# FocoosAI/focoos

Measured on AMD Instinct MI355X. Metric: images/sec @ 640^2 (infer bs=32), higher is better.
Workload: dtype bf16; 1 GPU; fai-detr-l-obj365 inference, bf16 MFMA, bs=32/GPU, 640x640, random-init weights (seed 0), uint8 HWC images resident in HBM, device post-process + D2H of packed detections included; global_batch=32, parallelism=replicas x1 (no data-path collective), steps_are=hipGraph replays, batches_in_flight=3, concurrent_batch_parts=1

## Files before the change

focoos_amd/_lib.py:

```python
from __future__ import annotations

import ctypes as C
import os
from typing import Optional

from .build import LIB_PATH, LIB_PATH_FP16

FX_ACT = {None: 0, "none": 0, "relu": 1, "silu": 2, "gelu": 3}


class FocoosAmdError(RuntimeError):
    pass


class FxConvDesc(C.Structure):
    _fields_ = [
        ("x", C.c_void_p), ("w", C.c_void_p), ("bias", C.c_void_p), ("residual", C.c_void_p), ("y", C.c_void_p),
        ("B", C.c_int32), ("H", C.c_int32), ("W", C.c_int32), ("C", C.c_int32), ("ldx", C.c_int32),
        ("Ho", C.c_int32), ("Wo", C.c_int32), ("N", C.c_int32), ("ldy", C.c_int32), ("ldr", C.c_int32),
        ("KH", C.c_int32), ("KW", C.c_int32), ("stride", C.c_int32), ("pad", C.c_int32),
        ("pool2", C.c_int32), ("act", C.c_int32), ("out_f32", C.c_int32), ("residual_after_act", C.c_int32),
        ("y_batch_stride", C.c_int64), ("w_frag", C.c_void_p), ("mask", C.c_void_p), ("ldm", C.c_int32), ("reserved0", C.c_int32),
    ]


def conv_frag_eligible(n: int, c: int, k: int, c32: bool = True) -> bool:
    if k == 1:
        return n % 256 == 0 and c % 256 == 0
    if k != 3:
        return False
    if c == 32:
        return c32 and n in (32, 64)
    return (n in (64, 128) or n % 256 == 0) and c % 64 == 0


class FxAugRecord(C.Structure):
    _fields_ = [
        ("crop_w", C.c_int32), ("crop_h", C.c_int32), ("pad_x", C.c_int32), ("pad_y", C.c_int32), ("res_w", C.c_int32), ("res_h", C.c_int32),
        ("crop_x", C.c_int32), ("crop_y", C.c_int32), ("flags", C.c_int32), ("reserved0", C.c_int32),
        ("brightness", C.c_float), ("contrast", C.c_float), ("saturation", C.c_float), ("reserved1", C.c_int32 * 3),
    ]


class FxPackEntry(C.Structure):
    _fields_ = [
        ("w", C.c_void_p), ("scale", C.c_void_p), ("bias", C.c_void_p), ("w_fwd", C.c_void_p), ("w_dgrad", C.c_void_p),
        ("w_fwd_frag", C.c_void_p), ("w_dgrad_frag", C.c_void_p), ("bias_out", C.c_void_p),
        ("N", C.c_int32), ("C", C.c_int32), ("KH", C.c_int32), ("KW", C.c_int32), ("ld_fwd", C.c_int32), ("ld_dgrad", C.c_int32),
        ("first_block", C.c_int32), ("n_offset", C.c_int32), ("n_total", C.c_int32), ("reserved", C.c_int32),
    ]


class FxPublishEntry(C.Structure):
    _fields_ = [
        ("w", C.c_void_p), ("bn_weight", C.c_void_p), ("bn_bias", C.c_void_p), ("bn_mean", C.c_void_p), ("bn_var", C.c_void_p),
        ("bias", C.c_void_p), ("w_rows", C.c_void_p), ("w_frag", C.c_void_p), ("bias_out", C.c_void_p), ("eps", C.c_double),
        ("N", C.c_int32), ("C", C.c_int32), ("KH", C.c_int32), ("KW", C.c_int32), ("Np", C.c_int32), ("first_block", C.c_int32),
    ]


class FxPwChainDesc(C.Structure):
    _fields_ = [
        ("x1", C.c_void_p), ("x2", C.c_void_p), ("residual", C.c_void_p), ("w1", C.c_void_p), ("bias1", C.c_void_p), ("y1", C.c_void_p),
        ("w2", C.c_void_p), ("bias2", C.c_void_p), ("y2", C.c_void_p),
        ("M", C.c_int32), ("K1a", C.c_int32), ("K1b", C.c_int32), ("N1", C.c_int32), ("N2", C.c_int32),
        ("ldx1", C.c_int32), ("ldx2", C.c_int32), ("ldr", C.c_int32), ("ldy1", C.c_int32), ("ldy2", C.c_int32),
        ("act1", C.c_int32), ("act2", C.c_int32),
        ("pool", C.c_void_p), ("ldp", C.c_int32), ("img_h", C.c_int32), ("img_w", C.c_int32), ("reserved0", C.c_int32),
    ]


class FxRcStage(C.Structure):
    _fields_ = [
        ("type", C.c_int32), ("K", C.c_int32), ("N", C.c_int32), ("act", C.c_int32),
        ("src", C.c_int32), ("dst", C.c_int32), ("aux", C.c_int32),
        ("ld", C.c_int32), ("ld2", C.c_int32), ("flags", C.c_int32),
        ("w", C.c_void_p), ("bias", C.c_void_p), ("gamma", C.c_void_p), ("beta", C.c_void_p), ("g0", C.c_void_p), ("g1", C.c_void_p),
    ]


_vp, _i, _f = C.c_void_p, C.c_int, C.c_float

SIGNATURES = {
    "fx_abi_version": [],
    "fx_build_flags": [],
    "fx_device_info": [_i, C.POINTER(C.c_int), C.c_char_p, _i],
    "fx_conv2d_nhwc_bf16": [C.POINTER(FxConvDesc), _vp],
    "fx_conv2d_variant": [_vp, C.c_char_p, _i],
    "fx_pw_chain_supported": [_i, _i, _i, _i],
    "fx_pw_chain_pool_supported": [_i, _i, _i, _i],
    "fx_conv3x3_flat_supported": [_i, _i, _i],
    "fx_pw_chain_bf16": [C.POINTER(FxPwChainDesc), _vp],
    "fx_stem_conv3x3s2": [_vp, _i, _vp, _vp, _vp, _vp, _vp, _i, _i, _i, _i, _vp],
    "fx_stem16_conv3x3s2": [_vp, _i, _vp, _vp, _vp, _vp, _vp, _i, _i, _i, _vp],
    "fx_conv3x3_c16_nhwc_bf16": [_vp, _i, _vp, _vp, _i, _vp, _i, _i, _i, _i, _i, _i, _i, _vp],
    "fx_semseg_eval_accumulate": [_vp, _vp, _i, _i, _i, _i, _i, _i, _i, _vp, C.c_int64, _vp, _vp, _i, _i, _vp, _vp, _vp, _vp, _vp],
    "fx_detr_eval_boxes_f32": [_vp, _vp, _vp, _i, _i, _i, _i, _vp, _vp, _vp, _vp, _vp],
    "fx_coco_match_workspace_bytes": [_i],
    "fx_coco_match_bbox": [_vp, _vp, _vp, _vp, _i, _i, _i, _vp, _vp, _vp, _vp, _vp, _vp, C.c_int64, _i, _vp, _vp, _vp, _vp, _vp, _vp, C.c_size_t,
                           _vp],
    "fx_mf_eval_masks_workspace_bytes": [_i, _i, _i],
    "fx_mf_eval_masks": [_vp, _vp, _vp, _i, _i, _i, _i, _i, _i, _i, _i, _vp, _vp, _vp, _vp, C.c_int64, _f, _vp, _vp, _vp, _vp, _vp, _vp, _vp, _vp,
                         _vp, _vp, C.c_size_t, _vp],
    "fx_coco_mask_inter": [_vp, _vp, _vp, C.c_int64, _vp, _vp, _vp, _i, _i, _i, _vp, _vp, _vp, _vp, _vp, C.c_int64, _vp, _vp, _vp, C.c_int64, _vp,
                           _vp, _vp],
    "fx_coco_match_segm": [_vp, _vp, _vp, _vp, _i, _i, _i, _i, _vp, _vp, _vp, _vp, _vp, _vp, _vp, C.c_int64, _i, _vp, _vp, _vp, _vp, _vp, _vp,
                           C.c_size_t, _vp],
    "fx_augment_images_u8": [_vp, _vp, _vp, _vp, _vp, C.c_int64, _vp, _vp, _i, _vp, _i, _i, _i, _vp, _vp],
    "fx_augment_labels": [_vp, _vp, _vp, _vp, _vp, _vp, C.c_int64, _vp, _vp, _vp, _i, _i, _vp, _i, _i, _i, _i, _vp, _vp],
    "fx_resize_bilinear_u8": [_vp, _i, _i, _vp, _i, _i, _vp],
    "fx_tile_gather_u8_f32": [_vp, _i, _i, _vp, _vp, _i, _vp, _i, _i, _vp],
    "fx_merge_detections_workspace_bytes": [_i, _i],
    "fx_merge_detections_nms": [_vp, _vp, _vp, _vp, _vp, _i, _i, _i, _i, _f, _i, _i, _vp, _vp, _vp, _vp, _vp, _vp, C.c_size_t, _vp],
    "fx_annotate_labels_from_detections": [_vp, _vp, _vp, _vp, _i, _i, _vp, _vp, _i, _i, _i, _i, _i, _i, _vp, _vp],
    "fx_annotate_u8": [_vp, _vp, _i, _i, _i, _i, _i, _vp, _vp, _vp, _vp, _vp, _i, C.c_int64, _vp, _vp, _i, _i, _i, _i, _vp],
    "fx_maxpool3x3s2_nhwc_bf16": [_vp, _i, _vp, _i, _i, _i, _i, _i, _vp],
    "fx_stem_conv12_u8_bf16": [_vp, _vp, _vp, _vp, _vp, _vp, _vp, _vp, _i, _i, _i, _i, _vp],
    "fx_stem_conv_pool_supported": [_i, _i, _i, _i],
    "fx_stem_conv3x3_relu_maxpool_bf16": [_vp, _i, _vp, _vp, _vp, _i, _i, _i, _i, _vp],
    "fx_avgpool2x2_nhwc_bf16": [_vp, _i, _vp, _i, _i, _i, _i, _i, _vp],
    "fx_resize_bilinear_nhwc_bf16": [_vp, _i, _vp, _i, _i, _i, _i, _i, _i, _i, _vp],
    "fx_add_rows_bf16": [_vp, _i, _vp, _i, _i, _vp, _i, _i, _i, _vp],
    "fx_layernorm_bf16": [_vp, _i, _vp, _i, _vp, _vp, _vp, _i, _i, _i, _vp],
    "fx_mha_bf16": [_vp, _i, _vp, _i, _vp, _i, _vp, _i, _i, _i, _i, _i, _vp],
    "fx_mha_workspace_bytes": [_i, _i, _i, _i, _i],
    "fx_mha_masked_bf16": [_vp, _i, _vp, _i, _vp, _i, _vp, _i, _i, _i, _i, _i, _vp, _i, _vp, C.c_size_t, _vp],
    "fx_upsample_nearest_add_nhwc_bf16": [_vp, _i, _vp, _i, _vp, _i, _i, _i, _i, _i, _i, _i, _vp],
    "fx_upsample_nearest_bwd_nhwc_bf16": [_vp, _i, _vp, _i, _i, _i, _i, _i, _i, _i, _vp],
    "fx_query_pixel_logits_bf16": [_vp, _i, _vp, _i, _i, _vp, _i, _vp, _i, _i, _i, _i, _i, _vp],
    "fx_mf_class_head": [_vp, _i, _vp, _vp, _vp, _i, _i, _i, _vp],
    "fx_mf_upsample_probs_f32": [_vp, _i, _i, _vp, _i, _i, _i, _vp],
    "fx_mf_upsample_probs_bf16": [_vp, _i, _i, _vp, _i, _i, _i, _vp],
    "fx_mf_postprocess_workspace_bytes": [_i, _i, _i],
    "fx_mf_postprocess_workspace_bytes_fused": [_i, _i, _i, _i, _i, _i],
    "fx_mf_postprocess": [_vp, _i, _i, _i, _i, _vp, _vp, _i, _i, _f, _f, _i, _vp, C.c_size_t, _vp, _vp, _vp, _vp, _vp, _vp, _vp, _vp],
    "fx_msda_bf16": [_vp, _i, _vp, _vp, _i, _i, _vp, _i, _vp, _i, _vp, _i, _vp, _i, _i, _i, _i, _i, _vp],
    "fx_rowmax_f32": [_vp, _i, _vp, _i, _i, _vp],
    "fx_enc_score_head_bf16": [_vp, _i, _vp, _i, _vp, _vp, _vp, _vp, _f, _vp, _vp, _i, _vp, _i, _vp, _i, _vp],
    "fx_row_chain": [_vp, _i, _i, _i, _vp],
    "fx_topk_rows_f32": [_vp, _i, _i, _i, _i, _vp, _vp, _vp],
    "fx_topk_rows_workspace_bytes": [_i, _i, _i],
    "fx_topk_rows_ws_f32": [_vp, _i, _i, _i, _i, _vp, _vp, _vp, C.c_size_t, _vp],
    "fx_gather_rows_bf16": [_vp, _i, _i, _vp, _i, _vp, _i, _i, _i, _vp],
    "fx_fill_rows_bf16": [_vp, _i, _i, _vp, _i, _vp, _i, _i, _vp],
    "fx_linear_k4_relu": [_vp, _vp, _vp, _vp, _i, _i, _i, _vp],
    "fx_bbox_head": [_vp, _i, _vp, _vp, _vp, _vp, _vp, _i, _i, _vp, _vp, _i, _i, _vp],
    "fx_detr_head_out": [_vp, _i, _vp, _vp, _vp, _i, _i, _vp],
    "fx_detr_postprocess": [_vp, _vp, _vp, _vp, _i, _i, _i, _i, _f, _vp, _vp, _vp, _vp, _vp],
    "fx_detr_match_cost_f32": [_vp, _i, _vp, _vp, _vp, _vp, _i, _i, _i, _i, _f, _f, _f, _f, _f, _vp, _vp],
    "fx_lsa_f32": [_vp, _i, _i, _i, _vp, _vp, _vp, _vp],
    "fx_lsa_status_f32": [_vp, _i, _i, _i, _vp, _vp, _vp, _vp, _vp],
    "fx_detr_set_loss_workspace_bytes": [_i, _i, _i],
    "fx_detr_set_loss_f32": [_vp, _i, _vp, _vp, _vp, _vp, _vp, _vp, _i, _i, _i, _i, _f, _f, _f, _f, _f, _f, _vp, _vp, _vp],
    "fx_detr_box_loss_f32": [_vp, _vp, _vp, _vp, _vp, _vp, _i, _i, _i, _i, _f, _f, _vp, _vp, _vp, _vp, _vp],
    "fx_detr_box_loss_bwd_f32": [_vp, _vp, _vp, _i, _i, _i, _vp, _vp, _vp, _vp],
    "fx_msda_f32_fwd": [_vp, _vp, _vp, _i, _i, _vp, _vp, _vp, _i, _i, _i, _i, _vp],
    "fx_msda_f32_bwd": [_vp, _vp, _vp, _i, _i, _vp, _vp, _vp, _vp, _vp, _vp, _i, _i, _i, _i, _vp],
    "fx_msda_train_fwd": [_vp, _i, _i, _vp, _vp, _i, _i, _vp, _vp, _vp, _i, _i, _i, _i, _vp],
    "fx_msda_train_bwd": [_vp, _i, _i, _vp, _vp, _i, _i, _vp, _vp, _vp, _vp, _i, _i, _vp, _vp, _i, _i, _i, _i, _vp],
    "fx_msda_bwd_slab_supported": [_vp, _i, _i, _i, _i, _i],
    "fx_msda_prep_bf16": [_vp, _i, _vp, _i, _vp, _vp, _vp, _i, _i, _i, _i, _vp],
    "fx_msda_prep_bwd_bf16": [_vp, _vp, _vp, _vp, _vp, _i, _vp, _i, _i, _i, _i, _i, _vp],
    "fx_msda_train_bwd_slab": [_vp, _i, _i, _vp, _vp, _vp, _i, _i, _vp, _vp, _vp, _i, _vp, _i, _vp, _vp, _i, _i, _i, _i, _vp],
    "fx_adamw_workspace_bytes": [],
    "fx_adamw_step_f32": [_vp, _vp, _vp, _vp, C.c_int64, _vp, _vp, _vp, _vp, _i, _i, _f, _f, _f, _f, _vp, _vp, _vp],
    "fx_adamw_step_scaled_f32": [_vp, _vp, _vp, _vp, C.c_int64, _vp, _vp, _vp, _vp, _i, _f, _f, _f, _f, _vp, _vp, _vp, _f, _f, _i, _vp],
    "fx_conv2d_wgrad_nhwc_bf16": [_vp, _i, _vp, _i, _vp, _i, _i, _i, _i, _i, _i, _i, _i, _i, _i, _i, _vp],
    "fx_conv2d_wgrad_bias_nhwc_bf16": [_vp, _i, _vp, _i, _vp, _vp, _i, _i, _i, _i, _i, _i, _i, _i, _i, _i, _i, _vp],
    "fx_point_sample_f32": [_vp, _i, _i, _i, _vp, _vp, _vp, _vp, _i, _i, _vp],
    "fx_mask_match_cost_f32": [_vp, _i, _vp, _vp, _vp, _vp, _i, _i, _i, _i, _i, C.c_float, C.c_float, C.c_float, _i, _vp, _vp],
    "fx_mask_match_cost_workspace_bytes": [_i, _i, _i],
    "fx_mask_match_cost_ws_f32": [_vp, _i, _vp, _vp, _vp, _vp, _i, _i, _i, _i, _i, C.c_float, C.c_float, C.c_float, _i, _vp, _vp, C.c_size_t, _vp],
    "fx_mask_set_loss_workspace_bytes": [_i, _i, _i, _i],
    "fx_mask_set_loss_f32": [_vp, _i, _vp, _i, _i, _vp, _i, _i, _i, _vp, _vp, _i, _vp, _vp, _vp, _i, _vp, _i, _i, _i, _i, _i, C.c_float, C.c_float,
                             C.c_float, C.c_float, C.c_float, _vp, C.c_size_t, _vp, _vp],
    "fx_mask_set_loss_cls_f32": [_vp, _i, _vp, _i, _i, _vp, _i, _i, _i, _vp, _vp, _i, _vp, _vp, _vp, _i, _vp, _i, _i, _i, _i, _i, C.c_float, _i, C.c_float,
                                 C.c_float, C.c_float, C.c_float, C.c_float, C.c_float, _vp, C.c_size_t, _vp, _vp],
    "fx_mask_class_loss_workspace_bytes": [_i, _i],
    "fx_mask_class_loss_f32": [_vp, _i, _vp, _vp, _vp, _vp, _i, _i, _i, _i, C.c_float, C.c_float, C.c_float, C.c_float, _vp, C.c_size_t, _vp, _vp],
    "fx_mask_class_loss_bwd_f32": [_vp, _i, _vp, _vp, _vp, _vp, _i, _i, _i, _i, C.c_float, C.c_float, C.c_float, C.c_float, _vp, _vp, _i, _vp],
    "fx_dwconv3x3s2_nhwc_bf16": [_vp, _i, _vp, _vp, _vp, _i, _i, _i, _i, _i, _vp],
    "fx_dwconv3x3s2_nhwc_f32out": [_vp, _i, _vp, _vp, _vp, _i, _i, _i, _i, _i, _vp],
    "fx_global_mean_nhwc_bf16": [_vp, _i, _vp, _i, _i, _i, _i, _vp],
    "fx_pooled_linear_f32": [_vp, _i, _vp, _vp, _i, _vp, _i, _i, _i, _i, _vp],
    "fx_channel_gate_nhwc_bf16": [_vp, _i, _vp, _i, _i, _vp, _i, _vp, _i, _vp, _i, _i, _i, _i, _vp],
    "fx_seg_postprocess_workspace_bytes": [_i, _i, _i, _i, _i, _i],
    "fx_seg_postprocess": [_vp, _i, _i, _i, _i, _vp, _vp, _i, _i, C.c_float, _i, _vp, C.c_size_t, _vp, _vp, _vp, _vp, _vp, _vp, _vp, _vp, _vp],
    "fx_pack_conv_weights_f32": [_vp, _vp, _vp, _vp, _vp, _vp, _i, _i, _i, _i, _vp],
    "fx_unpack_conv_wgrad_f32": [_vp, _vp, _vp, _i, _i, _i, _i, _i, _i, _vp],
    "fx_linear_wgrad_bias_bf16": [_vp, _i, _vp, _i, _vp, _i, _vp, _i, _i, _i, _i, _i, _vp],
    "fx_conv2d_wgrad_splits": [_i, _i, _i, _i, _i, _i, _i],
    "fx_conv2d_wgrad_variant": [_i, _i, _i, _i, _i, _i, _i, _i, _i, C.c_char_p, _i],
    "fx_conv2d_wgrad_partial_nhwc_bf16": [_vp, _i, _vp, _i, _vp, C.c_int64, _i, _i, _i, _i, _i, _i, _i, _i, _i, _i, _i, _i, _vp],
    "fx_unpack_conv_wgrad_sum_f32": [_vp, C.c_int64, _i, _vp, _vp, _i, _i, _i, _i, _i, _i, _vp],
    "fx_relu_bwd_bf16": [_vp, _i, _vp, _i, _vp, _i, _vp, _i, C.c_int64, _i, _i, _vp],
    "fx_zero_insert2_nhwc_bf16": [_vp, _i, _vp, _i, _i, _i, _i, _i, _i, _i, _vp],
    "fx_avgpool2x2_bwd_nhwc_bf16": [_vp, _i, _vp, _i, _i, _i, _i, _i, _vp],
    "fx_maxpool3x3s2_bwd_nhwc_bf16": [_vp, _i, _vp, _i, _vp, _i, _i, _i, _i, _i, _vp, _vp],
    "fx_normalize_pad8": [_vp, _i, _vp, _vp, _vp, C.c_int64, _vp],
    "fx_stem_conv3x3s2_linear": [_vp, _i, _vp, _vp, _vp, _vp, _vp, _i, _i, _i, _i, _vp],
    "fx_bn_stats_bf16": [_vp, _i, _i, _vp, C.c_int64, _i, _vp],
    "fx_bn_finalize_f32": [_vp, C.c_float, _vp, _vp, C.c_float, C.c_float, _vp, _vp, _vp, _vp, _vp, _vp, _vp, _i, _vp],
    "fx_bn_apply_bf16": [_vp, _i, _i, _vp, _vp, _vp, _i, _i, _vp, _i, C.c_int64, _i, _vp],
    "fx_bn_bwd_stats_bf16": [_vp, _i, _vp, _i, _i, _vp, _i, _vp, _vp, _vp, _vp, _i, _vp, C.c_int64, _i, _vp],
    "fx_bn_bwd_apply_bf16": [_vp, _i, _vp, _i, _i, _vp, _i, _vp, _vp, _vp, _vp, _i, _vp, C.c_float, _vp, _i, _vp, _i, C.c_int64, _i, _vp, _vp, _vp],
    "fx_act_fwd_bf16": [_vp, _i, _vp, _i, C.c_int64, _i, _i, _vp],
    "fx_act_bwd_bf16": [_vp, _i, _vp, _i, _vp, _i, C.c_int64, _i, _i, _vp],
    "fx_colsum_bf16": [_vp, _i, _vp, C.c_int64, _i, _vp],
    "fx_layernorm_bwd_bf16": [_vp, _i, _vp, _i, _vp, _vp, _i, _vp, _vp, _i, _i, _vp],
    "fx_resize_bilinear_bwd_nhwc_bf16": [_vp, _i, _vp, _i, _i, _i, _i, _i, _i, _i, _vp],
    "fx_cast_f32_bf16": [_vp, _vp, C.c_int64, _vp],
    "fx_mha_bwd_workspace_bytes": [_i, _i, _i, _i],
    "fx_mha_bwd_bf16": [_vp, _i, _vp, _i, _vp, _i, _vp, _i, _vp, _i, _vp, _i, _vp, _i, _vp, _i, _i, _i, _i, _i, _vp, C.c_size_t, _vp],
    "fx_mha_masked_bwd_bf16": [_vp, _i, _vp, _i, _vp, _i, _vp, _i, _vp, _i, _vp, _i, _vp, _i, _i, _i, _i, _i, _vp, _i, _vp, C.c_size_t, _vp],
    "fx_mask_set_loss_bwd_f32": [_vp, _i, _vp, _i, _i, _vp, _i, _i, _i, _vp, _vp, _i, _vp, _vp, _vp, _i, _vp, _i, _i, _i, _i, _i, C.c_float, C.c_float,
                                 C.c_float, C.c_float, C.c_float, _vp, C.c_size_t, _vp, _vp, _i, _vp, _vp],
    "fx_mask_set_loss_cls_bwd_f32": [_vp, _i, _vp, _i, _i, _vp, _i, _i, _i, _vp, _vp, _i, _vp, _vp, _vp, _i, _vp, _i, _i, _i, _i, _i, C.c_float, _i, C.c_float,
                                     C.c_float, C.c_float, C.c_float, C.c_float, C.c_float, _vp, C.c_size_t, _vp, _vp, _i, _vp, _vp],
    "fx_planes_to_rows_bf16": [_vp, _i, _i, _vp, _i, _i, _i, _vp],
    "fx_dwconv3x3s2_bwd_nhwc_bf16": [_vp, _i, _vp, _i, _vp, _vp, _i, _vp, _i, _i, _i, _i, _vp],
    "fx_rowdot_nhwc_bf16": [_vp, _i, _vp, _i, C.c_float, _vp, _i, _i, _i, _i, _i, _vp],
    "fx_bcast_vec_nhwc_bf16": [_vp, _i, C.c_float, _vp, _i, _i, _i, _i, _vp],
    "fx_scatter_rows_bf16": [_vp, _i, _vp, _i, _vp, _i, _i, _i, _i, _vp],
    "fx_pack_entry_blocks": [_i, _i, _i, _i],
    "fx_pack_weights_many_f32": [_vp, _i, _i, _vp],
    "fx_pack_frag_bf16": [_vp, _vp, _i, _i, _vp],
    "fx_publish_entry_blocks": [_i, _i, _i, _i],
    "fx_publish_weights_f32": [_vp, _i, _i, _vp],
    "fx_pack_linear_weights_f32": [_vp, _vp, _vp, _vp, _vp, _i, _i, _i, _i, _vp],
    "fx_box_refine_f32": [_vp, _vp, _vp, C.c_int64, _f, _vp],
    "fx_box_refine_bwd_f32": [_vp, _vp, _vp, _vp, _vp, C.c_int64, _f, _vp],
    "fx_vfl_loss_bf16": [_vp, _i, _vp, _vp, _f, _f, _f, _vp, _vp, _i, C.c_int64, _i, _vp],
    "fx_stream_fork": [_vp, _vp],
    "fx_stream_join": [_vp, _vp],
    "fx_graph_begin": [_vp],
    "fx_graph_end": [_vp, C.POINTER(C.c_void_p)],
    "fx_graph_launch": [_vp, _vp],
    "fx_graph_destroy": [_vp],
    "fx_graph_time": [_vp, _vp, _i, C.POINTER(C.c_float)],
}

_libs: dict = {}
_DTYPE = [os.environ.get("FX_DTYPE", "bf16")]


def compute_dtype() -> str:
    return _DTYPE[0]


def set_compute_dtype(name: str) -> str:
    if name not in ("bf16", "fp16"):
        raise FocoosAmdError(f"compute dtype {name!r}: the engine has a bfloat16 and an fp16 (+ loss scale) build")
    prev, _DTYPE[0] = _DTYPE[0], name
    return prev


class using_compute_dtype:

    def __init__(self, name: str):
        self.name, self.prev = name, None

    def __enter__(self):
        self.prev = set_compute_dtype(self.name)
        return self

    def __exit__(self, *exc):
        _DTYPE[0] = self.prev
        return False


def act_dtype():
    import torch

    return torch.float16 if _DTYPE[0] == "fp16" else torch.bfloat16


def lib_path(name: str = None) -> str:
    if (name or _DTYPE[0]) == "fp16":
        return os.environ.get("FOCOOS_AMD_LIB_FP16", LIB_PATH_FP16)
    return os.environ.get("FOCOOS_AMD_LIB", LIB_PATH)


FX_ABI_VERSION = 17


def load(name: str = None) -> C.CDLL:
    name = name or _DTYPE[0]
    if name in _libs:
        return _libs[name]
    import torch
    path = lib_path(name)
    if not os.path.exists(path):
        raise FocoosAmdError(
            f"{path} not found: the gfx950 HIP kernels are not built. Run `python -c 'import __graft_entry__ as g; g.build()'` "
            "(or `python -m focoos_amd.build`). focoos_amd has no CPU/PyTorch fallback by design."
        )
    lib = C.CDLL(path)
    for sym, argtypes in SIGNATURES.items():
        fn = getattr(lib, sym)
        fn.argtypes = argtypes
        fn.restype = C.c_int
    lib.fx_mha_bwd_workspace_bytes.restype = C.c_size_t
    lib.fx_seg_postprocess_workspace_bytes.restype = C.c_size_t
    lib.fx_mask_match_cost_workspace_bytes.restype = C.c_size_t
    lib.fx_mf_postprocess_workspace_bytes_fused.restype = C.c_size_t
    lib.fx_mask_set_loss_workspace_bytes.restype = C.c_size_t
    lib.fx_mask_class_loss_workspace_bytes.restype = C.c_size_t
    lib.fx_topk_rows_workspace_bytes.restype = C.c_size_t
    lib.fx_coco_match_workspace_bytes.restype = C.c_size_t
    lib.fx_mf_eval_masks_workspace_bytes.restype = C.c_size_t
    lib.fx_merge_detections_workspace_bytes.restype = C.c_size_t
    lib.fx_error_string.argtypes = [C.c_int]
    lib.fx_error_string.restype = C.c_char_p
    if lib.fx_abi_version() != FX_ABI_VERSION:
        raise FocoosAmdError(f"ABI version mismatch: library {lib.fx_abi_version()} != binding {FX_ABI_VERSION} (stale {os.path.basename(path)}: rebuild)")
    if bool(lib.fx_build_flags() & 2) != (name == "fp16"):
        raise FocoosAmdError(f"{path} was built for the other 16-bit element type (fx_build_flags = {lib.fx_build_flags()}) than {name!r}")
    _libs[name] = lib
    return lib


_warned_pk = False


def two_queue_safe() -> bool:
    global _warned_pk
    if not (load().fx_build_flags() & 1) or os.environ.get("FX_ALLOW_PK_TWO_QUEUES") == "1":
        return True
    if not _warned_pk:
        import warnings

        warnings.warn("libfocoos_amd was built with packed-fp32 instructions (FX_PK_F32): concurrent batch parts and the weight-gradient "
                      "side stream are disabled (two-queue hazard); rebuild without FX_PK_F32 for the default configuration")
        _warned_pk = True
    return False


def check(rc: int, what: str = "") -> None:
    if rc != 0:
        msg = load().fx_error_string(rc).decode()
        raise FocoosAmdError(f"libfocoos_amd {what} failed: {msg} (code {rc})")
```

focoos_amd/csrc/conv3x3_flat.hip:

```cpp
#include <type_traits>

#include "pw_common.h"

struct C3Args {
  const bf16_t* x;
  const bf16_t* wp;
  const float* bias;
  const bf16_t* res;
  bf16_t* y;
  int H, W, C, N, ldx, ldy, ldr, M;
  int act, res_after;
  int HLp;
  int HW;
  int64_t y_bstride;
  unsigned x_bytes, r_bytes;
};

template <int KT, int CC, int TN, int TM, int WN, int WM, int ACT, int RESMODE, int LOADER = 1>
__global__ __launch_bounds__((WN* WM + LOADER) * 64, 1) void conv3x3_flat_kernel(const C3Args p) {
  constexpr int NW = WN * WM, NT = (NW + LOADER) * 64, NDW = NW + LOADER;
  constexpr int BM = WM * TM * 32, BN = WN * TN * 32;
  constexpr int RL = CC / 8, ROWB = CC * 2;
  constexpr int KJ = 4;
  constexpr int NTAP = KT == 9 ? 9 : CC / 64;
  constexpr int PF = KJ;
  constexpr int RLT = BN / 8;
  static_assert(TN <= 2 && (KT == 9 ? CC == 64 : CC % 64 == 0), "tap = 64 channels = 4 k-steps");
  extern __shared__ __attribute__((aligned(16))) unsigned char smem[];

  const int tid = threadIdx.x, lane = tid & 63;
  const int wave = __builtin_amdgcn_readfirstlane(tid >> 6);
  const bool is_loader = LOADER && wave == NW;
  const int l32 = lane & 31, half = lane >> 5;
  const int wn = wave % WN, wm = wave / WN;
  const int nNt = p.N / BN;
  const int bid = fx_xcd_remap(blockIdx.x, gridDim.x);
  const int m0 = (bid / nNt) * BM, n0 = (bid % nNt) * BN;
  const int lo = KT == 9 ? m0 - p.W - 1 : m0;
  const int NCH = p.C / CC;
  const int buf_bytes = p.HLp * ROWB;
  const __amdgpu_buffer_rsrc_t xr = __builtin_amdgcn_make_buffer_rsrc((void*)p.x, 0, p.x_bytes, 0x00020000);
  unsigned char* T = smem;

  auto dma_chunk = [&](int cc, unsigned char* buf, int first, int step) {
    const int ninstr = p.HLp * RL / 64;
    for (int i = first; i < ninstr; i += step) {
      const int q = i * 64 + lane;
      const int r = q / RL, pc = q % RL;
      const int lc = pw_swz<RL>(r, pc);
      const int f = lo + r;
      const bool ok = f >= 0 && f < p.M;
      pw_dma16(xr, buf + i * 1024, ok ? (unsigned)(f * p.ldx + cc * CC + lc * 8) * 2u : FX_OOB);
    }
  };

  auto dma_res = [&](int first) {
    const __amdgpu_buffer_rsrc_t rr = __builtin_amdgcn_make_buffer_rsrc((void*)p.res, 0, p.r_bytes, 0x00020000);
    for (int i = first; i < BM * RLT / 64; i += NDW) {
      const int q = i * 64 + lane;
      const int r = q / RLT, pc = q % RLT;
      const int lc = pw_swz<RLT>(r, pc);
      const int m = m0 + r;
      pw_dma16(rr, T + i * 1024, m < p.M ? (unsigned)(m * p.ldr + n0 + lc * 8) * 2u : FX_OOB);
    }
  };

  f32x16 acc[TN][TM];
  bf16x8 ar[PF][TN];
  unsigned mask9[TM];
  int rbase[TM];
  const int Cs = p.C >> 4;
  const bf16_t* wbase = p.wp + (size_t)((n0 >> 5) + wn * TN) * (size_t)(KT * Cs) * 512 + lane * 8;
  auto a_ptr = [&](int a, int cc, int s) -> const bf16_t* {
    const int ks = KT == 9 ? (s / KJ) * Cs + cc * KJ + (s % KJ) : cc * (CC / 16) + s;
    return wbase + ((size_t)a * (size_t)(KT * Cs) + ks) * 512;
  };
  if (is_loader) {
    if (lane < 8) *reinterpret_cast<uint4*>(smem + (NCH > 1 ? 2 : 1) * buf_bytes + lane * 16) = make_uint4(0, 0, 0, 0);
    dma_chunk(0, smem, NW, NDW);
    for (int cc = 0; cc < NCH; ++cc) {
      asm volatile("s_waitcnt vmcnt(0)" ::: "memory");
      __syncthreads();
      if (cc + 1 < NCH) dma_chunk(cc + 1, smem + ((cc + 1) & 1) * buf_bytes, 0, 1);
    }
    __syncthreads();
    if constexpr (RESMODE != 0) {
      dma_res(NW);
      asm volatile("s_waitcnt vmcnt(0)" ::: "memory");
      __syncthreads();
    }
    __syncthreads();
  } else {
    if (!LOADER && wave == 0 && lane < 8) *reinterpret_cast<uint4*>(smem + buf_bytes + lane * 16) = make_uint4(0, 0, 0, 0);
    dma_chunk(0, smem, wave, NDW);
#pragma unroll
    for (int a = 0; a < TN; ++a)
#pragma unroll
      for (int gq = 0; gq < 4; ++gq) {
        const float4 bb = p.bias ? *reinterpret_cast<const float4*>(p.bias + n0 + (wn * TN + a) * 32 + 8 * gq + 4 * half) : make_float4(0.f, 0.f, 0.f, 0.f);
#pragma unroll
        for (int b = 0; b < TM; ++b) {
          acc[a][b][4 * gq] = bb.x; acc[a][b][4 * gq + 1] = bb.y; acc[a][b][4 * gq + 2] = bb.z; acc[a][b][4 * gq + 3] = bb.w;
        }
      }
    const int HW = p.H * p.W;
#pragma unroll
    for (int b = 0; b < TM; ++b) {
      const int pl = (wm * TM + b) * 32 + l32;
      const int m = m0 + pl;
      rbase[b] = KT == 9 ? pl + p.W + 1 : pl;
      const bool ok = m < p.M;
      const int mm = ok ? m : 0;
      const int rem = mm % HW;
      const int yy = rem / p.W, xx = rem - yy * p.W;
      unsigned msk = 0;
#pragma unroll
      for (int t = 0; t < 9; ++t) {
        const int dy = t / 3 - 1, dx = t % 3 - 1;
        if (ok && (unsigned)(yy + dy) < (unsigned)p.H && (unsigned)(xx + dx) < (unsigned)p.W) msk |= 1u << t;
      }
      mask9[b] = KT == 9 ? msk : 0x1ffu;
    }
#pragma unroll
    for (int i = 0; i < PF; ++i)
#pragma unroll
      for (int a = 0; a < TN; ++a) {
        ar[i][a] = bf16x8{0, 0, 0, 0, 0, 0, 0, 0};
        c3_ldg_async(ar[i][a], a_ptr(a, 0, i));
      }
    const int zrow = (NCH > 1 ? 2 : 1) * buf_bytes;
    int hc[KJ];
#pragma unroll
    for (int j = 0; j < KJ; ++j) hc[j] = (j * 2 + half) << 4;
    constexpr int SWM = (RL >= 16 ? 0xf0 : 0x70);
    constexpr int SWS = (RL >= 16 ? 4 : 3);
    auto tap_setup = [&](int t, int toff, int bufo, int (&ra)[TM], int (&sw)[TM]) {
#pragma unroll
      for (int b = 0; b < TM; ++b) {
        const int r = rbase[b] + toff;
        const bool ok = KT == 9 ? ((mask9[b] >> t) & 1u) : true;
        ra[b] = ok ? bufo + r * ROWB : zrow;
        sw[b] = ok ? ((r << SWS) & SWM) : 0;
      }
    };
    for (int cc = 0; cc < NCH; ++cc) {
      if (cc == 0) asm volatile("s_waitcnt vmcnt(0)" ::: "memory");
      __syncthreads();
      const int bufo = (cc & 1) * buf_bytes;
      const int ccn = cc + 1 < NCH ? cc + 1 : cc;
      int ra[TM], sw[TM];
      tap_setup(0, KT == 9 ? -p.W - 1 : 0, bufo, ra, sw);
      bf16x8 xb[2][TM];
#pragma unroll
      for (int b = 0; b < TM; ++b) xb[0][b] = *reinterpret_cast<const bf16x8*>(smem + ((hc[0] ^ sw[b]) + ra[b]));
#pragma unroll 1
      for (int t = 0; t < NTAP; ++t) {
        const int tn = t + 1;
        const bool last_tap = t == NTAP - 1;
        const int co = KT == 9 ? 0 : t * 128, con = KT == 9 ? 0 : tn * 128;
        const bf16_t* wnext[TN];
#pragma unroll
        for (int a = 0; a < TN; ++a) wnext[a] = a_ptr(a, last_tap ? ccn : cc, last_tap ? 0 : tn * KJ);
        int ran[TM], swn[TM];
        tap_setup(last_tap ? 0 : tn, (KT != 9 || last_tap) ? 0 : (tn / 3 - 1) * p.W + (tn % 3 - 1), bufo, ran, swn);
        auto kstep = [&](auto jc) {
          constexpr int j = decltype(jc)::value;
          constexpr bool tap_end = j + 1 == KJ;
          if constexpr (TN == 1) c3_wait<(KJ - 1) * TN>(ar[j][0]); else c3_wait<(KJ - 1) * TN>(ar[j][0], ar[j][1]);
#pragma unroll
          for (int a = 0; a < TN; ++a) {
#pragma unroll
            for (int b = 0; b < TM; ++b) {
              acc[a][b] = FX_MFMA_32x32x16(ar[j][a], xb[j & 1][b], acc[a][b]);
              if (a == 0) {
                if constexpr (!tap_end) {
                  xb[(j + 1) & 1][b] = *reinterpret_cast<const bf16x8*>(smem + (((co + hc[tap_end ? 0 : j + 1]) ^ sw[b]) + ra[b]));
                } else {
                  if (!last_tap) xb[0][b] = *reinterpret_cast<const bf16x8*>(smem + (((con + hc[0]) ^ swn[b]) + ran[b]));
                }
              }
              if (b == TM - 1) c3_ldg_async<j * 1024>(ar[j][a], wnext[a]);
              __builtin_amdgcn_sched_barrier(0);
            }
          }
        };
        c3_static_for<KJ>(kstep);
#pragma unroll
        for (int b = 0; b < TM; ++b) {
          ra[b] = ran[b];
          sw[b] = swn[b];
        }
      }
    }
#pragma unroll
    for (int i = 0; i < PF; ++i) {
      if constexpr (TN == 1) c3_wait<0>(ar[i][0]); else c3_wait<0>(ar[i][0], ar[i][1]);
    }
    __syncthreads();
    if constexpr (RESMODE != 0) {
      dma_res(wave);
      asm volatile("s_waitcnt vmcnt(0)" ::: "memory");
      __syncthreads();
    }
  #pragma unroll
      for (int a = 0; a < TN; ++a)
  #pragma unroll
        for (int b = 0; b < TM; ++b)
  #pragma unroll
          for (int gq = 0; gq < 4; ++gq) {
            const int row = (wm * TM + b) * 32 + l32;
            const int chunk = (wn * TN + a) * 4 + gq;
            unsigned char* tp = T + row * (BN * 2) + (pw_swz<RLT>(row, chunk) << 4) + half * 8;
            float v0 = acc[a][b][4 * gq], v1 = acc[a][b][4 * gq + 1], v2 = acc[a][b][4 * gq + 2], v3 = acc[a][b][4 * gq + 3];
            float r0 = 0.0f, r1 = 0.0f, r2 = 0.0f, r3 = 0.0f;
            if constexpr (RESMODE != 0) {
              const uint2 rv = *reinterpret_cast<const uint2*>(tp);
              r0 = bf16lo_to_f32(rv.x); r1 = bf16hi_to_f32(rv.x);
              r2 = bf16lo_to_f32(rv.y); r3 = bf16hi_to_f32(rv.y);
            }
            if constexpr (RESMODE == 1) { v0 += r0; v1 += r1; v2 += r2; v3 += r3; }
            if constexpr (ACT == FX_ACT_RELU) {
              v0 = fmaxf(v0, 0.0f); v1 = fmaxf(v1, 0.0f); v2 = fmaxf(v2, 0.0f); v3 = fmaxf(v3, 0.0f);
            } else if constexpr (ACT == FX_ACT_SILU) {
              v0 = v0 / (1.0f + __expf(-v0)); v1 = v1 / (1.0f + __expf(-v1)); v2 = v2 / (1.0f + __expf(-v2)); v3 = v3 / (1.0f + __expf(-v3));
            }
            if constexpr (RESMODE == 2) { v0 += r0; v1 += r1; v2 += r2; v3 += r3; }
            if constexpr (RESMODE == 3) {
              v0 = r0 > 0.0f ? v0 : 0.0f; v1 = r1 > 0.0f ? v1 : 0.0f; v2 = r2 > 0.0f ? v2 : 0.0f; v3 = r3 > 0.0f ? v3 : 0.0f;
            }
            uint2 o;
            o.x = pack_bf16x2(v0, v1);
            o.y = pack_bf16x2(v2, v3);
            *reinterpret_cast<uint2*>(tp) = o;
          }

    __syncthreads();
  }
  for (int q = tid; q < BM * RLT; q += NT) {
    const int row = q / RLT, lc = q % RLT;
    const int m = m0 + row;
    if (m < p.M) {
      const uint4 v = *reinterpret_cast<const uint4*>(T + row * (BN * 2) + (pw_swz<RLT>(row, lc) << 4));
      size_t yo = (size_t)m * p.ldy;
      if (p.y_bstride) {
        const int bb = m / p.HW;
        yo = (size_t)bb * p.y_bstride + (size_t)(m - bb * p.HW) * p.ldy;
      }
      *reinterpret_cast<uint4*>(p.y + yo + n0 + lc * 8) = v;
    }
  }
}

template <int KT, int CC, int TN, int TM, int WN, int WM, int ACT, int RESMODE, int LOADER = 1>
static int launch_c3(C3Args& a, hipStream_t stream) {
  constexpr int NW = WN * WM, BM = WM * TM * 32, BN = WN * TN * 32, RL = CC / 8;
  constexpr int RPI = 64 / RL > 0 ? 64 / RL : 1;
  const int HL = BM + (KT == 9 ? 2 * a.W + 2 : 0);
  a.HLp = (HL + RPI - 1) / RPI * RPI;
  const int halo = (a.C / CC > 1 ? 2 : 1) * a.HLp * CC * 2 + 128, tile = BM * BN * 2;
  const int smem = halo > tile ? halo : tile;
  if (smem > 160 * 1024) return FX_ERR_UNSUPPORTED;
  if (!LOADER && a.C != CC) return FX_ERR_UNSUPPORTED;
  auto kern = conv3x3_flat_kernel<KT, CC, TN, TM, WN, WM, ACT, RESMODE, LOADER>;
  static int attr_smem = 0;
  if (smem > attr_smem) {
    if (hipFuncSetAttribute(reinterpret_cast<const void*>(kern), hipFuncAttributeMaxDynamicSharedMemorySize, smem) != hipSuccess) return FX_ERR_RUNTIME;
    attr_smem = smem;
  }
  hipLaunchKernelGGL(kern, dim3(((a.M + BM - 1) / BM) * (a.N / BN)), dim3((NW + LOADER) * 64), smem, stream, a);
  return fx_launch_status();
}

int fx_c3_epilogue_mode(int act, bool has_res, int res_after) {
  if (!has_res) return act == FX_ACT_RELU ? 0 : (act == FX_ACT_SILU ? 1 : (act == FX_ACT_NONE ? 3 : -1));
  if (act == FX_ACT_SILU && res_after == 1) return 2;
  if (act == FX_ACT_RELU && res_after == 0) return 4;
  if (act == FX_ACT_NONE && res_after == 2) return 5;
  if (act == FX_ACT_NONE && res_after == 0) return 6;
  return -1;
}

bool fx_conv3x3_flat_fits(int C, int N, int W) {
  if (C % 64 != 0 || !(N == 64 || N == 128 || N == 256)) return false;
  const int BM = N == 256 ? 128 : 256;
  const int HLp = (BM + 2 * W + 2 + 7) / 8 * 8;
  const int halo = (C / 64 > 1 ? 2 : 1) * HLp * 128 + 128, tile = BM * N * 2;
  return (halo > tile ? halo : tile) <= 160 * 1024;
}

extern "C" int fx_conv3x3_flat_supported(int C, int N, int W) {
  return (fx_conv3x3_kplane_supported(C, N, W) || fx_conv3x3_c32_supported(C, N, W, 0) || fx_conv3x3_flat_fits(C, N, W)) ? 1 : 0;
}

static void c3_fill(C3Args& a, const ConvArgs& c, const bf16_t* w_frag) {
  a.x = c.x; a.wp = w_frag; a.bias = c.bias; a.res = c.res; a.y = reinterpret_cast<bf16_t*>(c.y);
  a.H = c.H; a.W = c.W; a.C = c.C; a.N = c.N; a.ldx = c.ldx; a.ldy = c.ldy; a.ldr = c.ldr; a.M = c.M;
  a.act = c.act; a.res_after = c.res_after; a.HLp = 0; a.HW = c.Ho * c.Wo; a.y_bstride = c.y_bstride;
  a.x_bytes = c.x_bytes; a.r_bytes = c.r_bytes;
}

int fx_launch_conv3x3_flat(const ConvArgs& c, const bf16_t* w_frag, int mode, hipStream_t stream) {
  C3Args a;
  c3_fill(a, c, w_frag);
#define FX_C3_TILE(ACT_, RM_)                                                      \
  {                                                                                \
    if (c.N == 64) return launch_c3<9, 64, 1, 4, 2, 2, ACT_, RM_>(a, stream);      \
    if (c.N == 128) return launch_c3<9, 64, 2, 4, 2, 2, ACT_, RM_>(a, stream);     \
    return launch_c3<9, 64, 2, 4, 4, 1, ACT_, RM_>(a, stream);                     \
  }
  switch (mode) {
    case 0: FX_C3_TILE(FX_ACT_RELU, 0)
    case 1: FX_C3_TILE(FX_ACT_SILU, 0)
    case 2: FX_C3_TILE(FX_ACT_SILU, 2)
    case 3: FX_C3_TILE(FX_ACT_NONE, 0)
    case 5: FX_C3_TILE(FX_ACT_NONE, 3)
    default: return FX_ERR_UNSUPPORTED;
  }
#undef FX_C3_TILE
}

int fx_launch_pw_flat(const ConvArgs& c, const bf16_t* w_frag, int mode, hipStream_t stream) {
  C3Args a;
  c3_fill(a, c, w_frag);
  static const int no_loader = fx_tune("FX_PW_NO_LOADER", 1);
  if (c.C == 256 && no_loader) {
    switch (mode) {
      case 0: return launch_c3<1, 256, 2, 4, 4, 1, FX_ACT_RELU, 0, 0>(a, stream);
      case 1: return launch_c3<1, 256, 2, 4, 4, 1, FX_ACT_SILU, 0, 0>(a, stream);
      case 3: return launch_c3<1, 256, 2, 4, 4, 1, FX_ACT_NONE, 0, 0>(a, stream);
      case 4: return launch_c3<1, 256, 2, 4, 4, 1, FX_ACT_RELU, 1, 0>(a, stream);
      case 5: return launch_c3<1, 256, 2, 4, 4, 1, FX_ACT_NONE, 3, 0>(a, stream);
      case 6: return launch_c3<1, 256, 2, 4, 4, 1, FX_ACT_NONE, 1, 0>(a, stream);
      default: return FX_ERR_UNSUPPORTED;
    }
  }
  static const int bm64 = fx_tune("FX_PWF_BM64_MAX_M", 20000);
  if (c.M <= bm64 && (mode == 0 || mode == 3)) {
    if (mode == 0) return launch_c3<1, 256, 2, 2, 4, 1, FX_ACT_RELU, 0>(a, stream);
    return launch_c3<1, 256, 2, 2, 4, 1, FX_ACT_NONE, 0>(a, stream);
  }
  switch (mode) {
    case 0: return launch_c3<1, 256, 2, 4, 4, 1, FX_ACT_RELU, 0>(a, stream);
    case 1: return launch_c3<1, 256, 2, 4, 4, 1, FX_ACT_SILU, 0>(a, stream);
    case 3: return launch_c3<1, 256, 2, 4, 4, 1, FX_ACT_NONE, 0>(a, stream);
    case 4: return launch_c3<1, 256, 2, 4, 4, 1, FX_ACT_RELU, 1>(a, stream);
    case 5: return launch_c3<1, 256, 2, 4, 4, 1, FX_ACT_NONE, 3>(a, stream);
    case 6: return launch_c3<1, 256, 2, 4, 4, 1, FX_ACT_NONE, 1>(a, stream);
    default: return FX_ERR_UNSUPPORTED;
  }
}
```

focoos_amd/csrc/conv_igemm.hip:

```cpp
#include <stdio.h>

#include "conv_common.h"

template <int BM, int BN, int BK, int WM, int WN, bool POOL, int NSTAGE = 2>
__global__ __launch_bounds__(256, (BK == 32 ? 4 : 2)) void conv_igemm_kernel(const ConvArgs p) {
  constexpr int CPR = BK / 8, RPP = 256 / CPR;
  constexpr int A_PASS = BM / RPP, B_PASS = (BN + RPP - 1) / RPP;
  constexpr int WTM = BM / WM, WTN = BN / WN, TM = WTM / 32, TN = WTN / 32;
  constexpr int A_BYTES = BM * BK * 2, B_BYTES = BN * BK * 2, STAGE = A_BYTES + B_BYTES;
  constexpr int EPI_LD = BN + 4;
  static_assert(WM * WN == 4, "4 waves");
  static_assert(BM % RPP == 0, "A passes");
  extern __shared__ __attribute__((aligned(16))) unsigned char smem[];

  const int tid = threadIdx.x, lane = tid & 63, wave = tid >> 6;
  const int wm = wave / WN, wn = wave % WN;
  const int bid = fx_xcd_remap(blockIdx.x, gridDim.x);
  const int mt = bid / p.nNt, nt = bid % p.nNt;
  const int m0 = mt * BM, n0 = nt * BN;

  const __amdgpu_buffer_rsrc_t xr = __builtin_amdgcn_make_buffer_rsrc((void*)p.x, 0, p.x_bytes, 0x00020000);
  const __amdgpu_buffer_rsrc_t wr = __builtin_amdgcn_make_buffer_rsrc((void*)p.w, 0, p.w_bytes, 0x00020000);

  const int kc = tid % CPR, r_in = tid / CPR;
// ... 28 lines not shown
    _Pragma("unroll") for (int i = 0; i < A_PASS; ++i) {                                                             \
      if constexpr (!POOL) {                                                                                         \
        int hi = a_hi0[i] + (KH_), wi = a_wi0[i] + (KW_);                                                            \
        bool ok = a_ok[i] && (unsigned)hi < (unsigned)p.H && (unsigned)wi < (unsigned)p.W;                           \
        ra[i] = buf_load16(xr, ok ? (unsigned)(a_off[i] + delta_) * 2u : FX_OOB);                                     \
      } else {                                                                                                       \
        float s_[8] = {0, 0, 0, 0, 0, 0, 0, 0};                                                                      \
        int cnt_ = 0;                                                                                                \
        _Pragma("unroll") for (int dy = 0; dy < 2; ++dy) _Pragma("unroll") for (int dx = 0; dx < 2; ++dx) {          \
          bool ok = a_ok[i] && (a_hi0[i] + dy) < p.H && (a_wi0[i] + dx) < p.W;                                       \
          uint4 v_ = buf_load16(xr, ok ? (unsigned)(a_off[i] + delta_ + (dy * p.W + dx) * p.ldx) * 2u : FX_OOB);      \
          float f_[8];                                                                                               \
          unpack_bf16x8(v_, f_);                                                                                     \
          _Pragma("unroll") for (int j = 0; j < 8; ++j) s_[j] += f_[j];                                              \
          cnt_ += ok ? 1 : 0;                                                                                        \
        }                                                                                                            \
        float inv_ = cnt_ > 0 ? 1.0f / (float)cnt_ : 0.0f;                                                           \
        _Pragma("unroll") for (int j = 0; j < 8; ++j) s_[j] *= inv_;                                                 \
        ra[i] = pack_bf16x8(s_);                                                                                     \
      }                                                                                                              \
    }                                                                                                                \
    _Pragma("unroll") for (int i = 0; i < B_PASS; ++i) {                                                             \
      if (BN % RPP == 0 || r_in + i * RPP < BN) rb[i] = buf_load16(wr, w_off[i] + (unsigned)(KBASE_)*2u);            \
    }                                                                                                                \
  }
#define FX_STORE_TILES(S_)                                                                                           \
  {                                                                                                                  \
    unsigned char* A_ = smem + (S_)*STAGE;                                                                           \
    unsigned char* B_ = A_ + A_BYTES;                                                                                \
    _Pragma("unroll") for (int i = 0; i < A_PASS; ++i) *reinterpret_cast<uint4*>(A_ + lds_off<BK>(r_in + i * RPP, kc)) = ra[i]; \
    _Pragma("unroll") for (int i = 0; i < B_PASS; ++i) {                                                             \
      if (BN % RPP == 0 || r_in + i * RPP < BN) *reinterpret_cast<uint4*>(B_ + lds_off<BK>(r_in + i * RPP, kc)) = rb[i]; \
    }                                                                                                                \
  }
#define FX_COMPUTE(S_)                                                                                               \
  {                                                                                                                  \
    const unsigned char* A_ = smem + (S_)*STAGE;                                                                     \
    const unsigned char* B_ = A_ + A_BYTES;                                                                          \
    _Pragma("unroll") for (int kk = 0; kk < BK / 16; ++kk) {                                                         \
      const int chunk = kk * 2 + lhalf;                                                                              \
      bf16x8 xa[TM], wb[TN];                                                                                         \
      _Pragma("unroll") for (int i = 0; i < TM; ++i) xa[i] =                                                         \
          *reinterpret_cast<const bf16x8*>(A_ + lds_off<BK>(wm * WTM + i * 32 + lrow, chunk));                       \
      _Pragma("unroll") for (int i = 0; i < TN; ++i) wb[i] =                                                         \
          *reinterpret_cast<const bf16x8*>(B_ + lds_off<BK>(wn * WTN + i * 32 + lrow, chunk));                       \
      _Pragma("unroll") for (int a = 0; a < TN; ++a) _Pragma("unroll") for (int b = 0; b < TM; ++b) acc[a][b] =      \
          FX_MFMA_32x32x16(wb[a], xa[b], acc[a][b]);                                 \
    }                                                                                                                \
  }

  f32x16 acc[TN][TM];
#pragma unroll
  for (int a = 0; a < TN; ++a)
#pragma unroll
    for (int b = 0; b < TM; ++b)
#pragma unroll
      for (int r = 0; r < 16; ++r) acc[a][b][r] = 0.0f;

  const int T = p.KH * p.KW * (p.C / BK);
  const int lrow = lane & 31, lhalf = lane >> 5;
  int kh = 0, kw = 0, c0 = 0, kbase = 0;
  FX_LOAD_TILES(kh, kw, c0, kbase);
  FX_STORE_TILES(0);
  __syncthreads();
  for (int t = 0; t < T - 1; ++t) {
    const int cur = (NSTAGE == 2) ? (t & 1) : 0;
    c0 += BK;
    kbase += BK;
    if (c0 == p.C) {
      c0 = 0;
      if (++kw == p.KW) {
        kw = 0;
        ++kh;
      }
    }
    FX_LOAD_TILES(kh, kw, c0, kbase);
    FX_COMPUTE(cur);
    if constexpr (NSTAGE == 2) {
      FX_STORE_TILES(cur ^ 1);
    } else {
      __syncthreads();
      FX_STORE_TILES(0);
    }
    __syncthreads();
  }
  constexpr int TPR = BN / 8, RPP2 = 256 / TPR, HALF = 64, PER_HALF = HALF / RPP2, NRES = BM / RPP2;
  const int col8 = (tid % TPR) * 8;
  const int n = n0 + col8;
  const bool n_ok = n < p.Nstore;
  uint4 rres[NRES];
  if (p.res) {
    const __amdgpu_buffer_rsrc_t rr = __builtin_amdgcn_make_buffer_rsrc((void*)p.res, 0, p.r_bytes, 0x00020000);
#pragma unroll
    for (int q = 0; q < NRES; ++q) {
      const int m = m0 + (q / PER_HALF) * HALF + tid / TPR + (q % PER_HALF) * RPP2;
      rres[q] = buf_load16(rr, (m < p.M && n_ok) ? (unsigned)(m * p.ldr + n) * 2u : FX_OOB);
    }
  }
  FX_COMPUTE((NSTAGE == 2) ? ((T - 1) & 1) : 0);
  __syncthreads();
#undef FX_LOAD_TILES
#undef FX_STORE_TILES
#undef FX_COMPUTE

  float* stg = reinterpret_cast<float*>(smem);
  float bs[8];
  if (p.bias && n_ok) {
    float4 b0 = *reinterpret_cast<const float4*>(p.bias + n), b1 = *reinterpret_cast<const float4*>(p.bias + n + 4);
    bs[0] = b0.x; bs[1] = b0.y; bs[2] = b0.z; bs[3] = b0.w; bs[4] = b1.x; bs[5] = b1.y; bs[6] = b1.z; bs[7] = b1.w;
  } else {
#pragma unroll
    for (int j = 0; j < 8; ++j) bs[j] = 0.0f;
  }
#pragma unroll
  for (int hh = 0; hh < BM / HALF; ++hh) {
    if ((wm * WTM) / HALF == hh) {
#pragma unroll
      for (int a = 0; a < TN; ++a)
#pragma unroll
        for (int b = 0; b < TM; ++b)
#pragma unroll
          for (int g = 0; g < 4; ++g) {
            int ml = wm * WTM + b * 32 + lrow - hh * HALF;
            int nl = wn * WTN + a * 32 + 8 * g + 4 * lhalf;
            float4 v = make_float4(acc[a][b][4 * g], acc[a][b][4 * g + 1], acc[a][b][4 * g + 2], acc[a][b][4 * g + 3]);
            *reinterpret_cast<float4*>(stg + ml * EPI_LD + nl) = v;
          }
    }
    __syncthreads();
#pragma unroll
    for (int j = 0; j < PER_HALF; ++j) {
      const int r = tid / TPR + j * RPP2;
      const int m = m0 + hh * HALF + r;
      if (m < p.M && n_ok) {
        float4 v0 = *reinterpret_cast<const float4*>(stg + r * EPI_LD + col8);
        float4 v1 = *reinterpret_cast<const float4*>(stg + r * EPI_LD + col8 + 4);
        float v[8] = {v0.x + bs[0], v0.y + bs[1], v0.z + bs[2], v0.w + bs[3], v1.x + bs[4], v1.y + bs[5], v1.z + bs[6], v1.w + bs[7]};
        float rf[8];
        if (p.res) {
          unpack_bf16x8(rres[hh * PER_HALF + j], rf);
          if (!p.res_after) {
#pragma unroll
            for (int i = 0; i < 8; ++i) v[i] += rf[i];
          }
        }
        if (p.act != FX_ACT_NONE) {
#pragma unroll
          for (int i = 0; i < 8; ++i) v[i] = fx_act(v[i], p.act);
        }
        if (p.res && p.res_after == 1) {
#pragma unroll
          for (int i = 0; i < 8; ++i) v[i] += rf[i];
        } else if (p.res && p.res_after == 2) {
#pragma unroll
          for (int i = 0; i < 8; ++i) v[i] = rf[i] > 0.0f ? v[i] : 0.0f;
        }
        if (p.mask) {
          float mf[8];
          unpack_bf16x8(*reinterpret_cast<const uint4*>(p.mask + (size_t)m * p.ldm + n), mf);
#pragma unroll
          for (int i = 0; i < 8; ++i) v[i] = mf[i] > 0.0f ? v[i] : 0.0f;
        }
        int64_t yoff;
        if (p.y_bstride) {
          int bb = m / HoWo;
          yoff = (int64_t)bb * p.y_bstride + (int64_t)(m - bb * HoWo) * p.ldy + n;
        } else {
          yoff = (int64_t)m * p.ldy + n;
        }
        if (p.out_f32) {
          float* dst = reinterpret_cast<float*>(p.y) + yoff;
          *reinterpret_cast<float4*>(dst) = make_float4(v[0], v[1], v[2], v[3]);
          *reinterpret_cast<float4*>(dst + 4) = make_float4(v[4], v[5], v[6], v[7]);
        } else {
          bf16_t* dst = reinterpret_cast<bf16_t*>(p.y) + yoff;
          *reinterpret_cast<uint4*>(dst) = pack_bf16x8(v);
        }
      }
    }
    if (hh + 1 < BM / HALF) __syncthreads();
  }
}

template <int BM, int BN, int BK, int WM, int WN, bool POOL, int NSTAGE = 2>
static int launch_conv(const ConvArgs& c, const bf16_t*, int, hipStream_t stream) {
  constexpr int STAGE = (BM + BN) * BK * 2;
  constexpr int EPI = 64 * (BN + 4) * 4;
  constexpr int SMEM = (NSTAGE * STAGE > EPI) ? NSTAGE * STAGE : EPI;
  static bool attr_set = false;
  auto kern = conv_igemm_kernel<BM, BN, BK, WM, WN, POOL, NSTAGE>;
  if (!attr_set) {
    if (hipFuncSetAttribute(reinterpret_cast<const void*>(kern), hipFuncAttributeMaxDynamicSharedMemorySize, SMEM) != hipSuccess)
      return FX_ERR_RUNTIME;
    attr_set = true;
  }
  ConvArgs a = c;
  a.nNt = (a.N + BN - 1) / BN;
  int nMt = (a.M + BM - 1) / BM;
  dim3 grid(nMt * a.nNt), block(256);
  hipLaunchKernelGGL(kern, grid, block, SMEM, stream, a);
  return fx_launch_status();
}

static int conv_prepare(const fx_conv_desc* d, ConvArgs& a) {
  FX_CHECK_ARG(d && d->x && d->w && d->y);
  FX_CHECK_ARG(d->B > 0 && d->H > 0 && d->W > 0 && d->Ho > 0 && d->Wo > 0 && d->N > 0);
  FX_CHECK_ARG(d->C > 0 && d->C % 32 == 0 && d->ldx >= d->C && d->ldx % 8 == 0);
  FX_CHECK_ARG(d->KH >= 1 && d->KW >= 1 && d->stride >= 1 && d->pad >= 0);
  const int Nstore = (d->N + 7) / 8 * 8;
  FX_CHECK_ARG(d->ldy >= Nstore && d->ldy % 8 == 0);
  FX_CHECK_ARG(!d->residual || (d->ldr >= Nstore && d->ldr % 8 == 0));
  FX_CHECK_ARG(((uintptr_t)d->x % 16) == 0 && ((uintptr_t)d->w % 16) == 0 && ((uintptr_t)d->y % 16) == 0);
  FX_CHECK_ARG(!d->residual || ((uintptr_t)d->residual % 16) == 0);
  FX_CHECK_ARG(!d->bias || ((uintptr_t)d->bias % 16) == 0);
  if (d->pool2) {
    FX_CHECK_ARG(d->KH == 1 && d->KW == 1 && d->stride == 1 && d->pad == 0);
    FX_CHECK_ARG(d->Ho == (d->H + 1) / 2 && d->Wo == (d->W + 1) / 2);
  } else {
    FX_CHECK_ARG(d->Ho == (d->H + 2 * d->pad - d->KH) / d->stride + 1);
    FX_CHECK_ARG(d->Wo == (d->W + 2 * d->pad - d->KW) / d->stride + 1);
  }
  if ((int64_t)d->B * d->H * d->W >= (1ll << 31) || (int64_t)d->B * d->Ho * d->Wo >= (1ll << 31)) return FX_ERR_UNSUPPORTED;
  const int64_t x_bytes = ((int64_t)d->B * d->H * d->W - 1) * d->ldx * 2 + (int64_t)d->C * 2;
  const int64_t Npad = (int64_t)(d->N + 127) / 128 * 128;
  const int64_t w_bytes = Npad * d->KH * d->KW * d->C * 2;
  const int64_t r_bytes = d->residual ? (((int64_t)d->B * d->Ho * d->Wo - 1) * d->ldr + Nstore) * 2 : 0;
  if (x_bytes >= 0xFFFFFFF0ll || w_bytes >= 0xFFFFFFF0ll || r_bytes >= 0xFFFFFFF0ll) return FX_ERR_UNSUPPORTED;
  a.x = reinterpret_cast<const bf16_t*>(d->x);
  a.w = reinterpret_cast<const bf16_t*>(d->w);
  a.bias = d->bias;
  a.res = reinterpret_cast<const bf16_t*>(d->residual);
  a.y = d->y;
  a.B = d->B; a.H = d->H; a.W = d->W; a.C = d->C; a.ldx = d->ldx;
  a.Ho = d->Ho; a.Wo = d->Wo; a.N = d->N; a.ldy = d->ldy; a.ldr = d->ldr;
  a.KH = d->KH; a.KW = d->KW; a.stride = d->stride; a.pad = d->pad;
  a.act = d->act; a.out_f32 = d->out_f32; a.res_after = d->residual_after_act;
  a.y_bstride = d->y_batch_stride;
  FX_CHECK_ARG(d->y_batch_stride >= 0 && d->y_batch_stride % 8 == 0);
  a.M = d->B * d->Ho * d->Wo;
  a.Ktot = d->KH * d->KW * d->C;
  a.Nstore = Nstore;
  a.nNt = 0;
  a.x_bytes = (unsigned)x_bytes;
  a.w_bytes = (unsigned)w_bytes;
  a.r_bytes = (unsigned)r_bytes;
  a.mask = reinterpret_cast<const bf16_t*>(d->mask);
  a.ldm = d->ldm;
  a.m_bytes = 0;
  if (d->mask) {
    FX_CHECK_ARG(d->ldm >= Nstore && d->ldm % 8 == 0 && ((uintptr_t)d->mask % 16) == 0 && !d->out_f32 && !d->pool2);
    const int64_t m_bytes = (((int64_t)d->B * d->Ho * d->Wo - 1) * d->ldm + Nstore) * 2;
    if (m_bytes >= 0xFFFFFFF0ll) return FX_ERR_UNSUPPORTED;
    a.m_bytes = (unsigned)m_bytes;
  }
  return FX_OK;
}

enum ConvRoute {
  R_C32, R_C3K, R_C3_FLAT, R_C3_S2, R_PWK, R_PW_FLAT, R_SMALL_M, R_DMA256, R_DMA128, R_POOL,
  R_K64_N128, R_K64_N64, R_K64_N32, R_K32_N128, R_K32_N64, R_K32_N32, R_UNSUPPORTED
};

static const struct {
  const char* label;
  bool by_c;
  ConvLauncher launch;
} kRoutes[R_UNSUPPORTED] = {
     {"conv3x3_c32<%d>", false, fx_launch_conv3x3_c32},
     {"conv3x3_kplane<%d>", false, fx_launch_conv3x3_kplane},
     {"conv3x3_flat<%d>", false, fx_launch_conv3x3_flat},
     {"conv3x3s2_kplane<%d>", false, fx_launch_conv3x3s2_kplane},
     {"pw_kplane<K%d>", true, fx_launch_pw_kplane},
     {"pw_flat<K%d>", true, fx_launch_pw_flat},
     {"conv_igemm<64,64,256,1stage>", false, launch_conv<64, 64, 256, 2, 2, false, 1>},
     {"conv_igemm_dma<256,256>", false, fx_launch_conv_dma256},
     {"conv_igemm_dma<256,128>", false, fx_launch_conv_dma128},
     {"conv_igemm<128,128,64,pool>", false, launch_conv<128, 128, 64, 2, 2, true>},
     {"conv_igemm<128,128,64>", false, launch_conv<128, 128, 64, 2, 2, false>},
     {"conv_igemm<128,64,64>", false, launch_conv<128, 64, 64, 2, 2, false>},
     {"conv_igemm<128,32,64>", false, launch_conv<128, 32, 64, 4, 1, false>},
     {"conv_igemm<128,128,32>", false, launch_conv<128, 128, 32, 2, 2, false>},
     {"conv_igemm<128,64,32>", false, launch_conv<128, 64, 32, 2, 2, false>},
     {"conv_igemm<128,32,32>", false, launch_conv<128, 32, 32, 4, 1, false>},
};

static ConvRoute conv_route(const fx_conv_desc* d, const ConvArgs& a, int mode) {
  const bool frag = d->w_frag && ((uintptr_t)d->w_frag % 16) == 0 && !d->mask && !d->pool2 && !d->out_f32;
  const int c3_min_m = fx_tune("FX_CONV3_MIN_M", 5000), pw_min_m = fx_tune("FX_PW_MIN_M", 5000);
  static const int c3_on = fx_tune("FX_CONV3_FLAT", 1), c3k_on = fx_tune("FX_C3_KPLANE", 1), c32_on = fx_tune("FX_C3_C32", 1);
  if (frag && c3_on && d->stride == 1 && d->KH == 3 && d->KW == 3 && d->pad == 1 && !d->y_batch_stride &&
      ((mode >= 0 && mode <= 3) || mode == 5) && a.M >= c3_min_m) {
    if (d->C == 32) {
      if (c32_on && fx_conv3x3_c32_supported(d->C, d->N, d->W, mode)) return R_C32;
    } else if (c3k_on && fx_conv3x3_kplane_supported(d->C, d->N, d->W)) {
      return R_C3K;
    } else if (fx_conv3x3_flat_fits(d->C, d->N, d->W)) {
      return R_C3_FLAT;
    }
  }
  static const int pw_on = fx_tune("FX_PW_FLAT", 1), pwk_on = fx_tune("FX_PW_KPLANE", 1);
  if (frag && pw_on && d->stride == 1 && d->KH == 1 && d->KW == 1 && d->pad == 0 && d->C % 256 == 0 && d->N % 256 == 0 && a.M >= pw_min_m &&
      (mode == 0 || mode == 1 || (mode >= 3 && mode <= 6)))
    return (pwk_on && fx_pw_kplane_supported(d->C, d->N, mode)) ? R_PWK : R_PW_FLAT;
  static const int s2_on = fx_tune("FX_C3S2_KPLANE", 1);
  if (frag && s2_on && d->stride == 2 && d->KH == 3 && d->KW == 3 && d->pad == 1 && !d->residual && d->H == 2 * d->Ho && d->W == 2 * d->Wo &&
      a.M >= c3_min_m && (mode == 0 || mode == 1 || mode == 3) && fx_conv3x3s2_kplane_supported(d->C, d->N, d->Wo, a.M))
    return R_C3_S2;
  static const int k64_min = fx_tune("FX_K64_MIN_KTOT", FX_K64_MIN_KTOT);
  static const int small_m = fx_tune("FX_SMALL_M", 16384);
  static const int small_k = fx_tune("FX_SMALL_M_KTOT", 2048);
  if (!d->pool2 && a.M <= small_m && d->C % 256 == 0 && a.Ktot <= small_k) return R_SMALL_M;
  if (!d->pool2 && !d->mask) {
    const int bn = fx_conv_dma_bn(a);
    if (bn) return bn == 256 ? R_DMA256 : R_DMA128;
  }
  if (d->pool2) return d->C % 64 != 0 ? R_UNSUPPORTED : R_POOL;
  if ((d->C % 64 == 0) && (a.Ktot >= k64_min)) return d->N > 64 ? R_K64_N128 : (d->N > 32 ? R_K64_N64 : R_K64_N32);
  return d->N > 64 ? R_K32_N128 : (d->N > 32 ? R_K32_N64 : R_K32_N32);
}

extern "C" int fx_conv2d_nhwc_bf16(const fx_conv_desc* d, fx_stream_t stream) {
  ConvArgs a;
  const int rc = conv_prepare(d, a);
  if (rc != FX_OK) return rc;
  const int mode = fx_c3_epilogue_mode(a.act, a.res != nullptr, a.res_after);
  const ConvRoute r = conv_route(d, a, mode);
  if (r == R_UNSUPPORTED) return FX_ERR_UNSUPPORTED;
  return kRoutes[r].launch(a, reinterpret_cast<const bf16_t*>(d->w_frag), mode, reinterpret_cast<hipStream_t>(stream));
}

extern "C" int fx_conv2d_variant(const fx_conv_desc* d, char* out, int cap) {
  FX_CHECK_ARG(out && cap >= 48);
  ConvArgs a;
  const int rc = conv_prepare(d, a);
  if (rc != FX_OK) return rc;
  const ConvRoute r = conv_route(d, a, fx_c3_epilogue_mode(a.act, a.res != nullptr, a.res_after));
  if (r == R_UNSUPPORTED) return FX_ERR_UNSUPPORTED;
  snprintf(out, cap, kRoutes[r].label, kRoutes[r].by_c ? d->C : d->N);
  return FX_OK;
}
```

focoos_amd/csrc/conv_pw_chain.hip:

```cpp
#include "pw_common.h"

struct PwChainArgs {
  const bf16_t* x1;
  const bf16_t* x2;
  const bf16_t* res;
  const bf16_t* w1p;
  const bf16_t* w2p;
  const float* b1;
  const float* b2;
  bf16_t* y1;
  bf16_t* y2;
  int ldx1, ldx2, ldr, ldy1, ldy2;
  int M, N1, act1, act2;
  unsigned x1_bytes, x2_bytes, r_bytes;
  bf16_t* pool;
  int ldp, H, W;
};

template <int RL, typename F>
__device__ __forceinline__ void pw_dma_rows_map(__amdgpu_buffer_rsrc_t r, unsigned char* tile, int nrows, int ld, int col0, int wave, int lane, F&& pix) {
  const int ninstr = nrows * RL / 64;
  for (int i = wave; i < ninstr; i += 4) {
    const int q = i * 64 + lane;
    const int row = q / RL, pc = q % RL;
    const int lc = pw_swz<RL>(row, pc);
    const int m = pix(row);
    const unsigned off = (m >= 0) ? (unsigned)(m * ld + col0 + lc * 8) * 2u : FX_OOB;
    pw_dma16(r, tile + i * 1024, off);
  }
}

template <int K1A, int K1B, int N2, int BM, bool QUAD = false>
__global__ __launch_bounds__(256, ((N2 <= 64 && K1B == 0) ? 4 : ((N2 <= 128 && (K1B == 0 || N2 <= 64)) ? 3 : 2))) void pw_chain_kernel(const PwChainArgs p) {
  constexpr int K1 = K1A + K1B, KS1 = K1 / 16, KS1A = K1A / 16;
  constexpr int RLA = K1A / 8, RLB = (K1B > 0 ? K1B : 64) / 8;
  constexpr int TM = BM / 32;
  constexpr int XA_BYTES = BM * K1A * 2, XB_BYTES = BM * K1B * 2;
  constexpr int PF1 = KS1 < 4 ? KS1 : 4;
  constexpr bool HAS2 = N2 > 0;
  constexpr int WN2 = !HAS2 ? 1 : (N2 >= 128 ? 4 : 2), WM2 = 4 / WN2;
  constexpr int TN2 = !HAS2 ? 1 : N2 / (32 * WN2), TM2 = BM / (32 * WM2);
  constexpr int RL2 = (HAS2 ? N2 : 64) / 8;
  constexpr int PF2 = 4;
  static_assert(BM == 64, "64-pixel tiles");
  static_assert(K1A % 64 == 0 && K1B % 64 == 0 && PF1 == 4, "K segments in multiples of 64 (= whole blocks of 4 k-steps)");
  static_assert(!HAS2 || (N2 % 64 == 0 && N2 <= 256), "N2");
  extern __shared__ __attribute__((aligned(16))) unsigned char smem[];
  unsigned char* XA = smem;
  unsigned char* XB = smem + XA_BYTES;
  unsigned char* T = smem + XA_BYTES + XB_BYTES;

  const int tid = threadIdx.x, lane = tid & 63;
  const int wave = __builtin_amdgcn_readfirstlane(tid >> 6);
  const int l32 = lane & 31, half = lane >> 5;
  const int m0 = blockIdx.x * BM;
  const int NG = p.N1 >> 8;
  const int KS2 = p.N1 >> 4;

  __shared__ int s_pix[QUAD ? BM : 1];
  if constexpr (QUAD) {
    if (tid < BM) {
      const int W2 = p.W >> 1, QI = (p.H >> 1) * W2;
      const int q = blockIdx.x * (BM / 4) + (tid >> 2), sub = tid & 3;
      int m = -1;
      if (q * 4 < p.M) {
        const int b = q / QI, rem = q - b * QI;
        const int y2 = rem / W2, x2 = rem - y2 * W2;
        m = (b * p.H + 2 * y2 + (sub >> 1)) * p.W + 2 * x2 + (sub & 1);
      }
      s_pix[tid] = m;
    }
    __syncthreads();
  }
  auto pix = [&](int row) -> int {
    if constexpr (!QUAD) {
      const int m = m0 + row;
      return m < p.M ? m : -1;
    } else {
      return s_pix[row];
    }
  };
  const __amdgpu_buffer_rsrc_t x1r = __builtin_amdgcn_make_buffer_rsrc((void*)p.x1, 0, p.x1_bytes, 0x00020000);
  pw_dma_rows_map<RLA>(x1r, XA, BM, p.ldx1, 0, wave, lane, pix);
  if constexpr (K1B > 0) {
    const __amdgpu_buffer_rsrc_t x2r = __builtin_amdgcn_make_buffer_rsrc((void*)p.x2, 0, p.x2_bytes, 0x00020000);
    pw_dma_rows_map<RLB>(x2r, XB, BM, p.ldx2, 0, wave, lane, pix);
  }
  const __amdgpu_buffer_rsrc_t rr = __builtin_amdgcn_make_buffer_rsrc((void*)(p.res ? p.res : p.x1), 0, p.res ? p.r_bytes : 0u, 0x00020000);

  const int wn2 = wave % WN2, wm2 = wave / WN2;
  f32x16 acc2[TN2][TM2];
#pragma unroll
  for (int a = 0; a < TN2; ++a)
#pragma unroll
    for (int b = 0; b < TM2; ++b)
#pragma unroll
      for (int r = 0; r < 16; ++r) acc2[a][b][r] = 0.0f;

  for (int g = 0; g < NG; ++g) {
    int l32g = l32, halfg = half, tidg = tid;
    asm volatile("" : "+v"(l32g), "+v"(halfg), "+v"(tidg));
    if (p.res) pw_dma_rows_map<32>(rr, T, BM, p.ldr, g * 256, wave, lane, pix);
    bf16x8 a2[PF2][TN2];
    const bf16_t* w2 = p.w2p + (size_t)((wn2 * TN2) * KS2 + g * 16) * 512 + lane * 8;
    if constexpr (HAS2) {
#pragma unroll
      for (int i = 0; i < PF2; ++i)
#pragma unroll
        for (int a = 0; a < TN2; ++a) a2[i][a] = pw_ldg_frag(w2 + (size_t)(a * KS2 + i) * 512);
    }
#pragma unroll
    for (int a = 0; a < 2; ++a) {
      const bf16_t* w1 = p.w1p + (size_t)((g * 8 + wave * 2 + a) * KS1) * 512 + lane * 8;
      bf16x8 a1[PF1];
#pragma unroll
      for (int i = 0; i < PF1; ++i) a1[i] = pw_ldg_frag(w1 + i * 512);
      f32x16 acc[TM];
#pragma unroll
      for (int gq = 0; gq < 4; ++gq) {
        const float4 bb = *reinterpret_cast<const float4*>(p.b1 + g * 256 + wave * 64 + a * 32 + 8 * gq + 4 * halfg);
#pragma unroll
        for (int b = 0; b < TM; ++b) {
          acc[b][4 * gq] = bb.x; acc[b][4 * gq + 1] = bb.y; acc[b][4 * gq + 2] = bb.z; acc[b][4 * gq + 3] = bb.w;
        }
      }
      if (a == 0) {
        asm volatile("s_waitcnt vmcnt(0)" ::: "memory");
        __syncthreads();
      }
#define FX_PW_STEPS(XT_, KROW_, RL_, KL0_)                                                                                  \
  _Pragma("unroll") for (int i = 0; i < PF1; ++i) {                                                                         \
    bf16x8 xb[TM];                                                                                                          \
    _Pragma("unroll") for (int b = 0; b < TM; ++b) {                                                                        \
      const int row = b * 32 + l32k;                                                                                         \
      xb[b] = *reinterpret_cast<const bf16x8*>((XT_) + row * ((KROW_)*2) + (pw_swz<RL_>(row, ((KL0_) + i) * 2 + halfg) << 4)); \
    }                                                                                                                       \
    _Pragma("unroll") for (int b = 0; b < TM; ++b) acc[b] = FX_MFMA_32x32x16(a1[i], xb[b], acc[b]); \
    const int kn = ks0 + i + PF1;                                                                                           \
    a1[i] = pw_ldg_frag(w1 + (kn < KS1 ? kn : KS1 - 1) * 512);  \
  }
#pragma unroll 1
      for (int ks0 = 0; ks0 < KS1; ks0 += PF1) {
        int l32k = l32g;
        asm volatile("" : "+v"(l32k));
        if (K1B == 0 || ks0 < KS1A) {
          FX_PW_STEPS(XA, K1A, RLA, ks0)
        } else {
          FX_PW_STEPS(XB, (K1B > 0 ? K1B : 64), RLB, ks0 - KS1A)
        }
      }
#undef FX_PW_STEPS
#pragma unroll
      for (int b = 0; b < TM; ++b)
#pragma unroll
        for (int gq = 0; gq < 4; ++gq) {
          const int row = b * 32 + l32g;
          const int chunk = wave * 8 + a * 4 + gq;
          unsigned char* tp = T + row * 512 + ((chunk ^ (row & 15)) << 4) + halfg * 8;
          float v0 = acc[b][4 * gq], v1 = acc[b][4 * gq + 1], v2 = acc[b][4 * gq + 2], v3 = acc[b][4 * gq + 3];
          if (p.res) {
            const uint2 r2 = *reinterpret_cast<const uint2*>(tp);
            v0 += bf16lo_to_f32(r2.x);
            v1 += bf16hi_to_f32(r2.x);
            v2 += bf16lo_to_f32(r2.y);
            v3 += bf16hi_to_f32(r2.y);
          }
          if (p.act1 == FX_ACT_RELU) {
            v0 = fmaxf(v0, 0.0f); v1 = fmaxf(v1, 0.0f); v2 = fmaxf(v2, 0.0f); v3 = fmaxf(v3, 0.0f);
          }
          uint2 o;
          o.x = pack_bf16x2(v0, v1);
          o.y = pack_bf16x2(v2, v3);
          *reinterpret_cast<uint2*>(tp) = o;
        }
    }
    __syncthreads();
#pragma unroll
    for (int i = 0; i < BM * 32 / 256; ++i) {
      const int q = tidg + i * 256;
      const int row = q >> 5, lc = q & 31;
      const uint4 v = *reinterpret_cast<const uint4*>(T + row * 512 + ((lc ^ (row & 15)) << 4));
      const int m = pix(row);
      if (m >= 0 && p.y1) *reinterpret_cast<uint4*>(p.y1 + (size_t)m * p.ldy1 + g * 256 + lc * 8) = v;
    }
    if constexpr (QUAD) {
#pragma unroll
      for (int i = 0; i < (BM / 4) * 32 / 256; ++i) {
        const int idx = tidg + i * 256;
        const int j = idx >> 5, lc = idx & 31;
        float s8[8] = {0, 0, 0, 0, 0, 0, 0, 0};
#pragma unroll
        for (int r = 0; r < 4; ++r) {
          const int row = 4 * j + r;
          float f[8];
          unpack_bf16x8(*reinterpret_cast<const uint4*>(T + row * 512 + ((lc ^ (row & 15)) << 4)), f);
#pragma unroll
          for (int e = 0; e < 8; ++e) s8[e] += f[e];
        }
#pragma unroll
        for (int e = 0; e < 8; ++e) s8[e] *= 0.25f;
        const int q = blockIdx.x * (BM / 4) + j;
        if (q * 4 < p.M) *reinterpret_cast<uint4*>(p.pool + (size_t)q * p.ldp + g * 256 + lc * 8) = pack_bf16x8(s8);
      }
    }
    if constexpr (HAS2) {
#pragma unroll
      for (int ks = 0; ks < 16; ++ks) {
        bf16x8 tb[TM2];
#pragma unroll
        for (int b = 0; b < TM2; ++b) {
          const int row = (wm2 * TM2 + b) * 32 + l32g;
          tb[b] = *reinterpret_cast<const bf16x8*>(T + row * 512 + (((ks * 2 + halfg) ^ (row & 15)) << 4));
        }
#pragma unroll
        for (int a = 0; a < TN2; ++a)
#pragma unroll
          for (int b = 0; b < TM2; ++b) acc2[a][b] = FX_MFMA_32x32x16(a2[ks % PF2][a], tb[b], acc2[a][b]);
        if (ks + PF2 < 16) {
#pragma unroll
          for (int a = 0; a < TN2; ++a) a2[ks % PF2][a] = pw_ldg_frag(w2 + (size_t)(a * KS2 + ks + PF2) * 512);
        }
      }
    }
    __syncthreads();
  }

  if constexpr (HAS2) {
#pragma unroll
    for (int a = 0; a < TN2; ++a)
#pragma unroll
      for (int gq = 0; gq < 4; ++gq) {
        const int n = (wn2 * TN2 + a) * 32 + 8 * gq + 4 * half;
        const float4 bb = *reinterpret_cast<const float4*>(p.b2 + n);
#pragma unroll
        for (int b = 0; b < TM2; ++b) {
          const int row = (wm2 * TM2 + b) * 32 + l32;
          float v0 = acc2[a][b][4 * gq] + bb.x, v1 = acc2[a][b][4 * gq + 1] + bb.y;
          float v2 = acc2[a][b][4 * gq + 2] + bb.z, v3 = acc2[a][b][4 * gq + 3] + bb.w;
          if (p.act2 == FX_ACT_RELU) {
            v0 = fmaxf(v0, 0.0f); v1 = fmaxf(v1, 0.0f); v2 = fmaxf(v2, 0.0f); v3 = fmaxf(v3, 0.0f);
          }
          uint2 o;
          o.x = pack_bf16x2(v0, v1);
          o.y = pack_bf16x2(v2, v3);
          *reinterpret_cast<uint2*>(T + row * (N2 * 2) + (pw_swz<RL2>(row, n >> 3) << 4) + half * 8) = o;
        }
      }
    __syncthreads();
#pragma unroll
    for (int i = 0; i < BM * RL2 / 256; ++i) {
      const int q = tid + i * 256;
      const int row = q / RL2, lc = q % RL2;
      const uint4 v = *reinterpret_cast<const uint4*>(T + row * (N2 * 2) + (pw_swz<RL2>(row, lc) << 4));
      const int m = pix(row);
      if (m >= 0) *reinterpret_cast<uint4*>(p.y2 + (size_t)m * p.ldy2 + lc * 8) = v;
    }
  }
}

template <int K1A, int K1B, int N2, bool QUAD = false>
static int launch_pw_chain(const PwChainArgs& a, hipStream_t stream) {
  constexpr int BM = 64;
  constexpr int SMEM = BM * (K1A + K1B) * 2 + BM * 512;
  static bool attr_set = false;
  auto kern = pw_chain_kernel<K1A, K1B, N2, BM, QUAD>;
  if (!attr_set) {
    if (hipFuncSetAttribute(reinterpret_cast<const void*>(kern), hipFuncAttributeMaxDynamicSharedMemorySize, SMEM) != hipSuccess)
      return FX_ERR_RUNTIME;
    attr_set = true;
  }
  hipLaunchKernelGGL(kern, dim3((a.M + BM - 1) / BM), dim3(256), SMEM, stream, a);
  return fx_launch_status();
}

#define FX_PW_INSTANCES(X)                                                                             \
  X(64, 0, 0) X(64, 0, 64) X(64, 0, 128) X(64, 64, 0) X(64, 64, 64) X(64, 64, 128)                     \
  X(128, 0, 0) X(128, 0, 128) X(128, 0, 256) X(128, 256, 0) X(128, 256, 128) X(128, 256, 256)          \
  X(256, 0, 0) X(256, 0, 256) X(256, 512, 0) X(256, 512, 256)

extern "C" int fx_pw_chain_supported(int K1a, int K1b, int N1, int N2) {
  if (N1 <= 0 || N1 % 256 != 0) return 0;
#define FX_PW_CASE(KA, KB, NN2) \
  if (K1a == KA && K1b == KB && N2 == NN2) return 1;
  FX_PW_INSTANCES(FX_PW_CASE)
#undef FX_PW_CASE
  return 0;
}

#define FX_PW_POOL_INSTANCES(X) X(64, 0, 128) X(128, 0, 256)

extern "C" int fx_pw_chain_pool_supported(int K1a, int K1b, int N1, int N2) {
  if (N1 <= 0 || N1 % 256 != 0) return 0;
#define FX_PW_CASE(KA, KB, NN2) \
  if (K1a == KA && K1b == KB && N2 == NN2) return 1;
  FX_PW_POOL_INSTANCES(FX_PW_CASE)
#undef FX_PW_CASE
  return 0;
}

extern "C" int fx_pw_chain_bf16(const fx_pw_chain_desc* d, fx_stream_t stream_) {
  FX_CHECK_ARG(d && d->x1 && d->w1 && d->bias1 && d->M > 0);
  FX_CHECK_ARG(d->y1 || (d->pool && d->N2 > 0));
  FX_CHECK_ARG(d->K1b == 0 || d->x2);
  FX_CHECK_ARG((d->act1 == FX_ACT_NONE || d->act1 == FX_ACT_RELU) && (d->act2 == FX_ACT_NONE || d->act2 == FX_ACT_RELU));
  FX_CHECK_ARG(d->N2 == 0 || (d->w2 && d->bias2 && d->y2));
  if (!fx_pw_chain_supported(d->K1a, d->K1b, d->N1, d->N2)) return FX_ERR_UNSUPPORTED;
  FX_CHECK_ARG(d->ldx1 >= d->K1a && d->ldx1 % 8 == 0 && (!d->y1 || (d->ldy1 >= d->N1 && d->ldy1 % 8 == 0)));
  FX_CHECK_ARG(d->K1b == 0 || (d->ldx2 >= d->K1b && d->ldx2 % 8 == 0));
  FX_CHECK_ARG(!d->residual || (d->ldr >= d->N1 && d->ldr % 8 == 0));
  FX_CHECK_ARG(d->N2 == 0 || (d->ldy2 >= d->N2 && d->ldy2 % 8 == 0));
  FX_CHECK_ARG(((uintptr_t)d->x1 % 16) == 0 && ((uintptr_t)d->x2 % 16) == 0 && ((uintptr_t)d->residual % 16) == 0);
  FX_CHECK_ARG(((uintptr_t)d->w1 % 16) == 0 && ((uintptr_t)d->w2 % 16) == 0 && ((uintptr_t)d->y1 % 16) == 0 && ((uintptr_t)d->y2 % 16) == 0);
  FX_CHECK_ARG(((uintptr_t)d->bias1 % 16) == 0 && ((uintptr_t)d->bias2 % 16) == 0);
  const int64_t x1_bytes = ((int64_t)d->M - 1) * d->ldx1 * 2 + (int64_t)d->K1a * 2;
  const int64_t x2_bytes = d->K1b ? ((int64_t)d->M - 1) * d->ldx2 * 2 + (int64_t)d->K1b * 2 : 0;
  const int64_t r_bytes = d->residual ? ((int64_t)d->M - 1) * d->ldr * 2 + (int64_t)d->N1 * 2 : 0;
  if (x1_bytes >= 0xFFFFFFF0ll || x2_bytes >= 0xFFFFFFF0ll || r_bytes >= 0xFFFFFFF0ll) return FX_ERR_UNSUPPORTED;
  PwChainArgs a;
  a.x1 = reinterpret_cast<const bf16_t*>(d->x1);
  a.x2 = reinterpret_cast<const bf16_t*>(d->x2);
  a.res = reinterpret_cast<const bf16_t*>(d->residual);
  a.w1p = reinterpret_cast<const bf16_t*>(d->w1);
  a.w2p = reinterpret_cast<const bf16_t*>(d->w2);
  a.b1 = d->bias1;
  a.b2 = d->bias2;
  a.y1 = reinterpret_cast<bf16_t*>(d->y1);
  a.y2 = reinterpret_cast<bf16_t*>(d->y2);
  a.ldx1 = d->ldx1; a.ldx2 = d->ldx2; a.ldr = d->ldr; a.ldy1 = d->ldy1; a.ldy2 = d->ldy2;
  a.M = d->M; a.N1 = d->N1; a.act1 = d->act1; a.act2 = d->act2;
  a.x1_bytes = (unsigned)x1_bytes; a.x2_bytes = (unsigned)x2_bytes; a.r_bytes = (unsigned)r_bytes;
  a.pool = reinterpret_cast<bf16_t*>(d->pool); a.ldp = d->ldp; a.H = d->img_h; a.W = d->img_w;
  hipStream_t stream = reinterpret_cast<hipStream_t>(stream_);
  if (d->pool) {
    FX_CHECK_ARG(d->img_h > 0 && d->img_w > 0 && d->img_h % 2 == 0 && d->img_w % 2 == 0 && d->M % (d->img_h * d->img_w) == 0);
    FX_CHECK_ARG(d->ldp >= d->N1 && d->ldp % 8 == 0 && ((uintptr_t)d->pool % 16) == 0);
    if (!fx_pw_chain_pool_supported(d->K1a, d->K1b, d->N1, d->N2)) return FX_ERR_UNSUPPORTED;
#define FX_PW_CASE(KA, KB, NN2) \
  if (d->K1a == KA && d->K1b == KB && d->N2 == NN2) return launch_pw_chain<KA, KB, NN2, true>(a, stream);
    FX_PW_POOL_INSTANCES(FX_PW_CASE)
#undef FX_PW_CASE
    return FX_ERR_UNSUPPORTED;
  }
#define FX_PW_CASE(KA, KB, NN2) \
  if (d->K1a == KA && d->K1b == KB && d->N2 == NN2) return launch_pw_chain<KA, KB, NN2>(a, stream);
  FX_PW_INSTANCES(FX_PW_CASE)
#undef FX_PW_CASE
  return FX_ERR_UNSUPPORTED;
}
```

focoos_amd/csrc/conv_pw_kplane.hip:

```cpp
#include <type_traits>

#include "pw_common.h"

#ifndef FX_PWK_RES_DEPTH
#define FX_PWK_RES_DEPTH 3
#endif

int fx_tune(const char* env_name, int default_value);

struct PWKArgs {
  const bf16_t* x;
  const bf16_t* wp;
  const float* bias;
  const bf16_t* res;
  bf16_t* y;
  int N, ldx, ldy, ldr, M;
  int ntg;
  int HW;
  int64_t y_bstride;
  unsigned x_bytes, r_bytes;
  int rot;
};

template <int OFF>
__device__ __forceinline__ void pwk_ldg(bf16x8& dst, unsigned voff, const bf16_t* sbase) {
  asm volatile("global_load_dwordx4 %0, %1, %2 offset:%3" : "+v"(dst) : "v"(voff), "s"(sbase), "n"(OFF) : "memory");
}
typedef __attribute__((address_space(3))) const bf16x8 pwk_lds_frag_t;
template <int IMM>
__device__ __forceinline__ bf16x8 pwk_lds_read(int addr) {
  return *reinterpret_cast<pwk_lds_frag_t*>((size_t)(unsigned)(addr + IMM));
}
__device__ __forceinline__ float pwk_act(float v, std::integral_constant<int, FX_ACT_RELU>) { return fmaxf(v, 0.0f); }
__device__ __forceinline__ float pwk_act(float v, std::integral_constant<int, FX_ACT_SILU>) { return v * __builtin_amdgcn_rcpf(1.0f + __expf(-v)); }
__device__ __forceinline__ float pwk_act(float v, std::integral_constant<int, FX_ACT_NONE>) { return v; }

template <int K, int ACT, int RESMODE, int TM = 4, int ABL = 0>
__global__ __launch_bounds__(256, TM == 4 ? 2 : 3) void conv_pw_kplane_kernel(const PWKArgs p) {
  constexpr int TN = 2, NW = 4, BM = TM * 32, BN = 256;
  constexpr int NTHR = 256, NDW = NTHR / 64;
  constexpr int KS = K / 16;
  constexpr int PLANE = BM * 16, XBYTES = 2 * KS * PLANE;
  constexpr int PF = 4;
  static_assert(KS % PF == 0 && (KS - 1) * PLANE < 65536, "plane offsets are 16-bit immediates");
  extern __shared__ __attribute__((aligned(16))) unsigned char smem[];
  float* biasL = reinterpret_cast<float*>(smem + XBYTES);

  const int tid = threadIdx.x, lane = tid & 63;
  const int wave = __builtin_amdgcn_readfirstlane(tid >> 6);
  const int l32 = lane & 31, half = lane >> 5;
  const int m0 = fx_xcd_remap(blockIdx.x, gridDim.x) * BM;
  const int nt_first = blockIdx.y * p.ntg;
  const int NT = min(p.N / BN, nt_first + p.ntg);
  const int cnt = NT - nt_first;
  const int rot = p.rot ? (int)(blockIdx.x % (unsigned)cnt) : 0;
  auto tile_of = [&](int k) { const int t = k + rot; return nt_first + (t >= cnt ? t - cnt : t); };

  for (int i = tid; i < p.N; i += NTHR) biasL[i] = p.bias ? p.bias[i] : 0.0f;
  {
    const __amdgpu_buffer_rsrc_t xr = __builtin_amdgcn_make_buffer_rsrc((void*)p.x, 0, p.x_bytes, 0x00020000);
    constexpr int NP = K / 8;
    static_assert(BM % 64 == 0, "64-row DMA blocks");
    for (int i = wave; i < (BM / 64) * NP; i += NDW) {
      const int blk = i / NP, c = i % NP;
      const int m = m0 + blk * 64 + lane;
      const int pln = (c & 1) * KS + (c >> 1);
      if constexpr (!(ABL & 16)) pw_dma16(xr, smem + pln * PLANE + blk * 1024, m < p.M ? (unsigned)(m * p.ldx + c * 8) * 2u : FX_OOB);
    }
  }
  f32x16 acc[TN][TM];
  bf16x8 ar[PF][TN];
  const unsigned wvoff = lane * 16;
  const bf16_t* wwave = p.wp + (size_t)(wave * TN) * KS * 512;
  auto w_ptr = [&](int a, int nt, int ks) -> const bf16_t* { return wwave + ((size_t)(nt * 8 + a) * KS + ks) * 512; };
#pragma unroll
  for (int a = 0; a < TN; ++a) {
    const bf16_t* w0 = w_ptr(a, tile_of(0), 0);
    c3_static_for<PF>([&](auto ic) {
      constexpr int i = decltype(ic)::value;
      ar[i][a] = bf16x8{0, 0, 0, 0, 0, 0, 0, 0};
      pwk_ldg<i * 1024>(ar[i][a], wvoff, w0);
    });
  }
  const int lds0 = (int)(unsigned)(size_t)((__attribute__((address_space(3))) unsigned char*)smem);
  int addr[TM];
#pragma unroll
  for (int b = 0; b < TM; ++b) addr[b] = lds0 + (b * 32 + l32) * 16 + half * KS * PLANE;
  asm volatile("s_waitcnt vmcnt(0)" ::: "memory");
  __syncthreads();

  for (int kt = 0; kt < cnt; ++kt) {
    const int nt = tile_of(kt);
    const int n0 = nt * BN;
    const int ntn = kt + 1 < cnt ? tile_of(kt + 1) : nt;
#pragma unroll
    for (int a = 0; a < TN; ++a)
#pragma unroll
      for (int gq = 0; gq < 4; ++gq) {
        const float4 bb = *reinterpret_cast<const float4*>(biasL + n0 + (wave * TN + a) * 32 + 8 * gq + 4 * half);
#pragma unroll
        for (int b = 0; b < TM; ++b) {
          acc[a][b][4 * gq] = bb.x; acc[a][b][4 * gq + 1] = bb.y; acc[a][b][4 * gq + 2] = bb.z; acc[a][b][4 * gq + 3] = bb.w;
        }
      }
    bf16x8 xb[2][TM];
#pragma unroll
    for (int b = 0; b < TM; ++b) xb[0][b] = pwk_lds_read<0>(addr[b]);
#pragma unroll 1
    for (int g = 0; g < KS / PF; ++g) {
      const bool last = g == KS / PF - 1;
      const bf16_t* wnext[TN];
#pragma unroll
      for (int a = 0; a < TN; ++a) wnext[a] = w_ptr(a, last ? ntn : nt, last ? 0 : (g + 1) * PF);
      const int aoff = g * PF * PLANE;
      auto kstep = [&](auto jc) {
        constexpr int j = decltype(jc)::value;
        if constexpr (TN == 1) c3_wait<(PF - 1) * TN>(ar[j][0]); else c3_wait<(PF - 1) * TN>(ar[j][0], ar[j][1]);
#pragma unroll
        for (int a = 0; a < TN; ++a) {
#pragma unroll
          for (int b = 0; b < TM; ++b) {
            if constexpr (!(ABL & 8)) acc[a][b] = FX_MFMA_32x32x16(ar[j][a], xb[j & 1][b], acc[a][b]);
            if (a == 0) {
              if constexpr (j + 1 < PF) xb[(j + 1) & 1][b] = pwk_lds_read<(j + 1) * PLANE>(addr[b] + aoff);
              else xb[0][b] = pwk_lds_read<PF * PLANE>(addr[b] + (last ? -PF * PLANE : aoff));
            }
            if constexpr (!(ABL & 1)) {
              if (b == TM - 1) pwk_ldg<j * 1024>(ar[j][a], wvoff, wnext[a]);
            }
            __builtin_amdgcn_sched_barrier(0);
          }
        }
      };
      c3_static_for<PF>(kstep);
    }
    constexpr int RD = (FX_PWK_RES_DEPTH < TM) ? FX_PWK_RES_DEPTH : TM;
    constexpr int RS = RD + 1 > TM ? TM : RD + 1;
    uint4 rr[RS][TN * 2];
    if constexpr (ABL & 4) {
#pragma unroll
      for (int i = 0; i < RS * TN * 2; ++i) (&rr[0][0])[i] = make_uint4(0, 0, 0, 0);
    }
    auto ld_res = [&](int b, uint4* dst) {
      const int m = min(m0 + b * 32 + l32, p.M - 1);
      const bf16_t* rrow = p.res + (size_t)m * p.ldr + n0 + wave * TN * 32 + half * 8;
#pragma unroll
      for (int a = 0; a < TN; ++a)
#pragma unroll
        for (int g2 = 0; g2 < 2; ++g2) dst[a * 2 + g2] = *reinterpret_cast<const uint4*>(rrow + a * 32 + g2 * 16);
    };
    if constexpr (RESMODE != 0 && !(ABL & 4)) {
#pragma unroll
      for (int b = 0; b < RD && b < TM; ++b) ld_res(b, rr[b % RS]);
    }
#pragma unroll
    for (int b = 0; b < TM; ++b) {
      if constexpr (RESMODE != 0 && !(ABL & 4)) {
        if (b + RD < TM) ld_res(b + RD, rr[(b + RD) % RS]);
      }
      const int row = b * 32 + l32;
      const int m = m0 + row;
      size_t yo = (size_t)m * p.ldy;
      if (p.y_bstride) {
        const int bb = m / p.HW;
        yo = (size_t)bb * p.y_bstride + (size_t)(m - bb * p.HW) * p.ldy;
      }
      bf16_t* yrow = p.y + yo + n0 + wave * TN * 32 + half * 8;
      const bool live = m < p.M;
#pragma unroll
      for (int a = 0; a < TN; ++a)
#pragma unroll
        for (int g2 = 0; g2 < 2; ++g2) {
          unsigned pk[2][2], rq[2][2] = {{0u, 0u}, {0u, 0u}};
          if constexpr (RESMODE != 0) {
            const uint4 R = rr[b % RS][a * 2 + g2];
            const auto s0 = __builtin_amdgcn_permlane32_swap(R.x, R.z, false, false);
            const auto s1 = __builtin_amdgcn_permlane32_swap(R.y, R.w, false, false);
            rq[0][0] = s0[0]; rq[1][0] = s0[1];
            rq[0][1] = s1[0]; rq[1][1] = s1[1];
          }
#pragma unroll
          for (int q = 0; q < 2; ++q) {
            const int gq = 2 * g2 + q;
            float v[4];
            const float r[4] = {bf16lo_to_f32(rq[q][0]), bf16hi_to_f32(rq[q][0]), bf16lo_to_f32(rq[q][1]),
                                bf16hi_to_f32(rq[q][1])};
#pragma unroll
            for (int e = 0; e < 4; ++e) {
              v[e] = acc[a][b][4 * gq + e];
              if constexpr (RESMODE == 1) v[e] += r[e];
              v[e] = pwk_act(v[e], std::integral_constant<int, ACT>{});
              if constexpr (RESMODE == 3) v[e] = r[e] > 0.0f ? v[e] : 0.0f;
            }
            pk[q][0] = pack_bf16x2(v[0], v[1]);
            pk[q][1] = pack_bf16x2(v[2], v[3]);
          }
#pragma unroll
          for (int w = 0; w < 2; ++w) {
            const auto sw = __builtin_amdgcn_permlane32_swap(pk[0][w], pk[1][w], false, false);
            pk[0][w] = sw[0];
            pk[1][w] = sw[1];
          }
          if (live && !((ABL & 2) && p.M > 0)) *reinterpret_cast<uint4*>(yrow + a * 32 + g2 * 16) = make_uint4(pk[0][0], pk[0][1], pk[1][0], pk[1][1]);
        }
    }
  }
#pragma unroll
  for (int i = 0; i < PF; ++i) {
    if constexpr (TN == 1) c3_wait<0>(ar[i][0]); else c3_wait<0>(ar[i][0], ar[i][1]);
  }
}

template <int K, int ACT, int RESMODE, int TM = 4, int ABL = 0>
static int launch_pwk(PWKArgs& a, hipStream_t stream) {
  constexpr int BM = TM * 32, BN = 256;
  const int smem = BM * K * 2 + a.N * 4;
  if (smem > 160 * 1024) return FX_ERR_UNSUPPORTED;
  const int mt = (a.M + BM - 1) / BM, NT = a.N / BN;
  static const int target = fx_tune("FX_PWK_TARGET_WGS", 512);
  const int want = K == 256 ? target : target / 2;
  int groups = mt >= want * 3 / 4 ? 1 : (want + mt - 1) / mt;
  if (groups > NT) groups = NT;
  a.ntg = (NT + groups - 1) / groups;
  groups = (NT + a.ntg - 1) / a.ntg;
  static const int rot = fx_tune("FX_PWK_ROT", 1);
  a.rot = rot;
  auto kern = conv_pw_kplane_kernel<K, ACT, RESMODE, TM, ABL>;
  static int attr_smem = 0;
  if (smem > attr_smem) {
    if (hipFuncSetAttribute(reinterpret_cast<const void*>(kern), hipFuncAttributeMaxDynamicSharedMemorySize, smem) != hipSuccess) return FX_ERR_RUNTIME;
    attr_smem = smem;
  }
  hipLaunchKernelGGL(kern, dim3(mt, groups), dim3(256), smem, stream, a);
  return fx_launch_status();
}

bool fx_pw_kplane_supported(int C, int N, int mode) {
  if (N <= 0 || N % 256 != 0 || N > 4096) return false;
  static const int k512_res = fx_tune("FX_PWK_K512_RES", 1);
  if (C == 256) return mode == 0 || mode == 1 || mode == 3 || mode == 4 || mode == 5 || mode == 6;
  if (C == 512) return mode == 0 || mode == 1 || mode == 3 || (k512_res && (mode == 4 || mode == 5 || mode == 6));
  return false;
}

int fx_launch_pw_kplane(const ConvArgs& c, const bf16_t* w_frag, int mode, hipStream_t stream) {
  if (!fx_pw_kplane_supported(c.C, c.N, mode)) return FX_ERR_UNSUPPORTED;
  PWKArgs a{};
  a.x = c.x; a.wp = w_frag; a.bias = c.bias; a.res = c.res; a.y = reinterpret_cast<bf16_t*>(c.y);
  a.N = c.N; a.ldx = c.ldx; a.ldy = c.ldy; a.ldr = c.ldr; a.M = c.M;
  a.HW = c.Ho * c.Wo; a.y_bstride = c.y_bstride; a.x_bytes = c.x_bytes; a.r_bytes = c.r_bytes;
  if (c.C == 256) {
    switch (mode) {
      case 0: return launch_pwk<256, FX_ACT_RELU, 0>(a, stream);
      case 1: return launch_pwk<256, FX_ACT_SILU, 0>(a, stream);
      case 3: return launch_pwk<256, FX_ACT_NONE, 0>(a, stream);
      case 4: return launch_pwk<256, FX_ACT_RELU, 1>(a, stream);
      case 5: return launch_pwk<256, FX_ACT_NONE, 3>(a, stream);
      case 6: return launch_pwk<256, FX_ACT_NONE, 1>(a, stream);
    }
  } else {
    switch (mode) {
      case 0: return launch_pwk<512, FX_ACT_RELU, 0>(a, stream);
      case 1: return launch_pwk<512, FX_ACT_SILU, 0>(a, stream);
      case 3: return launch_pwk<512, FX_ACT_NONE, 0>(a, stream);
      case 4: return launch_pwk<512, FX_ACT_RELU, 1>(a, stream);
      case 5: return launch_pwk<512, FX_ACT_NONE, 3>(a, stream);
      case 6: return launch_pwk<512, FX_ACT_NONE, 1>(a, stream);
    }
  }
  return FX_ERR_UNSUPPORTED;
}
```

focoos_amd/engine.py:

```python
from __future__ import annotations

import ctypes as C
import math
import os
import weakref
from typing import Dict, List, Optional, Sequence, Tuple

import torch

from . import _lib
from ._lib import FX_ACT, FxConvDesc, FxPwChainDesc, FxRcStage, check
from .engine_stdc import StdcEngineMixin, StdcPlanMixin
from .state_spec import RESNET_BLOCKS

BN_EPS = 1e-5
DEFAULT_STREAMS = 2
MIN_PART_BATCH = 4
DEFAULT_PIPELINE_DEPTH = 3


class NT:

    __slots__ = ("t", "B", "H", "W", "C", "ld", "off")

# ... 335 lines not shown

    def load_state_dict(self, sd: Dict[str, torch.Tensor]) -> None:
        self._pack_all(self._begin_load(sd))
        self._end_load()

    def _pack_all(self, sd: Dict[str, torch.Tensor]) -> None:
        P: Dict[str, PackedConv] = {}

        def cbn(name, conv="conv", norm="norm"):
            P[name] = self._pack_bn(sd, f"{name}.{conv}.weight", f"{name}.{norm}")

        if self.stdc:
            self._pack_stdc(sd, P)
        else:
            self._pack_backbone(sd, P)
        pd = "pixel_decoder"
        for i in range(3):
            P[f"{pd}.input_proj.{i}"] = self._pack_bn(sd, f"{pd}.input_proj.{i}.0.weight", f"{pd}.input_proj.{i}.1")
        for li in range(self.n_enc):
            p = f"{pd}.encoder.0.layers.{li}"
            Wi, bi_ = sd[f"{p}.self_attn.in_proj_weight"], sd[f"{p}.self_attn.in_proj_bias"]
            P[f"{p}.qk"] = self._pack_linear(Wi[:512], bi_[:512])
            P[f"{p}.v"] = self._pack_linear(Wi[512:], bi_[512:])
            P[f"{p}.out_proj"] = self._pack_linear(sd[f"{p}.self_attn.out_proj.weight"], sd[f"{p}.self_attn.out_proj.bias"])
            for l in ("linear1", "linear2"):
                P[f"{p}.{l}"] = self._pack_linear(sd[f"{p}.{l}.weight"], sd[f"{p}.{l}.bias"])
            for nrm in ("norm1", "norm2"):
                setattr(self, f"_ln_{p}.{nrm}", None)
        self.ln = {}

        def ln(name):
            self._pack_ln(sd, name)

        for li in range(self.n_enc):
            ln(f"{pd}.encoder.0.layers.{li}.norm1")
            ln(f"{pd}.encoder.0.layers.{li}.norm2")
        for i in range(2):
            cbn(f"{pd}.lateral_convs.{i}")
            cbn(f"{pd}.downsample_convs.{i}")
        for blk in ("fpn_blocks", "pan_blocks"):
            for i in range(2):
                p = f"{pd}.{blk}.{i}"
                w1, b1 = _fold_bn(sd, f"{p}.conv1.conv.weight", f"{p}.conv1.norm")
                w2, b2 = _fold_bn(sd, f"{p}.conv2.conv.weight", f"{p}.conv2.norm")
                P[f"{p}.conv12"] = self._pack(torch.cat([w1, w2], 0), torch.cat([b1, b2], 0))
                for j in range(3):
                    q = f"{p}.bottlenecks.{j}"
                    w3, b3 = _fold_bn(sd, f"{q}.conv1.conv.weight", f"{q}.conv1.norm")
                    w1_, b1_ = _fold_bn(sd, f"{q}.conv2.conv.weight", f"{q}.conv2.norm")
                    w3 = w3.clone()
                    w3[:, :, 1:2, 1:2] += w1_
                    P[f"{q}.rep"] = self._pack(w3, b3 + b1_)
        hp = "head.predictor"
        for i in range(3):
            cbn(f"{hp}.input_proj.{i}")
        P[f"{hp}.enc_output.0"] = self._pack_linear(sd[f"{hp}.enc_output.0.weight"], sd[f"{hp}.enc_output.0.bias"])
        ln(f"{hp}.enc_output.1")
        P[f"{hp}.enc_score"] = self._pack_linear(sd[f"{hp}.enc_score_classifier.weight"], sd[f"{hp}.enc_score_classifier.bias"])
        self.score_head = None
        ncp = (self.nc + 127) // 128 * 128
        if ncp <= 384:
            sw, sb = sd[f"{hp}.enc_score_classifier.weight"].float(), sd[f"{hp}.enc_score_classifier.bias"].float()
            w2 = sw.new_zeros(ncp, self.hd)
            w2[: self.nc] = sw
            b2 = sb.new_full((ncp,), -3e38)
            b2[: self.nc] = sb
            self.score_head = (self._pack_frag(sd[f"{hp}.enc_output.0.weight"].float()), self._dev(sd[f"{hp}.enc_output.0.bias"].float()),
                               self._pack_frag(w2), self._dev(b2), ncp)
        b0 = sd[f"{hp}.enc_output.0.bias"].float().cpu()
        row = torch.nn.functional.layer_norm(b0.to(torch.bfloat16).float(), (self.hd,), sd[f"{hp}.enc_output.1.weight"].float().cpu(),
                                             sd[f"{hp}.enc_output.1.bias"].float().cpu(), 1e-5)
        self.invalid_row = self._dev(row, torch.bfloat16)

        def mlp3(prefix, key):
            P[f"{key}.0"] = self._pack_linear(sd[f"{prefix}.layers.0.weight"], sd[f"{prefix}.layers.0.bias"])
            P[f"{key}.1"] = self._pack_linear(sd[f"{prefix}.layers.1.weight"], sd[f"{prefix}.layers.1.bias"])
            return self._dev(sd[f"{prefix}.layers.2.weight"].float()), self._dev(sd[f"{prefix}.layers.2.bias"].float())

        self.bbox_last: Dict[str, Tuple[torch.Tensor, torch.Tensor]] = {}
        self.bbox_last["enc"] = mlp3(f"{hp}.enc_bbox_classifier", f"{hp}.enc_bbox")
        self.qpos0 = (self._dev(sd[f"{hp}.query_pos_head.layers.0.weight"].float()), self._dev(sd[f"{hp}.query_pos_head.layers.0.bias"].float()))
        P[f"{hp}.qpos1"] = self._pack_linear(sd[f"{hp}.query_pos_head.layers.1.weight"], sd[f"{hp}.query_pos_head.layers.1.bias"])
        vw, vb = [], []
        for li in range(self.nl):
            p = f"{hp}.decoder.layers.{li}"
            Wi, bi_ = sd[f"{p}.self_attn.in_proj_weight"], sd[f"{p}.self_attn.in_proj_bias"]
            P[f"{p}.qk"] = self._pack_linear(Wi[:512], bi_[:512])
            P[f"{p}.v"] = self._pack_linear(Wi[512:], bi_[512:])
            P[f"{p}.out_proj"] = self._pack_linear(sd[f"{p}.self_attn.out_proj.weight"], sd[f"{p}.self_attn.out_proj.bias"])
            ca = f"{p}.cross_attn"
            P[f"{ca}.offaw"] = self._pack_linear(torch.cat([sd[f"{ca}.sampling_offsets.weight"], sd[f"{ca}.attention_weights.weight"]], 0),
                                                 torch.cat([sd[f"{ca}.sampling_offsets.bias"], sd[f"{ca}.attention_weights.bias"]], 0))
            vw.append(sd[f"{ca}.value_proj.weight"])
            vb.append(sd[f"{ca}.value_proj.bias"])
            P[f"{ca}.output_proj"] = self._pack_linear(sd[f"{ca}.output_proj.weight"], sd[f"{ca}.output_proj.bias"])
            for l in ("linear1", "linear2"):
                P[f"{p}.{l}"] = self._pack_linear(sd[f"{p}.{l}.weight"], sd[f"{p}.{l}.bias"])
            for nrm in ("norm1", "norm2", "norm3"):
                ln(f"{p}.{nrm}")
            self.bbox_last[f"dec{li}"] = mlp3(f"{hp}.dec_bbox_classifier.{li}", f"{hp}.dec_bbox.{li}")
        P[f"{hp}.value_all"] = self._pack_linear(torch.cat(vw, 0), torch.cat(vb, 0))
        last = self.nl - 1
        P[f"{hp}.dec_score"] = self._pack_linear(sd[f"{hp}.dec_score_classifier.{last}.weight"], sd[f"{hp}.dec_score_classifier.{last}.bias"])
        RC: Dict[str, Tuple[torch.Tensor, torch.Tensor]] = {}

        def rc(key, W, b, pad_to=None):
            W, b = W.float(), b.float()
            if pad_to is not None and W.shape[0] < pad_to:
                W = torch.cat([W, W.new_zeros(pad_to - W.shape[0], W.shape[1])], 0)
                b = torch.cat([b, b.new_zeros(pad_to - b.shape[0])], 0)
            RC[key] = (self._pack_frag(W), self._dev(b))

        rc("qpos1", sd[f"{hp}.query_pos_head.layers.1.weight"], sd[f"{hp}.query_pos_head.layers.1.bias"])
        for li in range(self.nl):
            p = f"{hp}.decoder.layers.{li}"
            Wi, bi_ = sd[f"{p}.self_attn.in_proj_weight"], sd[f"{p}.self_attn.in_proj_bias"]
            rc(f"{li}.qk", Wi[:512], bi_[:512])
            rc(f"{li}.v", Wi[512:], bi_[512:])
            rc(f"{li}.o", sd[f"{p}.self_attn.out_proj.weight"], sd[f"{p}.self_attn.out_proj.bias"])
            ca = f"{p}.cross_attn"
            rc(f"{li}.offaw", torch.cat([sd[f"{ca}.sampling_offsets.weight"], sd[f"{ca}.attention_weights.weight"]], 0),
               torch.cat([sd[f"{ca}.sampling_offsets.bias"], sd[f"{ca}.attention_weights.bias"]], 0))
            rc(f"{li}.o2", sd[f"{ca}.output_proj.weight"], sd[f"{ca}.output_proj.bias"])
            rc(f"{li}.f1", sd[f"{p}.linear1.weight"], sd[f"{p}.linear1.bias"])
            rc(f"{li}.f2", sd[f"{p}.linear2.weight"], sd[f"{p}.linear2.bias"])
            RC[f"{li}.ffn_b"] = (None, self._dev(torch.cat([sd[f"{p}.linear1.bias"].float(), sd[f"{p}.linear2.bias"].float()])))
            self.dec_ffn = int(sd[f"{p}.linear1.weight"].shape[0])
            bb = f"{hp}.dec_bbox_classifier.{li}"
            rc(f"{li}.bb0", sd[f"{bb}.layers.0.weight"], sd[f"{bb}.layers.0.bias"])
            rc(f"{li}.bb1", sd[f"{bb}.layers.1.weight"], sd[f"{bb}.layers.1.bias"])
        self.nc_pad32 = (self.nc + 31) // 32 * 32
        rc("score", sd[f"{hp}.dec_score_classifier.{last}.weight"], sd[f"{hp}.dec_score_classifier.{last}.bias"], pad_to=self.nc_pad32)
        self.RC = RC
        self.P = P

    @staticmethod
    def _pos_embed_sine(h: int, w: int, npf: int, temperature: float = 10000.0) -> torch.Tensor:
        ys = torch.arange(h, dtype=torch.float32).view(h, 1).expand(h, w)
        xs = torch.arange(w, dtype=torch.float32).view(1, w).expand(h, w)
        i = torch.arange(npf, dtype=torch.float32)
        dim_t = temperature ** (2 * torch.div(i, 2, rounding_mode="floor") / npf)
        px, py = xs[..., None] / dim_t, ys[..., None] / dim_t
        out = torch.cat([py[..., 0::2].sin(), py[..., 1::2].cos(), px[..., 0::2].sin(), px[..., 1::2].cos()], dim=-1)
        return out.reshape(h * w, 2 * npf)

    @staticmethod
    def _anchors(shapes: Sequence[Tuple[int, int]], grid_size: float = 0.05, eps: float = 1e-2):
        out = []
        for lvl, (h, w) in enumerate(shapes):
            gy, gx = torch.meshgrid(torch.arange(h, dtype=torch.float32), torch.arange(w, dtype=torch.float32), indexing="ij")
            xy = (torch.stack([gx, gy], -1) + 0.5) / torch.tensor([w, h], dtype=torch.float32)
            wh = torch.ones_like(xy) * grid_size * (2.0 ** (2 - lvl))
            out.append(torch.cat([xy, wh], -1).reshape(h * w, 4))
        a = torch.cat(out, 0)
        valid = ((a > eps) & (a < 1 - eps)).all(-1)
        a = torch.log(a / (1 - a))
        a = torch.where(valid[:, None], a, torch.zeros_like(a))
        return a, torch.nonzero(~valid).flatten().to(torch.int32)

    def plan(self, B: int, H: int, W: int, f32_input: bool = False, nsplit: Optional[int] = None):
        if nsplit is None:
            nsplit = int(os.environ.get("FX_STREAMS", str(DEFAULT_STREAMS)))
        if nsplit > 1 and not _lib.two_queue_safe():
            nsplit = 1
        while nsplit > 1 and (B % nsplit or B // nsplit < MIN_PART_BATCH):
            nsplit -= 1
        key = (B, H, W, f32_input, nsplit)
        if key not in self.plans:
            self.plans[key] = _Plan(self, B, H, W, f32_input) if nsplit <= 1 else _MultiPlan(self, _Plan, B, H, W, f32_input, nsplit)
        return self.plans[key]

    def pipeline(self, B: int, H: int, W: int, depth: Optional[int] = None, f32_input: bool = False, nsplit: int = 1) -> "_Pipeline":
        if depth is None:
            depth = int(os.environ.get("FX_PIPELINE_DEPTH", str(DEFAULT_PIPELINE_DEPTH)))
        if not _lib.two_queue_safe():
            depth, nsplit = 1, 1
        key = ("pipeline", B, H, W, f32_input, nsplit, depth)
        if key not in self.plans:
            self.plans[key] = _Pipeline(self, _Plan, B, H, W, f32_input, depth, nsplit)
        return self.plans[key]

    def forward(self, images: torch.Tensor, sizes: Optional[torch.Tensor] = None, threshold: Optional[float] = None,
                forced_topk: Optional[torch.Tensor] = None, use_graph: bool = True) -> "_Plan":
        assert images.dim() == 4 and images.shape[-1] == 3 and images.is_contiguous() and images.device == self.dev
        f32 = images.dtype == torch.float32
        assert f32 or images.dtype == torch.uint8
        B, H, W, _ = images.shape
        pl = self.plan(B, H, W, f32, 1 if (forced_topk is not None or not use_graph) else None)
        cur = torch.cuda.current_stream(self.dev)
        self.stream.wait_stream(cur)
        with torch.cuda.stream(self.stream):
            pl.input.copy_(images, non_blocking=True)
            if sizes is None:
                pl.sizes.copy_(torch.tensor([[H, W]] * B, dtype=torch.int32), non_blocking=False)
            else:
                pl.sizes.copy_(sizes.to(torch.int32), non_blocking=True)
            pl.run(self.stream.cuda_stream, threshold if threshold is not None else self.threshold, forced_topk, use_graph)
        cur.wait_stream(self.stream)
        return pl


class _PlanBase:

    size_multiple = 32
    needed_res = (2, 3, 4, 5)

    def __init__(self, eng: _EngineBase, B: int, H: int, W: int, f32_input: bool, parent: Optional["_MultiPlan"] = None, index: int = 0):
        if H % self.size_multiple or W % self.size_multiple or H < 32 or W < 32:
            raise _lib.FocoosAmdError(f"input height/width must be multiples of {self.size_multiple} (and at least 32)")
        self.eng, self.B, self.H, self.W, self.f32_input = eng, B, H, W, f32_input
        self.parent, self.index = parent, index
        self.lib = eng.lib
        self.dev = eng.dev
        self.ops: List[Tuple] = []
        self.split_at: Optional[int] = None
        self.keep: List = []
        self.meta: Dict[int, dict] = {}
        self.bufs: Dict[str, NT] = {}
        self._win = None
        self.graph = None
        self.graph_thr = None
        self._thr_cell = None
        self._build()

    def _new(self, name: str, B: int, H: int, W: int, Cc: int, dtype=torch.bfloat16) -> NT:
        if self._win is not None:
            b0, bs = self._win
            assert B == bs, (name, B, bs)
            full = self.bufs.get(name)
            if full is None:
                full = NT(torch.empty(self.B * H * W * Cc, dtype=dtype, device=self.dev), self.B, H, W, Cc, Cc, 0)
                self.bufs[name] = full
            return NT(full.t, bs, H, W, Cc, Cc, b0 * H * W * Cc)
        guard = int(os.environ.get("FX_GUARD", "0"))
        if guard:
            t = torch.empty(B * H * W * Cc + 2 * guard, dtype=dtype, device=self.dev)
            t.view(torch.uint8).fill_(0x5A)
            nt = NT(t, B, H, W, Cc, Cc, guard)
            self.guards = getattr(self, "guards", [])
            self.guards.append((name, t, guard))
        else:
            t = torch.empty(B * H * W * Cc, dtype=dtype, device=self.dev)
            nt = NT(t, B, H, W, Cc, Cc, 0)
        self.bufs[name] = nt
        return nt

    def check_guards(self):
        bad = []
        for name, t, g in getattr(self, "guards", []):
            u = t.view(torch.uint8)
            es = t.element_size()
            head, tail = u[: g * es], u[-g * es:]
            if not bool((head == 0x5A).all()) or not bool((tail == 0x5A).all()):
                bad.append((name, int((head != 0x5A).sum()), int((tail != 0x5A).sum())))
        return bad

    def _op(self, fn, *args):
        self.ops.append((fn, args))

    def _io(self, name: str, shape: Tuple[int, ...], dtype) -> torch.Tensor:
        if self.parent is not None:
            return self.parent.io_slice(name, shape, dtype, self.index)
        return torch.empty(*shape, dtype=dtype, device=self.dev)

    def conv(self, x: NT, pc: PackedConv, out: Optional[NT] = None, name: Optional[str] = None, stride: int = 1, act=None,
             residual: Optional[NT] = None, res_after: bool = False, pool2: bool = False, out_f32: bool = False,
             y_batch_stride: int = 0, extra_flops_per_pixel: float = 0.0) -> NT:
        assert x.C == pc.C, (name, x.C, pc.C)
        pad = (pc.KH - 1) // 2
        if pool2:
            Ho, Wo = (x.H + 1) // 2, (x.W + 1) // 2
        else:
            Ho, Wo = (x.H + 2 * pad - pc.KH) // stride + 1, (x.W + 2 * pad - pc.KW) // stride + 1
        if out is None:
            ncols = (pc.N + 7) // 8 * 8
            out = self._new(name, x.B, Ho, Wo, ncols, torch.float32 if out_f32 else torch.bfloat16)
            out.C = pc.N
        assert out.H == Ho and out.W == Wo and out.C == pc.N, (name, out.H, Ho, out.C, pc.N)
        d = FxConvDesc()
        d.x, d.w, d.bias = x.ptr, pc.w.data_ptr(), pc.b.data_ptr()
        d.residual = residual.ptr if residual is not None else None
        d.y = out.ptr
        d.B, d.H, d.W, d.C, d.ldx = x.B, x.H, x.W, x.C, x.ld
        d.Ho, d.Wo, d.N, d.ldy = Ho, Wo, pc.N, out.ld
        d.ldr = residual.ld if residual is not None else 0
        d.KH, d.KW, d.stride, d.pad = pc.KH, pc.KW, stride, pad
        d.pool2, d.act, d.out_f32 = int(pool2), FX_ACT[act], int(out_f32)
        d.residual_after_act = int(res_after)
        d.y_batch_stride = y_batch_stride
        d.w_frag = pc.wf.data_ptr() if pc.wf is not None else None
        self.keep.append(d)
        M = x.B * Ho * Wo
        flops = 2.0 * M * pc.N * pc.KH * pc.KW * pc.C + extra_flops_per_pixel * M
        label = C.create_string_buffer(64)
        check(self.lib.fx_conv2d_variant(C.byref(d), label, 64), "fx_conv2d_variant")
        variant = label.value.decode()
        alg_bytes = 2.0 * x.B * x.H * x.W * pc.C + (4.0 if out_f32 else 2.0) * M * pc.N + (2.0 * M * pc.N if residual is not None else 0.0) \
            + 2.0 * pc.N * pc.KH * pc.KW * pc.C
        self.meta[len(self.ops)] = {"kind": "conv", "variant": variant, "flops": flops, "flops_executed": flops - extra_flops_per_pixel * M, "bytes": alg_bytes,
                                    "name": name or "slice", "M": M, "N": pc.N, "K": pc.KH * pc.KW * pc.C}
        self._op(self.lib.fx_conv2d_nhwc_bf16, C.byref(d))
        return out

    def pw_chain(self, x1: NT, x2: Optional[NT], residual: Optional[NT], cc: Tuple, ca: Optional[Tuple], name1: str, name2: Optional[str],
                 pool_name: Optional[str] = None, keep_y1: bool = True):
        w1, b1, k1a, k1b, n1 = cc
        assert x1.C == k1a and (x2 is None) == (k1b == 0) and (x2 is None or x2.C == k1b), (name1, x1.C, k1a, k1b)
        M = x1.rows
        assert keep_y1 or (pool_name is not None and ca is not None)
        y1 = self._new(name1, x1.B, x1.H, x1.W, n1) if keep_y1 else None
        d = FxPwChainDesc()
        d.x1, d.ldx1, d.K1a = x1.ptr, x1.ld, k1a
        d.x2, d.ldx2, d.K1b = (x2.ptr, x2.ld, k1b) if x2 is not None else (None, 0, 0)
        d.residual, d.ldr = (residual.ptr, residual.ld) if residual is not None else (None, 0)
        d.w1, d.bias1, d.N1, d.M = w1.data_ptr(), b1.data_ptr(), n1, M
        d.y1, d.ldy1 = (y1.ptr, y1.ld) if y1 is not None else (None, 0)
        d.act1 = d.act2 = FX_ACT["relu"]
        y2, n2 = None, 0
        if ca is not None:
            w2, b2, n2 = ca
            y2 = self._new(name2, x1.B, x1.H, x1.W, n2)
            d.w2, d.bias2, d.y2, d.ldy2 = w2.data_ptr(), b2.data_ptr(), y2.ptr, y2.ld
        d.N2 = n2
        pooled = None
        if pool_name is not None:
            pooled = self._new(pool_name, x1.B, x1.H // 2, x1.W // 2, n1)
            d.pool, d.ldp, d.img_h, d.img_w = pooled.ptr, pooled.ld, x1.H, x1.W
        self.keep.append(d)
        self.meta[len(self.ops)] = {"kind": "conv", "variant": f"pw_chain<{k1a},{k1b},{n2}>" + ("+pool" if pooled is not None else "") + ("-y1" if y1 is None else ""),
                                    "flops": 2.0 * M * n1 * (k1a + k1b + n2),
                                    "name": name1 + ("+" + name2.rsplit("res_layers.", 1)[-1] if name2 else ""), "M": M, "N": n1, "K": k1a + k1b,
                                    "bytes": 2.0 * M * (k1a + k1b + (n1 if residual is not None else 0) + (n1 if y1 is not None else 0) + n2
                                                        + (n1 / 4 if pooled is not None else 0))}
        self._op(self.lib.fx_pw_chain_bf16, C.byref(d))
        if pool_name is not None:
            return y1, y2, pooled
        return y1, y2

    def linear(self, x: NT, pc: PackedConv, **kw) -> NT:
        return self.conv(x.as_rows() if (x.H != 1 or x.W != 1) else x, pc, **kw)

    def layernorm(self, x: NT, name_ln: str, out_name: str, residual: Optional[NT] = None) -> NT:
        g, b = self.eng.ln[name_ln]
        cols = int(g.numel())
        out = self._new(out_name, x.rows, 1, 1, cols)
        self._op(self.lib.fx_layernorm_bf16, x.ptr, x.ld, residual.ptr if residual is not None else None,
                 residual.ld if residual is not None else 0, g.data_ptr(), b.data_ptr(), out.ptr, out.ld, x.rows, cols)
        return out

    def add_rows(self, x: NT, y: NT, y_rows: int, out_name: str) -> NT:
        out = self._new(out_name, x.rows, 1, 1, x.C)
        self._op(self.lib.fx_add_rows_bf16, x.ptr, x.ld, y.ptr, y.ld, y_rows, out.ptr, out.ld, x.rows, x.C)
        return out

    RC_S0, RC_S1, RC_S2, RC_S3, RC_BIG, RC_REF, RC_RED, RC_LDS = 0, 16384, 32768, 49152, 65536, 131072, 131584, 132608
    RC2_REF, RC2_RED, RC2_LDS = 65536, 66048, 67072

    def _rc_program(self, stages: List[FxRcStage], rows: int, label: str, flops: float, lds: Optional[int] = None):
        arr = (FxRcStage * len(stages))(*stages)
        host = torch.frombuffer(bytearray(bytes(arr)), dtype=torch.uint8)
        dev = host.to(self.dev)
        self.keep.append(dev)
        self.meta[len(self.ops)] = {"kind": "conv", "variant": "row_chain", "flops": flops, "name": label, "M": rows, "N": 0, "K": 0}
        self._op(self.lib.fx_row_chain, dev.data_ptr(), len(stages), rows, self.RC_LDS if lds is None else lds)

    def resize(self, x: NT, out: NT):
        self._op(self.lib.fx_resize_bilinear_nhwc_bf16, x.ptr, x.ld, out.ptr, out.ld, x.B, x.H, x.W, x.C, out.H, out.W)

    def mha(self, qkv: NT, B: int, L: int, out_name: str) -> NT:
        out = self._new(out_name, B * L, 1, 1, 256)
        q, k, v = qkv.slice(0, 256), qkv.slice(256, 256), qkv.slice(512, 256)
        self._op(self.lib.fx_mha_bf16, q.ptr, q.ld, k.ptr, k.ld, v.ptr, v.ld, out.ptr, out.ld, B, L, L, 8)
        return out

    def build_backbone(self) -> Dict[int, NT]:
        e, P, B, lib = self.eng, self.eng.P, self.B, self.lib
        H, W = self.H, self.W
        bb = "pixel_decoder.backbone"
        self.input = self._io("input", (B, H, W, 3), torch.float32 if self.f32_input else torch.uint8)
        self.sizes = self._io("sizes", (B, 2), torch.int32)
        blocks = RESNET_BLOCKS[e.depth]
        feats = {}
        use_chain = int(os.environ.get("FX_PW_CHAIN", "1")) != 0
        max_stage = int(os.environ.get("FX_PW_CHAIN_MAX_STAGE", "1"))
        pc2 = P[f"{bb}.conv1.conv1_2"]
        if os.environ.get("FX_STEM12_FUSE", "1") != "0" and not self.f32_input and pc2.wf is not None and pc2.N == 32:
            x = self._new("conv1_2", B, (H + 1) // 2, (W + 1) // 2, 32)
            M2 = x.rows
            self.meta[len(self.ops)] = {"kind": "conv", "variant": "stem_c1+c2", "flops": 2.0 * M2 * 32 * (27 + 288), "flops_executed": 2.0 * M2 * 32 * (32 * 1.29 + 288),
                                        "bytes": 3.0 * B * H * W + 2.0 * M2 * 32 + 2.0 * 32 * 288, "name": "conv1_1+conv1_2", "M": M2, "N": 32, "K": 288}
            self._op(lib.fx_stem_conv12_u8_bf16, self.input.data_ptr(), e.stem_w.data_ptr(), e.stem_b.data_ptr(), e.px_mean.data_ptr(), e.px_inv_std.data_ptr(),
                     pc2.wf.data_ptr(), pc2.b.data_ptr(), x.ptr, x.ld, B, H, W)
        else:
            c1 = self._new("conv1_1", B, (H + 1) // 2, (W + 1) // 2, 32)
            self._op(lib.fx_stem_conv3x3s2, self.input.data_ptr(), int(self.f32_input), e.stem_w.data_ptr(), e.stem_b.data_ptr(),
                     e.px_mean.data_ptr(), e.px_inv_std.data_ptr(), c1.ptr, B, H, W, 32)
            x = self.conv(c1, pc2, name="conv1_2", act="relu")
        pc3 = P[f"{bb}.conv1.conv1_3"]
        if os.environ.get("FX_STEM_FUSE", "1") != "0" and pc3.wf is not None and lib.fx_stem_conv_pool_supported(x.C, pc3.N, x.H, x.W) == 1:
            mp = self._new("maxpool", B, (x.H + 1) // 2, (x.W + 1) // 2, 64)
            M3 = B * x.H * x.W
            self.meta[len(self.ops)] = {"kind": "conv", "variant": "stem_c3+pool", "flops": 2.0 * M3 * 64 * 288, "flops_executed": 2.0 * M3 * 64 * 288 * 1.37,
                                        "bytes": 2.0 * M3 * 32 + 2.0 * mp.rows * 64 + 2.0 * 64 * 288, "name": "conv1_3+maxpool", "M": M3, "N": 64, "K": 288}
            self._op(lib.fx_stem_conv3x3_relu_maxpool_bf16, x.ptr, x.ld, pc3.wf.data_ptr(), pc3.b.data_ptr(), mp.ptr, mp.ld, B, x.H, x.W)
        else:
            x = self.conv(x, pc3, name="conv1_3", act="relu")
            mp = self._new("maxpool", B, (x.H + 1) // 2, (x.W + 1) // 2, 64)
            self._op(lib.fx_maxpool3x3s2_nhwc_bf16, x.ptr, x.ld, mp.ptr, mp.ld, B, x.H, x.W, 64)
        x = mp
        seq = [(si, bi) for si in range(4) for bi in range(blocks[si])]
        a_next: Optional[NT] = None
        pooled_next: Optional[NT] = None
        use_pool = int(os.environ.get("FX_PW_CHAIN_POOL", "1")) != 0
        for idx, (si, bi) in enumerate(seq):
            p = f"{bb}.res_layers.{si}.blocks.{bi}"
            stride = 2 if (bi == 0 and si != 0) else 1
            a = a_next if a_next is not None else self.conv(x, P[f"{p}.branch2a"], name=f"{p}.a", act="relu")
            a_next = None
            bmid = self.conv(a, P[f"{p}.branch2b"], name=f"{p}.b", stride=stride, act="relu")
            short_in = None
            if bi == 0:
                short_in = x
                if stride == 2 and pooled_next is not None:
                    short_in, pooled_next = pooled_next, None
                elif stride == 2:
                    short_in = self._new(f"{p}.pool", x.B, (x.H + 1) // 2, (x.W + 1) // 2, x.C)
                    self._op(lib.fx_avgpool2x2_nhwc_bf16, x.ptr, x.ld, short_in.ptr, short_in.ld, x.B, x.H, x.W, x.C)
            nxt = seq[idx + 1] if idx + 1 < len(seq) else None
            cc = e.chain_c.get((si, bi)) if (use_chain and si <= max_stage) else None
            n2 = 0
            if cc is not None:
                ca = e.chain_a.get(nxt) if nxt is not None else None
                if ca is not None and lib.fx_pw_chain_supported(cc[2], cc[3], cc[4], ca[2]) == 1:
                    n2 = ca[2]
                elif lib.fx_pw_chain_supported(cc[2], cc[3], cc[4], 0) != 1:
                    cc = None
            if cc is not None:
                nxt_name = f"{bb}.res_layers.{nxt[0]}.blocks.{nxt[1]}.a" if n2 else None
                want_pool = (use_pool and nxt is not None and nxt[0] == si + 1 and bi != 0 and bmid.H % 2 == 0 and bmid.W % 2 == 0
                             and lib.fx_pw_chain_pool_supported(cc[2], cc[3], cc[4], n2) == 1)
                if want_pool:
                    keep = bool(n2 == 0 or (si + 2) in self.needed_res or os.environ.get("FX_SKIP_UNUSED_RES", "1") == "0")
                    x, a_next, pooled_next = self.pw_chain(bmid, short_in, x, cc, e.chain_a[nxt] if n2 else None, f"{p}.c", nxt_name,
                                                           pool_name=f"{bb}.res_layers.{nxt[0]}.blocks.0.pool", keep_y1=keep)
                else:
                    x, a_next = self.pw_chain(bmid, short_in, None if bi == 0 else x, cc, e.chain_a[nxt] if n2 else None, f"{p}.c", nxt_name)
            else:
                short = x if bi != 0 else self.conv(short_in, P[f"{p}.short" if si == 0 else f"{p}.short.conv"], name=f"{p}.s")
                x = self.conv(bmid, P[f"{p}.branch2c"], name=f"{p}.c", residual=short, act="relu")
            if bi == blocks[si] - 1:
                feats[si + 2] = x
        for k, v in feats.items():
            if v is not None:
                self.bufs[f"res{k}"] = v
        return feats

    def patch_args(self, fn, args, thr: float):
        return args

    def _launch(self, ops, stream: int, thr: float):
        for fn, args in ops:
            check(fn(*self.patch_args(fn, args, thr), C.c_void_p(stream)), fn.__name__)

    def capture_and_launch(self, stream: int, thr: float):
        if self.graph is None or self.graph_thr != thr:
            if self.graph is not None:
                check(self.lib.fx_graph_destroy(self.graph), "fx_graph_destroy")
                self.graph = None
            self._launch(self.ops, stream, thr)
            torch.cuda.current_stream(self.dev).synchronize()
            check(self.lib.fx_graph_begin(C.c_void_p(stream)), "fx_graph_begin")
            try:
                self._launch(self.ops, stream, thr)
            finally:
                g = C.c_void_p()
                rc = self.lib.fx_graph_end(C.c_void_p(stream), C.byref(g))
            check(rc, "fx_graph_end")
            self.graph, self.graph_thr = g, thr
        check(self.lib.fx_graph_launch(self.graph, C.c_void_p(stream)), "fx_graph_launch")

    def time_graph(self, stream: int, iters: int) -> float:
        ms = C.c_float(0)
        check(self.lib.fx_graph_time(self.graph, C.c_void_p(stream), iters, C.byref(ms)), "fx_graph_time")
        return ms.value

    def __del__(self):
        try:
            if self.graph is not None:
                self.lib.fx_graph_destroy(self.graph)
        except Exception:
            pass


class _Plan(StdcPlanMixin, _PlanBase):

    needed_res = (3, 4, 5)
    size_multiple = 1

    def _build(self):
        e, P, B, lib = self.eng, self.eng.P, self.B, self.lib
        H, W = self.H, self.W
        feats = self.build_stdc() if e.stdc else self.build_backbone()
        fd = e.fd
        pd = "pixel_decoder"
        (h8, w8), (h16, w16), (h32, w32) = ((feats[k].H, feats[k].W) for k in (3, 4, 5))
        if h8 * w8 + h16 * w16 + h32 * w32 < e.nq:
            raise _lib.FocoosAmdError(f"input {H}x{W} gives {h8 * w8 + h16 * w16 + h32 * w32} encoder tokens, fewer than the {e.nq} queries to select")
        cat80 = self._new("cat80", B, h8, w8, 2 * fd)
        cat40a = self._new("cat40a", B, h16, w16, 2 * fd)
        cat40b = self._new("cat40b", B, h16, w16, 2 * fd)
        cat20 = self._new("cat20", B, h32, w32, 2 * fd)
        self.conv(feats[3], P[f"{pd}.input_proj.0"], out=cat80.slice(fd, fd))
        self.conv(feats[4], P[f"{pd}.input_proj.1"], out=cat40a.slice(fd, fd))
        src = self.conv(feats[5], P[f"{pd}.input_proj.2"], name="proj5")
        L = h32 * w32
        if e.n_enc > 0:
            pos = e._pos_embed_sine(h32, w32, 128).to(device=self.dev, dtype=torch.bfloat16).contiguous()
            self.pos = NT(pos, L, 1, 1, 256, 256)
            s = src.as_rows()
            for li in range(e.n_enc):
                p = f"{pd}.encoder.0.layers.{li}"
                qk_in = self.add_rows(s, self.pos, L, f"aifi{li}.qk_in")
                qkv = self._new(f"aifi{li}.qkv", B * L, 1, 1, 768)
                self.linear(qk_in, P[f"{p}.qk"], out=qkv.slice(0, 512))
                self.linear(s, P[f"{p}.v"], out=qkv.slice(512, 256))
                att = self.mha(qkv, B, L, f"aifi{li}.att")
                o = self.linear(att, P[f"{p}.out_proj"], name=f"aifi{li}.o", residual=s)
                s1 = self.layernorm(o, f"{p}.norm1", f"aifi{li}.s1")
                f1 = self.linear(s1, P[f"{p}.linear1"], name=f"aifi{li}.f1", act="gelu")
                f2 = self.linear(f1, P[f"{p}.linear2"], name=f"aifi{li}.f2", residual=s1)
                s = self.layernorm(f2, f"{p}.norm2", f"aifi{li}.s2")
            self.bufs["aifi"] = s
            src = NT(s.t, B, h32, w32, 256, 256, s.off)

        def csp(xin: NT, p: str, out_name: str) -> NT:
            c12 = self.conv(xin, P[f"{p}.conv12"], name=f"{p}.c12", act="silu")
            x1 = c12.slice(0, fd)
            for j in range(3):
                last = j == 2
                x1 = self.conv(x1, P[f"{p}.bottlenecks.{j}.rep"], name=out_name if last else f"{p}.rep{j}", act="silu",
                               residual=c12.slice(fd, fd) if last else None, res_after=True,
                               extra_flops_per_pixel=2.0 * fd * fd)
            return x1

        lat0 = self.conv(src, P[f"{pd}.lateral_convs.0"], out=cat20.slice(fd, fd), act="silu")
        self.resize(lat0, cat40a.slice(0, fd))
        fpn0 = csp(cat40a, f"{pd}.fpn_blocks.0", "fpn0")
        lat1 = self.conv(fpn0, P[f"{pd}.lateral_convs.1"], out=cat40b.slice(fd, fd), act="silu")
        self.resize(lat1, cat80.slice(0, fd))
        out80 = csp(cat80, f"{pd}.fpn_blocks.1", "enc_s8")
        d0 = self._new("down0", B, h16, w16, fd)
        self.resize(out80, d0)
        self.conv(d0, P[f"{pd}.downsample_convs.0"], out=cat40b.slice(0, fd), act="silu")
        out40 = csp(cat40b, f"{pd}.pan_blocks.0", "enc_s16")
        d1 = self._new("down1", B, h32, w32, fd)
        self.resize(out40, d1)
        self.conv(d1, P[f"{pd}.downsample_convs.1"], out=cat20.slice(0, fd), act="silu")
        out20 = csp(cat20, f"{pd}.pan_blocks.1", "enc_s32")
        hp = "head.predictor"
        shapes = [(h32, w32), (h16, w16), (h8, w8)]
        S = sum(a * b for a, b in shapes)
        self.S = S
        starts = [0, shapes[0][0] * shapes[0][1], shapes[0][0] * shapes[0][1] + shapes[1][0] * shapes[1][1]]
        memory = self._new("memory", B, S, 1, 256)
        for i, (f, st) in enumerate(zip((out20, out40, out80), starts)):
            lvl = NT(memory.t, B, f.H, f.W, 256, 256, memory.off + st * 256)
            self.conv(f, P[f"{hp}.input_proj.{i}"], out=lvl, y_batch_stride=S * 256)
        mem_rows = memory.as_rows()
        anchors, invalid = e._anchors(shapes)
        self.anchors = anchors.to(self.dev).contiguous()
        self.invalid = invalid.to(self.dev).contiguous()
        self.shapes_t = torch.tensor(shapes, dtype=torch.int32, device=self.dev)
        self.starts_t = torch.tensor(starts, dtype=torch.int32, device=self.dev)
        Q, K = e.nq, e.nc
        self.enc_scores = self._io("enc_scores", (B, S), torch.float32)
        if e.score_head is not None and int(os.environ.get("FX_SCORE_HEAD", "1")) != 0:
            w1, b1, w2, b2, ncp = e.score_head
            valid = torch.ones(S, dtype=torch.uint8)
            valid[invalid.long()] = 0
            self.valid_u8 = valid.to(self.dev)
            om = self._new("output_memory", B * S, 1, 1, 256)
            g_, b_ = e.ln[f"{hp}.enc_output.1"]
            self.meta[len(self.ops)] = {"kind": "conv", "variant": f"score_head<{ncp}>", "flops": 2.0 * B * S * 256 * (256 + K), "name": "enc_output+enc_score+max",
                                        "M": B * S, "N": 256 + K, "K": 256, "bytes": 2.0 * B * S * 256 * 2 + 4.0 * B * S}
            self._op(lib.fx_enc_score_head_bf16, mem_rows.ptr, mem_rows.ld, self.valid_u8.data_ptr(), S, w1.data_ptr(), b1.data_ptr(), g_.data_ptr(),
                     b_.data_ptr(), C.c_float(1e-5), w2.data_ptr(), b2.data_ptr(), ncp, om.ptr, om.ld, self.enc_scores.data_ptr(), B * S)
        else:
            om_lin = self.linear(mem_rows, P[f"{hp}.enc_output.0"], name="om_lin")
            om = self.layernorm(om_lin, f"{hp}.enc_output.1", "output_memory")
            self._op(lib.fx_fill_rows_bf16, om.ptr, om.ld, S, self.invalid.data_ptr(), int(self.invalid.numel()), e.invalid_row.data_ptr(), B, 256)
            enc_logits = self.linear(om, P[f"{hp}.enc_score"], name="enc_logits", out_f32=True)
            self._op(lib.fx_rowmax_f32, enc_logits.ptr, enc_logits.ld, self.enc_scores.data_ptr(), B * S, K)
        self.enc_topk_val = self._io("enc_topk_val", (B, Q), torch.float32)
        self.enc_topk = self._io("enc_topk", (B, Q), torch.int32)
        self._op(lib.fx_topk_rows_f32, self.enc_scores.data_ptr(), S, B, S, Q, self.enc_topk_val.data_ptr(), self.enc_topk.data_ptr())
        self.split_at = len(self.ops)
        R = B * Q
        tgt = self._new("target", R, 1, 1, 256)
        self._op(lib.fx_gather_rows_bf16, om.ptr, om.ld, S, self.enc_topk.data_ptr(), Q, tgt.ptr, tgt.ld, B, 256)
        hb = self.linear(tgt, P[f"{hp}.enc_bbox.0"], name="encbb.0", act="relu")
        hb = self.linear(hb, P[f"{hp}.enc_bbox.1"], name="encbb.1", act="relu")
        self.ref_unact = torch.empty(R, 4, dtype=torch.float32, device=self.dev)
        refs = [torch.empty(R, 4, dtype=torch.float32, device=self.dev) for _ in range(e.nl + 1)]
        wl, bl = e.bbox_last["enc"]
        self._op(lib.fx_bbox_head, hb.ptr, hb.ld, wl.data_ptr(), bl.data_ptr(), None, self.anchors.data_ptr(), self.enc_topk.data_ptr(), Q, 1,
                 refs[0].data_ptr(), self.ref_unact.data_ptr(), R, 256)
        value = self.linear(mem_rows, P[f"{hp}.value_all"], name="value_all")
        if int(os.environ.get("FX_ROW_CHAIN", "1")) != 0 and e.hd == 256:
            logits = self._build_decoder_row_chain(tgt, refs, value, R, B, Q, S)
        else:
            logits = self._build_decoder_per_op(tgt, refs, value, R, B, Q, S)
        self.refs = refs
        self.probs = self._io("probs", (B, Q, K), torch.float32)
        self.boxes = self._io("boxes", (B, Q, 4), torch.float32)
        self._op(lib.fx_detr_head_out, logits.ptr, logits.ld, refs[e.nl].data_ptr(), self.probs.data_ptr(), self.boxes.data_ptr(), R, K)
        tk = min(e.top_k, Q * K)
        self.top_k = tk
        self.det_scores = self._io("det_scores", (B, tk), torch.float32)
        self.det_flat = self._io("det_flat", (B, tk), torch.int32)
        self.det_labels = self._io("det_labels", (B, tk), torch.int32)
        self.det_queries = self._io("det_queries", (B, tk), torch.int32)
        self.det_boxes = self._io("det_boxes", (B, tk, 4), torch.int32)
        self.det_count = self._io("det_count", (B,), torch.int32)
        nws = int(lib.fx_topk_rows_workspace_bytes(B, Q * K, tk))
        self.topk_ws = torch.empty(max(nws, 8), dtype=torch.uint8, device=self.dev)
        self.keep.append(self.topk_ws)
        self._op(lib.fx_topk_rows_ws_f32, self.probs.data_ptr(), Q * K, B, Q * K, tk, self.det_scores.data_ptr(), self.det_flat.data_ptr(),
                 self.topk_ws.data_ptr(), C.c_size_t(self.topk_ws.numel()))
        self.post_index = len(self.ops)
        self._op(lib.fx_detr_postprocess, self.det_scores.data_ptr(), self.det_flat.data_ptr(), self.boxes.data_ptr(), self.sizes.data_ptr(), B, Q,
                 K, tk, None, self.det_labels.data_ptr(), self.det_queries.data_ptr(), self.det_boxes.data_ptr(), self.det_count.data_ptr())

    def _build_decoder_per_op(self, tgt: NT, refs, value: NT, R: int, B: int, Q: int, S: int) -> NT:
        e, P, lib = self.eng, self.eng.P, self.lib
        hp = "head.predictor"
        qp1 = self._new("qpos_h", R, 1, 1, 512)
        for li in range(e.nl):
            p = f"{hp}.decoder.layers.{li}"
            ref = refs[li]
            self._op(lib.fx_linear_k4_relu, ref.data_ptr(), e.qpos0[0].data_ptr(), e.qpos0[1].data_ptr(), qp1.ptr, qp1.ld, R, 512)
            qpos = self.linear(qp1, P[f"{hp}.qpos1"], name=f"dec{li}.qpos")
            qk_in = self.add_rows(tgt, qpos, R, f"dec{li}.qk_in")
            qkv = self._new(f"dec{li}.qkv", R, 1, 1, 768)
            self.linear(qk_in, P[f"{p}.qk"], out=qkv.slice(0, 512))
            self.linear(tgt, P[f"{p}.v"], out=qkv.slice(512, 256))
            att = self.mha(qkv, B, Q, f"dec{li}.att")
            o = self.linear(att, P[f"{p}.out_proj"], name=f"dec{li}.o", residual=tgt)
            t1 = self.layernorm(o, f"{p}.norm1", f"dec{li}.t1")
            q2 = self.add_rows(t1, qpos, R, f"dec{li}.q2")
            offaw = self.linear(q2, P[f"{p}.cross_attn.offaw"], name=f"dec{li}.offaw", out_f32=True)
            ms = self._new(f"dec{li}.msda", R, 1, 1, 256)
            vsl = value.slice(li * 256, 256)
            self._op(lib.fx_msda_bf16, vsl.ptr, vsl.ld, self.shapes_t.data_ptr(), self.starts_t.data_ptr(), 3, 4, offaw.ptr, offaw.ld,
                     offaw.ptr + 192 * 4, offaw.ld, ref.data_ptr(), 1, ms.ptr, ms.ld, B, S, Q, 8)
            o2 = self.linear(ms, P[f"{p}.cross_attn.output_proj"], name=f"dec{li}.o2", residual=t1)
            t2 = self.layernorm(o2, f"{p}.norm2", f"dec{li}.t2")
            f1 = self.linear(t2, P[f"{p}.linear1"], name=f"dec{li}.f1", act="relu")
            f2 = self.linear(f1, P[f"{p}.linear2"], name=f"dec{li}.f2", residual=t2)
            tgt = self.layernorm(f2, f"{p}.norm3", f"dec{li}.out")
            hb = self.linear(tgt, P[f"{hp}.dec_bbox.{li}.0"], name=f"dec{li}.bb0", act="relu")
            hb = self.linear(hb, P[f"{hp}.dec_bbox.{li}.1"], name=f"dec{li}.bb1", act="relu")
            wl, bl = e.bbox_last[f"dec{li}"]
            self._op(lib.fx_bbox_head, hb.ptr, hb.ld, wl.data_ptr(), bl.data_ptr(), ref.data_ptr(), None, None, Q, 0, refs[li + 1].data_ptr(),
                     None, R, 256)
        logits = self.linear(tgt, P[f"{hp}.dec_score"], name="logits", out_f32=True)
        return logits

    def _build_decoder_row_chain(self, tgt: NT, refs, value: NT, R: int, B: int, Q: int, S: int) -> NT:
        e, lib = self.eng, self.lib
        RC = e.RC
        S0, S1, S2, S3, BIG, REF, RED = self.RC_S0, self.RC_S1, self.RC_S2, self.RC_S3, self.RC_BIG, self.RC_REF, self.RC_RED
        relu = FX_ACT["relu"]

        def st(type_, K=0, N=0, act=0, src=-1, dst=-1, aux=-1, ld=0, ld2=0, flags=0, w=None, bias=None, gamma=None, beta=None, g0=None, g1=None):
            s_ = FxRcStage()
            s_.type, s_.K, s_.N, s_.act, s_.src, s_.dst, s_.aux, s_.ld, s_.ld2, s_.flags = type_, K, N, act, src, dst, aux, ld, ld2, flags
            s_.w, s_.bias, s_.gamma, s_.beta, s_.g0, s_.g1 = w, bias, gamma, beta, g0, g1
            return s_

        def load(nt: NT, dst):
            return st(0, K=nt.C, dst=dst, g0=nt.ptr, ld=nt.ld)

        def gemm(key, src, K, N, dst=-1, act=0, out: Optional[NT] = None, f32=False):
            w, b = RC[key]
            return st(1, K=K, N=N, act=act, src=src, dst=dst, w=w.data_ptr(), bias=b.data_ptr(), g0=out.ptr if out is not None else None,
                      ld=out.ld if out is not None else 0, flags=int(f32))

        def gemm_ln(key, src, K, aux, ln_name, dst, out: Optional[NT] = None):
            w, b = RC[key]
            g_, b_ = e.ln[ln_name]
            return st(2, K=K, N=256, src=src, dst=dst, aux=aux, w=w.data_ptr(), bias=b.data_ptr(), gamma=g_.data_ptr(), beta=b_.data_ptr(),
                      g0=out.ptr if out is not None else None, ld=out.ld if out is not None else 0, ld2=RED)

        hp = "head.predictor"
        qkv = self._new("dec.qkv", R, 1, 1, 768)
        qpos = self._new("dec.qpos", R, 1, 1, 256)
        t1 = self._new("dec.t1", R, 1, 1, 256)
        offaw = self._new("dec.offaw", R, 1, 1, 288, torch.float32)
        ncp = e.nc_pad32
        logits = self._new("logits", R, 1, 1, ncp, torch.float32)
        logits.C = e.nc

        hidden = int(e.dec_ffn)
        lean = os.environ.get("FX_RC_LEAN", "1") != "0" and hidden % 256 == 0 and hidden <= 2048
        if lean:
            REF, RED = self.RC2_REF, self.RC2_RED
        lds = self.RC2_LDS if lean else None

        def gemm_ln(key, src, K, aux, ln_name, dst, out: Optional[NT] = None):
            w, b = RC[key]
            g_, b_ = e.ln[ln_name]
            return st(2, K=K, N=256, src=src, dst=dst, aux=aux, w=w.data_ptr(), bias=b.data_ptr(), gamma=g_.data_ptr(), beta=b_.data_ptr(),
                      g0=out.ptr if out is not None else None, ld=out.ld if out is not None else 0, ld2=RED)

        def ffn_ln(li, src, res, slot_a, slot_b, ln_name, dst, out: Optional[NT] = None):
            g_, b_ = e.ln[ln_name]
            return st(7, K=256, N=hidden, act=slot_a, flags=slot_b, src=src, aux=res, dst=dst, w=RC[f"{li}.f1"][0].data_ptr(), g1=RC[f"{li}.f2"][0].data_ptr(),
                      bias=RC[f"{li}.ffn_b"][1].data_ptr(), gamma=g_.data_ptr(), beta=b_.data_ptr(), g0=out.ptr if out is not None else None,
                      ld=out.ld if out is not None else 0, ld2=RED)

        def pre_attention(li, tgt_slot, ref_global=None):
            if lean:
                assert tgt_slot == S3
                k4 = st(4, N=512, dst=S0, ld2=S1, flags=4, aux=(-1 if ref_global is not None else REF), w=e.qpos0[0].data_ptr(), bias=e.qpos0[1].data_ptr(),
                        g0=ref_global)
                w, b = RC["qpos1"]
                q1 = st(1, K=512, N=256, src=S0, aux=S1, dst=S2, flags=4, w=w.data_ptr(), bias=b.data_ptr(), g0=qpos.ptr, ld=qpos.ld)
                return [k4, q1, st(3, K=256, src=S3, aux=S2, dst=S0), gemm(f"{li}.qk", S0, 256, 512, out=qkv.slice(0, 512)),
                        gemm(f"{li}.v", S3, 256, 256, out=qkv.slice(512, 256))]
            k4 = st(4, N=512, dst=BIG, aux=(-1 if ref_global is not None else REF), w=e.qpos0[0].data_ptr(), bias=e.qpos0[1].data_ptr(), g0=ref_global)
            return [k4, gemm("qpos1", BIG, 512, 256, dst=S1, out=qpos), st(3, K=256, src=tgt_slot, aux=S1, dst=S2),
                    gemm(f"{li}.qk", S2, 256, 512, out=qkv.slice(0, 512)), gemm(f"{li}.v", tgt_slot, 256, 256, out=qkv.slice(512, 256))]

        fl_pre = 2.0 * R * (512 * 256 + 256 * 768)
        first_slot = S3 if lean else S0
        self._rc_program([load(tgt, first_slot)] + pre_attention(0, first_slot, refs[0].data_ptr()), R, "dec0.pre", fl_pre, lds)
        for li in range(e.nl):
            p = f"{hp}.decoder.layers.{li}"
            att = self.mha(qkv, B, Q, f"dec{li}.att")
            prog = [load(att, S0), load(tgt, S1), load(qpos, S2), gemm_ln(f"{li}.o", S0, 256, S1, f"{p}.norm1", S3, out=t1),
                    st(3, K=256, src=S3, aux=S2, dst=S0), gemm(f"{li}.offaw", S0, 256, 288, out=offaw, f32=True)]
            self._rc_program(prog, R, f"dec{li}.post_attn", 2.0 * R * 256 * (256 + 288), lds)
            ms = self._new(f"dec{li}.msda", R, 1, 1, 256)
            vsl = value.slice(li * 256, 256)
            self._op(lib.fx_msda_bf16, vsl.ptr, vsl.ld, self.shapes_t.data_ptr(), self.starts_t.data_ptr(), 3, 4, offaw.ptr, offaw.ld,
                     offaw.ptr + 192 * 4, offaw.ld, refs[li].data_ptr(), 1, ms.ptr, ms.ld, B, S, Q, 8)
            out = self._new(f"dec{li}.out", R, 1, 1, 256)
            wl, bl = e.bbox_last[f"dec{li}"]
            last = li == e.nl - 1
            if lean:
                ffn = [ffn_ln(li, S2, S2, S0, S1, f"{p}.norm3", S3, out=out)]
            else:
                ffn = [gemm(f"{li}.f1", S2, 256, 1024, dst=BIG, act=relu), gemm_ln(f"{li}.f2", BIG, 1024, S2, f"{p}.norm3", S3, out=out)]
            prog = [load(ms, S0), load(t1, S1), gemm_ln(f"{li}.o2", S0, 256, S1, f"{p}.norm2", S2)] + ffn + [
                    gemm(f"{li}.bb0", S3, 256, 256, dst=S0, act=relu), gemm(f"{li}.bb1", S0, 256, 256, dst=S1, act=relu),
                    st(5, K=256, src=S1, aux=(-1 if last else REF), w=wl.data_ptr(), bias=bl.data_ptr(), g0=refs[li].data_ptr(), g1=refs[li + 1].data_ptr())]
            fl = 2.0 * R * (256 * 256 * 3 + 2 * 256 * 1024)
            if last:
                prog.append(gemm("score", S3, 256, ncp, out=logits, f32=True))
                fl += 2.0 * R * 256 * e.nc
            else:
                prog += pre_attention(li + 1, S3)
                fl += fl_pre
            self._rc_program(prog, R, f"dec{li}.post_msda", fl, lds)
            tgt = out
        return logits

    def patch_args(self, fn, args, thr: float):
        if fn is self.lib.fx_detr_postprocess:
            return args[:8] + (C.c_float(thr),) + args[9:]
        return args

    def run(self, stream: int, thr: float, forced_topk: Optional[torch.Tensor] = None, use_graph: bool = True):
        if forced_topk is not None:
            self._launch(self.ops[: self.split_at], stream, thr)
            self.enc_topk.copy_(forced_topk.to(device=self.dev, dtype=torch.int32))
            self._launch(self.ops[self.split_at:], stream, thr)
            return
        if not use_graph:
            self._launch(self.ops, stream, thr)
            return
        self.capture_and_launch(stream, thr)


class _Pipeline:

    def __init__(self, eng: _EngineBase, plan_cls, B: int, H: int, W: int, f32_input: bool, depth: int, nsplit: int = 1, **kw):
        self.eng, self.B, self.H, self.W, self.depth, self.nsplit = eng, B, H, W, max(1, depth), nsplit
        self.dev = eng.dev
        self.lanes = []
        lane_streams = _concurrent_streams(self.dev, self.depth) if nsplit <= 1 else None
        for j in range(self.depth):
            if nsplit > 1:
                pl = _MultiPlan(eng, plan_cls, B, H, W, f32_input, nsplit, stream_offset=nsplit * j, **kw)
                st = eng.stream if j == 0 else _device_stream(self.dev, nsplit * j)
            else:
                pl = plan_cls(eng, B, H, W, f32_input, **kw)
                st = lane_streams[j]
            self.lanes.append((pl, st))
        self.tickets = 0
        self._events = [None] * self.depth

    def lane(self, ticket: int):
        return self.lanes[ticket % self.depth]

    def submit(self, images: torch.Tensor, sizes: Optional[torch.Tensor] = None, threshold: Optional[float] = None, host: Optional[dict] = None) -> int:
        t = self.tickets
        self.tickets += 1
        pl, st = self.lanes[t % self.depth]
        st.wait_stream(torch.cuda.current_stream(self.dev))
        with torch.cuda.stream(st):
            pl.input.copy_(images, non_blocking=True)
            if sizes is None:
                pl.sizes.copy_(torch.tensor([[self.H, self.W]] * self.B, dtype=torch.int32), non_blocking=False)
            else:
# ... 131 lines not shown
```

include/focoos_amd.h:

```cpp
#ifndef FOCOOS_AMD_H
#define FOCOOS_AMD_H

#include <stddef.h>
#include <stdint.h>

#ifdef __cplusplus
extern "C" {
#endif

#define FX_ABI_VERSION 17

enum { FX_OK = 0, FX_ERR_INVALID_ARGUMENT = -1, FX_ERR_LAUNCH = -2, FX_ERR_UNSUPPORTED = -3, FX_ERR_RUNTIME = -4 };
enum { FX_ACT_NONE = 0, FX_ACT_RELU = 1, FX_ACT_SILU = 2, FX_ACT_GELU = 3 };
enum { FX_CLASS_LOSS_CE = 0, FX_CLASS_LOSS_FOCAL = 1, FX_CLASS_LOSS_BCE = 2, FX_CLASS_LOSS_BCE_FOCAL = 3 };

typedef void* fx_stream_t;

int fx_abi_version(void);
int fx_build_flags(void);
const char* fx_error_string(int code);
int fx_device_info(int device, int* cu_count, char* arch_name, int arch_name_len);

typedef struct fx_conv_desc {
  const void* x;
  const void* w;
  const float* bias;
  const void* residual;
  void* y;
  int32_t B, H, W, C, ldx;
  int32_t Ho, Wo, N, ldy, ldr;
  int32_t KH, KW, stride, pad;
  int32_t pool2;
  int32_t act;
  int32_t out_f32;
  int32_t residual_after_act;
  int64_t y_batch_stride;
  const void* w_frag;
  const void* mask;
  int32_t ldm, reserved0;
} fx_conv_desc;
int fx_conv2d_nhwc_bf16(const fx_conv_desc* d, fx_stream_t stream);
int fx_conv2d_variant(const fx_conv_desc* d, char* out, int cap);
int fx_conv3x3_flat_supported(int C, int N, int W);

typedef struct fx_pw_chain_desc {
  const void* x1;
  const void* x2;
  const void* residual;
  const void* w1;
  const float* bias1;
  void* y1;
  const void* w2;
  const float* bias2;
  void* y2;
  int32_t M, K1a, K1b, N1, N2;
  int32_t ldx1, ldx2, ldr, ldy1, ldy2;
  int32_t act1, act2;
  void* pool;
  int32_t ldp, img_h, img_w, reserved0;
} fx_pw_chain_desc;
int fx_pw_chain_supported(int K1a, int K1b, int N1, int N2);
int fx_pw_chain_pool_supported(int K1a, int K1b, int N1, int N2);
int fx_pw_chain_bf16(const fx_pw_chain_desc* d, fx_stream_t stream);

int fx_stem_conv3x3s2(const void* x, int in_f32, const float* w, const float* bias, const float* mean,
                      const float* inv_std, void* y, int B, int H, int W, int Cout, fx_stream_t stream);

int fx_stem_conv12_u8_bf16(const void* x_u8, const float* w1, const float* b1, const float* mean, const float* inv_std, const void* w2_frag,
                           const float* b2, void* y, int ldy, int B, int H, int W, fx_stream_t stream);

int fx_stem16_conv3x3s2(const void* x, int in_f32, const float* w, const float* bias, const float* mean, const float* inv_std, void* y, int B,
                        int H, int W, fx_stream_t stream);
int fx_conv3x3_c16_nhwc_bf16(const void* x, int ldx, const void* w_frag, const float* bias, int relu, void* y, int ldy, int B, int H, int W, int C,
                             int N, int stride, fx_stream_t stream);

int fx_semseg_eval_accumulate(const float* mask_probs, const float* probs, int B, int Q, int K, int h, int w, int Hin, int Win, const int32_t* sizes,
                              int64_t max_pixels, const void* gt, const int64_t* gt_off, int gt_int32, int ignore_label, int64_t* conf,
                              int32_t* status, int32_t* pred, float* score, fx_stream_t stream);

int fx_detr_eval_boxes_f32(const int32_t* idx, const float* boxes, const int32_t* sizes, int B, int Q, int K, int T,
                           int32_t* label, float* xyxy, int32_t* keep, float* xywh, fx_stream_t stream);

size_t fx_coco_match_workspace_bytes(int max_gt);
int fx_coco_match_bbox(const int32_t* label, const float* score, const int32_t* keep, const float* xywh, int B, int T, int K,
                       const double* gt_box, const int32_t* gt_cat, const int32_t* gt_flag, const double* gt_area, const int64_t* gt_off,
                       const int64_t* gt_off_host, int64_t n_gt, int max_gt, int32_t* rank, uint64_t* matched, uint64_t* ignored,
                       int64_t* npig, int32_t* status, void* ws, size_t ws_bytes, fx_stream_t stream);

size_t fx_mf_eval_masks_workspace_bytes(int B, int Q, int max_h);
int fx_mf_eval_masks(const float* mask_probs, const float* val, const int32_t* idx, int B, int Q, int K, int T, int h, int w, int Hin, int Win,
                     const int32_t* sizes, const int32_t* sizes_host, const int64_t* word_off, const int64_t* word_off_host, int64_t n_words,
                     float mask_threshold, void* words, int32_t* qlist, int32_t* nref, int32_t* count, int32_t* box, float* psum, int32_t* label,
                     int32_t* query, float* score, void* ws, size_t ws_bytes, fx_stream_t stream);
int fx_coco_mask_inter(const void* words, const int64_t* word_off, const int64_t* word_off_host, int64_t n_words, const int32_t* qlist,
                       const int32_t* nref, const int32_t* box, int B, int Q, int T, const int32_t* sizes, const int32_t* sizes_host,
                       const void* gt_words, const int64_t* gt_word_off, const int64_t* gt_word_off_host, int64_t n_gt_words,
                       const int32_t* gt_box, const int64_t* gt_off, const int64_t* gt_off_host, int64_t n_gt, int32_t* inter, int32_t* gcount,
                       fx_stream_t stream);
int fx_coco_match_segm(const int32_t* label, const float* score, const int32_t* query, const int32_t* dcount, int B, int T, int K, int Q,
                       const int32_t* inter, const int32_t* gcount, const int32_t* gt_cat, const int32_t* gt_flag, const double* gt_area,
                       const int64_t* gt_off, const int64_t* gt_off_host, int64_t n_gt, int max_gt, int32_t* rank, uint64_t* matched,
                       uint64_t* ignored, int64_t* npig, int32_t* status, void* ws, size_t ws_bytes, fx_stream_t stream);

typedef struct fx_aug_record {
  int32_t crop_w, crop_h, pad_x, pad_y, res_w, res_h, crop_x, crop_y, flags, reserved0;
  float brightness, contrast, saturation;
  int32_t reserved1[3];
} fx_aug_record;

int fx_augment_images_u8(const uint8_t* src, const int64_t* src_off, const int32_t* sizes, const fx_aug_record* recs, const int64_t* src_off_host,
                         int64_t src_bytes, const int32_t* sizes_host, const fx_aug_record* recs_host, int B, uint8_t* dst, int Ho, int Wo,
                         int pad_value, uint64_t* mean_ws, fx_stream_t stream);

int fx_augment_labels(const void* src, const int64_t* src_off, const int32_t* plane_rec, const int32_t* sizes, const fx_aug_record* recs,
                      const int64_t* src_off_host, int64_t src_count, const int32_t* plane_rec_host, const int32_t* sizes_host,
                      const fx_aug_record* recs_host, int P, int B, void* dst, int Ho, int Wo, int elem_int32, int pad_value, int32_t* flags,
                      fx_stream_t stream);

int fx_resize_bilinear_u8(const uint8_t* x, int H, int W, float* y, int Ho, int Wo, fx_stream_t stream);

int fx_tile_gather_u8_f32(const uint8_t* frame, int H, int W, const int32_t* windows, const int32_t* windows_host, int N, float* y, int Ho, int Wo,
                          fx_stream_t stream);

#define FX_MERGE_NMS_CAP 4096
enum { FX_MERGE_IOU = 0, FX_MERGE_IOS = 1 };
size_t fx_merge_detections_workspace_bytes(int N, int T);
int fx_merge_detections_nms(const float* det_scores, const int32_t* det_labels, const int32_t* det_boxes, const int32_t* det_count,
                            const int32_t* windows, int N, int T, int frame_h, int frame_w, float merge_threshold, int metric, int max_detections,
                            float* out_scores, int32_t* out_labels, int32_t* out_boxes, int32_t* out_count, int32_t* status, void* workspace,
                            size_t workspace_bytes, fx_stream_t stream);

#define FX_ANN_LNAME 24
#define FX_ANN_LMAX 32
#define FX_ANN_GLYPHS 95
#define FX_ANN_MAX_DIM 16384
enum { FX_ANN_BOXES = 1, FX_ANN_MASKS = 2, FX_ANN_LABELS = 4 };
typedef struct fx_annotate_record {
  int32_t x0, y0, w, h;
  uint32_t colour;
  int32_t nchar;
  uint8_t glyph[FX_ANN_LMAX];
} fx_annotate_record;

int fx_annotate_labels_from_detections(const float* scores, const int32_t* labels, const int32_t* boxes, const int32_t* count, int B, int T,
                                       const uint8_t* name_glyphs, const int32_t* name_len, int K, int H, int W, int s, int gw, int gh,
                                       fx_annotate_record* rec, fx_stream_t stream);

int fx_annotate_u8(const uint8_t* src, uint8_t* dst, int B, int H, int W, int b0, int T, const int32_t* det_count, const int32_t* det_labels,
                   const int32_t* det_boxes, const int32_t* det_area, const int32_t* mask_words, int words_per_row, int64_t plane_stride_words,
                   const fx_annotate_record* rec, const uint32_t* atlas, int gw, int gh, int s, int flags, fx_stream_t stream);

int fx_maxpool3x3s2_nhwc_bf16(const void* x, int ldx, void* y, int ldy, int B, int H, int W, int C, fx_stream_t stream);
int fx_stem_conv_pool_supported(int C, int N, int H, int W);
int fx_stem_conv3x3_relu_maxpool_bf16(const void* x, int ldx, const void* w_frag, const float* bias, void* y, int ldy, int B, int H, int W,
                                      fx_stream_t stream);

int fx_avgpool2x2_nhwc_bf16(const void* x, int ldx, void* y, int ldy, int B, int H, int W, int C, fx_stream_t stream);

int fx_resize_bilinear_nhwc_bf16(const void* x, int ldx, void* y, int ldy, int B, int H, int W, int C, int Ho, int Wo,
                                 fx_stream_t stream);

int fx_add_rows_bf16(const void* x, int ldx, const void* y, int ldy_, int y_rows, void* out, int ldo, int rows, int cols,
                     fx_stream_t stream);

int fx_layernorm_bf16(const void* x, int ldx, const void* residual, int ldr, const float* gamma, const float* beta, void* out,
                      int ldo, int rows, int cols, fx_stream_t stream);

int fx_mha_bf16(const void* q, int ldq, const void* k, int ldk, const void* v, int ldv, void* out, int ldo, int B, int Lq, int Lk,
                int heads, fx_stream_t stream);

int fx_msda_bf16(const void* value, int ldv, const int32_t* spatial_shapes, const int32_t* level_start, int L, int P,
                 const float* loc, int ld_loc, const float* attn, int ld_attn, const float* ref, int mode, void* out, int ldo,
                 int B, int S, int Q, int M, fx_stream_t stream);

int fx_rowmax_f32(const float* x, int ldx, float* out, int rows, int cols, fx_stream_t stream);

int fx_enc_score_head_bf16(const void* memory, int ldm, const uint8_t* valid, int S, const void* w1, const float* b1,
                           const float* gamma, const float* beta, float eps, const void* w2, const float* b2, int n2_pad,
                           void* output_memory, int ldo, float* scores, int M, fx_stream_t stream);

typedef struct fx_rc_stage {
  int32_t type, K, N, act;
  int32_t src, dst, aux;
  int32_t ld, ld2, flags;
  const void* w;
  const float* bias;
  const float* gamma;
  const float* beta;
  void* g0;
  void* g1;
} fx_rc_stage;
int fx_row_chain(const fx_rc_stage* program_device, int n_stages, int rows, int lds_bytes, fx_stream_t stream);

int fx_topk_rows_f32(const float* scores, int ld, int B, int n, int k, float* out_val, int32_t* out_idx, fx_stream_t stream);
size_t fx_topk_rows_workspace_bytes(int B, int n, int k);
int fx_topk_rows_ws_f32(const float* scores, int ld, int B, int n, int k, float* out_val, int32_t* out_idx, void* workspace, size_t workspace_bytes,
                        fx_stream_t stream);

int fx_gather_rows_bf16(const void* src, int lds, int rows_per_batch, const int32_t* idx, int k, void* out, int ldo, int B, int cols,
                        fx_stream_t stream);

int fx_fill_rows_bf16(void* x, int ldx, int rows_per_batch, const int32_t* rows_idx, int n_idx, const void* row_bf16, int B, int cols,
                      fx_stream_t stream);

int fx_linear_k4_relu(const float* ref, const float* w, const float* b, void* out, int ldo, int rows, int N, fx_stream_t stream);

int fx_bbox_head(const void* h, int ldh, const float* w, const float* b, const float* ref, const float* anchors, const int32_t* idx,
                 int rows_per_batch, int mode, float* new_ref, float* unact_out, int rows, int K, fx_stream_t stream);

int fx_detr_head_out(const float* logits, int ldl, const float* ref_cxcywh, float* probs, float* boxes_xyxy, int rows, int K,
                     fx_stream_t stream);

int fx_detr_postprocess(const float* topk_val, const int32_t* topk_idx, const float* boxes_xyxy, const int32_t* sizes, int B, int Q,
                        int K, int top_k, float threshold, int32_t* labels, int32_t* queries, int32_t* boxes_i32, int32_t* count,
                        fx_stream_t stream);

int fx_mha_workspace_bytes(int B, int Lq, int Lk, int heads, int masked);
int fx_mha_masked_bf16(const void* q, int ldq, const void* k, int ldk, const void* v, int ldv, void* out, int ldo, int B, int Lq, int Lk,
                       int heads, const uint32_t* mask_bits, int ld_mask_words, void* workspace, size_t workspace_bytes, fx_stream_t stream);

int fx_upsample_nearest_add_nhwc_bf16(const void* lateral, int ldl, const void* top, int ldt, void* out, int ldo, int B, int H, int W,
                                      int Hs, int Ws, int C, fx_stream_t stream);
int fx_upsample_nearest_bwd_nhwc_bf16(const void* dy, int lddy, void* dtop, int lddt, int B, int H, int W, int Hs, int Ws, int C,
                                      fx_stream_t stream);

int fx_query_pixel_logits_bf16(const void* embed, int lde, const void* feat, int ldf, int mode, float* out, int ldo, uint32_t* bits,
                               int ld_words, int B, int Q, int P, int C, fx_stream_t stream);

int fx_mf_class_head(const float* logits, int ldl, float* probs, float* score, int32_t* label, int rows, int K, int use_sigmoid,
                     fx_stream_t stream);

int fx_mf_upsample_probs_f32(const float* lowres, int h, int w, float* out, int H, int W, int BQ, fx_stream_t stream);
int fx_mf_upsample_probs_bf16(const float* lowres, int h, int w, void* out, int H, int W, int BQ, fx_stream_t stream);

int fx_mf_postprocess_workspace_bytes(int B, int Q, int H);
size_t fx_mf_postprocess_workspace_bytes_fused(int B, int Q, int h, int w, int H, int W);
int fx_mf_postprocess(const float* mask_probs_lowres, int h, int w, int H, int W, const float* score, const int32_t* label, int B, int Q,
                      float mask_threshold, float threshold, int use_mask_score, void* workspace, size_t workspace_bytes,
                      int32_t* det_count, int32_t* det_query, float* det_score, int32_t* det_label, int32_t* det_box, int32_t* det_area,
                      uint32_t* mask_words, fx_stream_t stream);

int fx_point_sample_f32(const void* src, int src_is_u8, int H, int W, const int32_t* src_index, const float* coords, const int32_t* coord_index,
                        float* out, int R, int P, fx_stream_t stream);

int fx_mask_match_cost_f32(const float* logits, int ldl, const float* pred_pts, const float* tgt_pts, const int32_t* tgt_labels,
                           const int32_t* tgt_offsets, int B, int Q, int K, int P, int Tmax, float w_class, float w_mask, float w_dice,
                           int cls_sigmoid, float* cost, fx_stream_t stream);
size_t fx_mask_match_cost_workspace_bytes(int B, int Q, int Tmax);
int fx_mask_match_cost_ws_f32(const float* logits, int ldl, const float* pred_pts, const float* tgt_pts, const int32_t* tgt_labels,
                              const int32_t* tgt_offsets, int B, int Q, int K, int P, int Tmax, float w_class, float w_mask, float w_dice,
                              int cls_sigmoid, float* cost, void* workspace, size_t workspace_bytes, fx_stream_t stream);

size_t fx_mask_set_loss_workspace_bytes(int B, int Q, int sum_T, int n_over);
int fx_mask_set_loss_f32(const float* logits, int ldl, const float* pred_masks, int h, int w, const void* tgt_masks, int tgt_is_u8, int H, int W,
                         const int32_t* tgt_labels, const int32_t* tgt_offsets, int sum_T, const int32_t* pred_idx, const int32_t* tgt_idx,
                         const float* rand_over, int n_over, const float* rand_extra, int n_extra, int num_points, int B, int Q, int K,
                         float eos_coef, float num_masks, float w_ce, float w_mask, float w_dice, void* workspace, size_t workspace_bytes,
                         float* out3, fx_stream_t stream);
int fx_mask_set_loss_cls_f32(const float* logits, int ldl, const float* pred_masks, int h, int w, const void* tgt_masks, int tgt_is_u8, int H, int W,
                             const int32_t* tgt_labels, const int32_t* tgt_offsets, int sum_T, const int32_t* pred_idx, const int32_t* tgt_idx,
                             const float* rand_over, int n_over, const float* rand_extra, int n_extra, int num_points, int B, int Q, int K,
                             float eos_coef, int cls_mode, float focal_alpha, float focal_gamma, float num_masks, float w_ce, float w_mask,
                             float w_dice, void* workspace, size_t workspace_bytes, float* out3, fx_stream_t stream);
size_t fx_mask_class_loss_workspace_bytes(int B, int Q);
int fx_mask_class_loss_f32(const float* logits, int ldl, const int32_t* tgt_labels, const int32_t* tgt_offsets, const int32_t* pred_idx,
                           const int32_t* tgt_idx, int B, int Q, int K, int mode, float focal_alpha, float focal_gamma, float num_masks, float w_ce,
                           void* workspace, size_t workspace_bytes, float* out1, fx_stream_t stream);
int fx_mask_class_loss_bwd_f32(const float* logits, int ldl, const int32_t* tgt_labels, const int32_t* tgt_offsets, const int32_t* pred_idx,
                               const int32_t* tgt_idx, int B, int Q, int K, int mode, float focal_alpha, float focal_gamma, float num_masks,
                               float w_ce, const float* grad1, float* dlogits, int lddl, fx_stream_t stream);

int fx_dwconv3x3s2_nhwc_bf16(const void* x, int ldx, const float* w, const float* bias, void* y, int ldy, int B, int H, int W, int C,
                             fx_stream_t stream);
int fx_dwconv3x3s2_nhwc_f32out(const void* x, int ldx, const float* w, const float* bias, float* y, int ldy, int B, int H, int W, int C,
                               fx_stream_t stream);

int fx_global_mean_nhwc_bf16(const void* x, int ldx, float* out, int ldo, int B, int P, int C, fx_stream_t stream);

int fx_pooled_linear_f32(const float* in, int ldi, const float* W, const float* bias, int act, float* out, int ldo, int B, int C, int N,
                         fx_stream_t stream);

int fx_channel_gate_nhwc_bf16(const void* x, int ldx, const float* gate, int ldg, int self_add, const float* add_vec, int ldv,
                              const void* add_map, int ldm, void* y, int ldy, int B, int P, int C, fx_stream_t stream);

size_t fx_seg_postprocess_workspace_bytes(int B, int Q, int h, int w, int H, int W);
int fx_seg_postprocess(const float* mask_probs_lowres, int h, int w, int H, int W, const float* score, const int32_t* label, int B, int Q,
                       float threshold, int use_mask_score, void* workspace, size_t workspace_bytes, int32_t* det_count, int32_t* det_query,
                       float* det_score, int32_t* det_label, int32_t* det_box, int32_t* det_area, uint32_t* mask_words, uint8_t* winner_out,
                       fx_stream_t stream);

int fx_detr_match_cost_f32(const float* logits, int ldl, const float* boxes, const int32_t* tgt_labels, const float* tgt_boxes,
                           const int32_t* tgt_offsets, int B, int Q, int K, int Tmax, float w_class, float w_bbox, float w_giou, float alpha,
                           float gamma, float* cost, fx_stream_t stream);

int fx_lsa_f32(const float* cost, int B, int Q, int Tmax, const int32_t* tgt_offsets, int32_t* pred_idx, int32_t* tgt_idx, fx_stream_t stream);
int fx_lsa_status_f32(const float* cost, int B, int Q, int Tmax, const int32_t* tgt_offsets, int32_t* pred_idx, int32_t* tgt_idx, int32_t* status,
                      fx_stream_t stream);

int fx_detr_set_loss_workspace_bytes(int B, int Q, int sum_T);
int fx_detr_set_loss_f32(const float* logits, int ldl, const float* boxes, const int32_t* tgt_labels, const float* tgt_boxes,
                         const int32_t* tgt_offsets, const int32_t* pred_idx, const int32_t* tgt_idx, int B, int Q, int K, int sum_T,
                         float num_boxes, float focal_alpha, float focal_gamma, float w_vfl, float w_bbox, float w_giou, void* workspace,
                         float* out3, fx_stream_t stream);

int fx_detr_box_loss_f32(const float* boxes, const int32_t* tgt_labels, const float* tgt_boxes, const int32_t* tgt_offsets,
                         const int32_t* pred_idx, const int32_t* tgt_idx, int B, int Q, int K, int sum_T, float scale_bbox, float scale_giou,
                         int32_t* q_cls, float* q_score, float* loss2, float* pair_grad, fx_stream_t stream);
int fx_detr_box_loss_bwd_f32(const float* pair_grad, const int32_t* tgt_offsets, const int32_t* pred_idx, int B, int Q, int sum_T,
                             const float* g_bbox, const float* g_giou, float* dboxes, fx_stream_t stream);

int fx_msda_f32_fwd(const float* value, const int32_t* spatial_shapes, const int32_t* level_start, int L, int P, const float* loc,
                    const float* attn, float* out, int B, int S, int Q, int M, fx_stream_t stream);
int fx_msda_f32_bwd(const float* value, const int32_t* spatial_shapes, const int32_t* level_start, int L, int P, const float* loc,
                    const float* attn, const float* grad_out, float* grad_value, float* grad_loc, float* grad_attn, int B, int S, int Q, int M,
                    fx_stream_t stream);
int fx_msda_train_fwd(const void* value, int value_bf16, int ldv, const int32_t* spatial_shapes, const int32_t* level_start, int L, int P,
                      const float* loc, const float* attn, float* out, int B, int S, int Q, int M, fx_stream_t stream);
int fx_msda_train_bwd(const void* value, int value_bf16, int ldv, const int32_t* spatial_shapes, const int32_t* level_start, int L, int P,
                      const float* loc, const float* attn, const float* grad_out, float* grad_value, int ldg, int zero_grad_value,
                      float* grad_loc, float* grad_attn, int B, int S, int Q, int M, fx_stream_t stream);
int fx_msda_bwd_slab_supported(const int32_t* shapes_host, int L, int P, int Q, int M, int grad_out_bf16);
int fx_msda_train_bwd_slab(const void* value, int value_bf16, int ldv, const int32_t* spatial_shapes, const int32_t* level_start,
                           const int32_t* shapes_host, int L, int P, const float* loc, const float* attn, const void* grad_out,
                           int grad_out_bf16, void* grad_value_bf16, int ldg, float* grad_loc, float* grad_attn, int B, int S, int Q, int M,
                           fx_stream_t stream);

int fx_msda_prep_bf16(const void* off, int ld_off, const void* logit, int ld_logit, const float* ref, float* loc, float* aw, int BQ, int M, int L,
                      int P, fx_stream_t stream);
int fx_msda_prep_bwd_bf16(const float* grad_loc, const float* grad_attn, const float* aw, const float* ref, void* grad_off, int ld_off,
                          void* grad_logit, int ld_logit, int BQ, int M, int L, int P, fx_stream_t stream);

int fx_adamw_workspace_bytes(void);
int fx_adamw_step_f32(float* params, const float* grads, float* exp_avg, float* exp_avg_sq, int64_t numel, const int64_t* chunk_start,
                      const int32_t* chunk_len, const float* chunk_lr, const float* chunk_wd, int nchunks, int step, float beta1, float beta2,
                      float eps, float max_grad_norm, void* workspace, float* total_norm_out, fx_stream_t stream);

typedef struct fx_loss_scale_state {
  float scale;
  int32_t growth_tracker;
  int32_t good_steps;
  int32_t skipped_steps;
} fx_loss_scale_state;
int fx_adamw_step_scaled_f32(float* params, const float* grads, float* exp_avg, float* exp_avg_sq, int64_t numel, const int64_t* chunk_start,
                             const int32_t* chunk_len, const float* chunk_lr, const float* chunk_wd, int nchunks, float beta1, float beta2, float eps,
                             float max_grad_norm, void* workspace, float* total_norm_out, fx_loss_scale_state* state, float growth_factor,
                             float backoff_factor, int growth_interval, fx_stream_t stream);

int fx_conv2d_wgrad_nhwc_bf16(const void* x, int ldx, const void* dz, int lddz, float* dw, int B, int H, int W, int C, int Ho, int Wo, int N,
                              int KH, int KW, int stride, int pad, fx_stream_t stream);
int fx_conv2d_wgrad_bias_nhwc_bf16(const void* x, int ldx, const void* dz, int lddz, float* dw, float* dbias, int B, int H, int W, int C, int Ho,
                                   int Wo, int N, int KH, int KW, int stride, int pad, fx_stream_t stream);

int fx_pack_conv_weights_f32(const float* w, const float* scale, void* w_fwd, void* w_dgrad, void* w_fwd_frag, void* w_dgrad_frag, int N, int C,
                             int KH, int KW, fx_stream_t stream);

int fx_pack_frag_bf16(const void* w_rows, void* frag, int rows, int K, fx_stream_t stream);

int fx_pack_linear_weights_f32(const float* w, const float* bias, void* w_fwd, void* w_t, float* bias_out, int N, int K, int Np, int Kp,
                               fx_stream_t stream);

typedef struct {
  const float* w;
  const float* scale;
  const float* bias;
  void* w_fwd;
// ... 135 lines not shown
```

Baseline: 5047 images/s.

## Fuse stride-8 input projection into backbone pw-chain and add GELU kplane path

Measured after the change: 5025 images/s. Within noise of the previous version (-0.4%).

```diff
diff --git a/focoos_amd/_lib.py b/focoos_amd/_lib.py
--- a/focoos_amd/_lib.py
+++ b/focoos_amd/_lib.py
@@ -66,7 +66,8 @@
         ("M", C.c_int32), ("K1a", C.c_int32), ("K1b", C.c_int32), ("N1", C.c_int32), ("N2", C.c_int32),
         ("ldx1", C.c_int32), ("ldx2", C.c_int32), ("ldr", C.c_int32), ("ldy1", C.c_int32), ("ldy2", C.c_int32),
         ("act1", C.c_int32), ("act2", C.c_int32),
-        ("pool", C.c_void_p), ("ldp", C.c_int32), ("img_h", C.c_int32), ("img_w", C.c_int32), ("reserved0", C.c_int32),
+        ("pool", C.c_void_p), ("ldp", C.c_int32), ("img_h", C.c_int32), ("img_w", C.c_int32), ("N3", C.c_int32),
+        ("w3", C.c_void_p), ("bias3", C.c_void_p), ("y3", C.c_void_p), ("ldy3", C.c_int32), ("act3", C.c_int32),
     ]
 
 
@@ -89,6 +90,7 @@
     "fx_conv2d_variant": [_vp, C.c_char_p, _i],
     "fx_pw_chain_supported": [_i, _i, _i, _i],
     "fx_pw_chain_pool_supported": [_i, _i, _i, _i],
+    "fx_pw_chain_proj_supported": [_i, _i, _i, _i, _i],
     "fx_conv3x3_flat_supported": [_i, _i, _i],
     "fx_pw_chain_bf16": [C.POINTER(FxPwChainDesc), _vp],
     "fx_stem_conv3x3s2": [_vp, _i, _vp, _vp, _vp, _vp, _vp, _i, _i, _i, _i, _vp],
@@ -281,7 +283,7 @@
     return os.environ.get("FOCOOS_AMD_LIB", LIB_PATH)
 
 
-FX_ABI_VERSION = 17
+FX_ABI_VERSION = 18
 
 
 def load(name: str = None) -> C.CDLL:
diff --git a/focoos_amd/csrc/conv3x3_flat.hip b/focoos_amd/csrc/conv3x3_flat.hip
--- a/focoos_amd/csrc/conv3x3_flat.hip
+++ b/focoos_amd/csrc/conv3x3_flat.hip
@@ -272,7 +272,7 @@
 }
 
 int fx_c3_epilogue_mode(int act, bool has_res, int res_after) {
-  if (!has_res) return act == FX_ACT_RELU ? 0 : (act == FX_ACT_SILU ? 1 : (act == FX_ACT_NONE ? 3 : -1));
+  if (!has_res) return act == FX_ACT_RELU ? 0 : (act == FX_ACT_SILU ? 1 : (act == FX_ACT_NONE ? 3 : (act == FX_ACT_GELU ? 7 : -1)));
   if (act == FX_ACT_SILU && res_after == 1) return 2;
   if (act == FX_ACT_RELU && res_after == 0) return 4;
   if (act == FX_ACT_NONE && res_after == 2) return 5;
diff --git a/focoos_amd/csrc/conv_igemm.hip b/focoos_amd/csrc/conv_igemm.hip
--- a/focoos_amd/csrc/conv_igemm.hip
+++ b/focoos_amd/csrc/conv_igemm.hip
@@ -354,6 +354,10 @@
   if (frag && pw_on && d->stride == 1 && d->KH == 1 && d->KW == 1 && d->pad == 0 && d->C % 256 == 0 && d->N % 256 == 0 && a.M >= pw_min_m &&
       (mode == 0 || mode == 1 || (mode >= 3 && mode <= 6)))
     return (pwk_on && fx_pw_kplane_supported(d->C, d->N, mode)) ? R_PWK : R_PW_FLAT;
+  static const int pwk_gelu = fx_tune("FX_PW_KPLANE_GELU", 1);
+  if (frag && pw_on && pwk_on && pwk_gelu && mode == 7 && d->stride == 1 && d->KH == 1 && d->KW == 1 && d->pad == 0 && a.M >= pw_min_m &&
+      fx_pw_kplane_supported(d->C, d->N, mode))
+    return R_PWK;
   static const int s2_on = fx_tune("FX_C3S2_KPLANE", 1);
   if (frag && s2_on && d->stride == 2 && d->KH == 3 && d->KW == 3 && d->pad == 1 && !d->residual && d->H == 2 * d->Ho && d->W == 2 * d->Wo &&
       a.M >= c3_min_m && (mode == 0 || mode == 1 || mode == 3) && fx_conv3x3s2_kplane_supported(d->C, d->N, d->Wo, a.M))
diff --git a/focoos_amd/csrc/conv_pw_chain.hip b/focoos_amd/csrc/conv_pw_chain.hip
--- a/focoos_amd/csrc/conv_pw_chain.hip
+++ b/focoos_amd/csrc/conv_pw_chain.hip
@@ -10,8 +10,11 @@
   const float* b2;
   bf16_t* y1;
   bf16_t* y2;
-  int ldx1, ldx2, ldr, ldy1, ldy2;
-  int M, N1, act1, act2;
+  const bf16_t* w3p;
+  const float* b3;
+  bf16_t* y3;
+  int ldx1, ldx2, ldr, ldy1, ldy2, ldy3;
+  int M, N1, act1, act2, act3;
   unsigned x1_bytes, x2_bytes, r_bytes;
   bf16_t* pool;
   int ldp, H, W;
@@ -30,7 +33,7 @@
   }
 }
 
-template <int K1A, int K1B, int N2, int BM, bool QUAD = false>
+template <int K1A, int K1B, int N2, int BM, bool QUAD = false, int N3 = 0>
 __global__ __launch_bounds__(256, ((N2 <= 64 && K1B == 0) ? 4 : ((N2 <= 128 && (K1B == 0 || N2 <= 64)) ? 3 : 2))) void pw_chain_kernel(const PwChainArgs p) {
   constexpr int K1 = K1A + K1B, KS1 = K1 / 16, KS1A = K1A / 16;
   constexpr int RLA = K1A / 8, RLB = (K1B > 0 ? K1B : 64) / 8;
@@ -42,6 +45,8 @@
   constexpr int TN2 = !HAS2 ? 1 : N2 / (32 * WN2), TM2 = BM / (32 * WM2);
   constexpr int RL2 = (HAS2 ? N2 : 64) / 8;
   constexpr int PF2 = 4;
+  constexpr bool HAS3 = N3 > 0;
+  static_assert(!HAS3 || (N3 == 256 && N2 == 256), "the third output shares GEMM2's wave layout");
   static_assert(BM == 64, "64-pixel tiles");
   static_assert(K1A % 64 == 0 && K1B % 64 == 0 && PF1 == 4, "K segments in multiples of 64 (= whole blocks of 4 k-steps)");
   static_assert(!HAS2 || (N2 % 64 == 0 && N2 <= 256), "N2");
@@ -96,6 +101,19 @@
     for (int b = 0; b < TM2; ++b)
 #pragma unroll
       for (int r = 0; r < 16; ++r) acc2[a][b][r] = 0.0f;
+  f32x16 acc3[HAS3 ? TN2 : 1][HAS3 ? TM2 : 1];
+  if constexpr (HAS3) {
+#pragma unroll
+    for (int a = 0; a < TN2; ++a)
+#pragma unroll
+      for (int gq = 0; gq < 4; ++gq) {
+        const float4 bb = *reinterpret_cast<const float4*>(p.b3 + (wn2 * TN2 + a) * 32 + 8 * gq + 4 * half);
+#pragma unroll
+        for (int b = 0; b < TM2; ++b) {
+          acc3[a][b][4 * gq] = bb.x; acc3[a][b][4 * gq + 1] = bb.y; acc3[a][b][4 * gq + 2] = bb.z; acc3[a][b][4 * gq + 3] = bb.w;
+        }
+      }
+  }
 
   for (int g = 0; g < NG; ++g) {
     int l32g = l32, halfg = half, tidg = tid;
@@ -103,12 +121,14 @@
     if (p.res) pw_dma_rows_map<32>(rr, T, BM, p.ldr, g * 256, wave, lane, pix);
     bf16x8 a2[PF2][TN2];
     const bf16_t* w2 = p.w2p + (size_t)((wn2 * TN2) * KS2 + g * 16) * 512 + lane * 8;
-    if constexpr (HAS2) {
+    const bf16_t* w3 = HAS3 ? p.w3p + (size_t)((wn2 * TN2) * KS2 + g * 16) * 512 + lane * 8 : nullptr;
+    auto a2_prefetch = [&]() {
 #pragma unroll
       for (int i = 0; i < PF2; ++i)
 #pragma unroll
         for (int a = 0; a < TN2; ++a) a2[i][a] = pw_ldg_frag(w2 + (size_t)(a * KS2 + i) * 512);
-    }
+    };
+    if constexpr (HAS2 && !HAS3) a2_prefetch();
 #pragma unroll
     for (int a = 0; a < 2; ++a) {
       const bf16_t* w1 = p.w1p + (size_t)((g * 8 + wave * 2 + a) * KS1) * 512 + lane * 8;
@@ -174,6 +194,7 @@
           *reinterpret_cast<uint2*>(tp) = o;
         }
     }
+    if constexpr (HAS3) a2_prefetch();
     __syncthreads();
 #pragma unroll
     for (int i = 0; i < BM * 32 / 256; ++i) {
@@ -203,7 +224,7 @@
         if (q * 4 < p.M) *reinterpret_cast<uint4*>(p.pool + (size_t)q * p.ldp + g * 256 + lc * 8) = pack_bf16x8(s8);
       }
     }
-    if constexpr (HAS2) {
+    if constexpr (HAS2 && !HAS3) {
 #pragma unroll
       for (int ks = 0; ks < 16; ++ks) {
         bf16x8 tb[TM2];
@@ -220,6 +241,34 @@
 #pragma unroll
           for (int a = 0; a < TN2; ++a) a2[ks % PF2][a] = pw_ldg_frag(w2 + (size_t)(a * KS2 + ks + PF2) * 512);
         }
+      }
+    }
+    if constexpr (HAS3) {
+      bf16x8 tb[2][TM2];
+      auto tb_read = [&](int ks, bf16x8* dst) {
+#pragma unroll
+        for (int b = 0; b < TM2; ++b) {
+          const int row = (wm2 * TM2 + b) * 32 + l32g;
+          dst[b] = *reinterpret_cast<const bf16x8*>(T + row * 512 + (((ks * 2 + halfg) ^ (row & 15)) << 4));
+        }
+      };
+      tb_read(0, tb[0]);
+#pragma unroll
+      for (int ks = 0; ks < 32; ++ks) {
+        if (ks + 1 < 32) tb_read((ks + 1) & 15, tb[(ks + 1) & 1]);
+#pragma unroll
+        for (int a = 0; a < TN2; ++a)
+#pragma unroll
+          for (int b = 0; b < TM2; ++b) {
+            if (ks < 16) acc2[a][b] = FX_MFMA_32x32x16(a2[ks % PF2][a], tb[ks & 1][b], acc2[a][b]);
+            else acc3[a][b] = FX_MFMA_32x32x16(a2[ks % PF2][a], tb[ks & 1][b], acc3[a][b]);
+          }
+        if (ks + PF2 < 32) {
+          const bf16_t* wn = ks + PF2 < 16 ? w2 + (size_t)(ks + PF2) * 512 : w3 + (size_t)(ks + PF2 - 16) * 512;
+#pragma unroll
+          for (int a = 0; a < TN2; ++a) a2[ks % PF2][a] = pw_ldg_frag(wn + (size_t)(a * KS2) * 512);
+        }
+        __builtin_amdgcn_sched_barrier(0);
       }
     }
     __syncthreads();
@@ -256,14 +305,45 @@
       if (m >= 0) *reinterpret_cast<uint4*>(p.y2 + (size_t)m * p.ldy2 + lc * 8) = v;
     }
   }
-}
-
-template <int K1A, int K1B, int N2, bool QUAD = false>
+  if constexpr (HAS3) {
+    constexpr int RL3 = N3 / 8;
+    __syncthreads();
+#pragma unroll
+    for (int a = 0; a < TN2; ++a)
+#pragma unroll
+      for (int gq = 0; gq < 4; ++gq) {
+        const int n = (wn2 * TN2 + a) * 32 + 8 * gq + 4 * half;
+#pragma unroll
+        for (int b = 0; b < TM2; ++b) {
+          const int row = (wm2 * TM2 + b) * 32 + l32;
+          float v0 = acc3[a][b][4 * gq], v1 = acc3[a][b][4 * gq + 1], v2 = acc3[a][b][4 * gq + 2], v3 = acc3[a][b][4 * gq + 3];
+          if (p.act3 == FX_ACT_RELU) {
+            v0 = fmaxf(v0, 0.0f); v1 = fmaxf(v1, 0.0f); v2 = fmaxf(v2, 0.0f); v3 = fmaxf(v3, 0.0f);
+          }
+          uint2 o;
+          o.x = pack_bf16x2(v0, v1);
+          o.y = pack_bf16x2(v2, v3);
+          *reinterpret_cast<uint2*>(T + row * (N3 * 2) + (pw_swz<RL3>(row, n >> 3) << 4) + half * 8) = o;
+        }
+      }
+    __syncthreads();
+#pragma unroll
+    for (int i = 0; i < BM * RL3 / 256; ++i) {
+      const int q = tid + i * 256;
+      const int row = q / RL3, lc = q % RL3;
+      const uint4 v = *reinterpret_cast<const uint4*>(T + row * (N3 * 2) + (pw_swz<RL3>(row, lc) << 4));
+      const int m = pix(row);
+      if (m >= 0) *reinterpret_cast<uint4*>(p.y3 + (size_t)m * p.ldy3 + lc * 8) = v;
+    }
+  }
+}
+
+template <int K1A, int K1B, int N2, bool QUAD = false, int N3 = 0>
 static int launch_pw_chain(const PwChainArgs& a, hipStream_t stream) {
   constexpr int BM = 64;
   constexpr int SMEM = BM * (K1A + K1B) * 2 + BM * 512;
   static bool attr_set = false;
-  auto kern = pw_chain_kernel<K1A, K1B, N2, BM, QUAD>;
+  auto kern = pw_chain_kernel<K1A, K1B, N2, BM, QUAD, N3>;
   if (!attr_set) {
     if (hipFuncSetAttribute(reinterpret_cast<const void*>(kern), hipFuncAttributeMaxDynamicSharedMemorySize, SMEM) != hipSuccess)
       return FX_ERR_RUNTIME;
@@ -298,12 +378,17 @@
   return 0;
 }
 
+extern "C" int fx_pw_chain_proj_supported(int K1a, int K1b, int N1, int N2, int N3) {
+  return (K1a == 128 && K1b == 0 && N1 > 0 && N1 % 256 == 0 && N2 == 256 && N3 == 256) ? 1 : 0;
+}
+
 extern "C" int fx_pw_chain_bf16(const fx_pw_chain_desc* d, fx_stream_t stream_) {
   FX_CHECK_ARG(d && d->x1 && d->w1 && d->bias1 && d->M > 0);
   FX_CHECK_ARG(d->y1 || (d->pool && d->N2 > 0));
   FX_CHECK_ARG(d->K1b == 0 || d->x2);
   FX_CHECK_ARG((d->act1 == FX_ACT_NONE || d->act1 == FX_ACT_RELU) && (d->act2 == FX_ACT_NONE || d->act2 == FX_ACT_RELU));
   FX_CHECK_ARG(d->N2 == 0 || (d->w2 && d->bias2 && d->y2));
+  FX_CHECK_ARG(d->N3 >= 0 && (d->N3 == 0 || (d->w3 && d->bias3 && d->y3 && (d->act3 == FX_ACT_NONE || d->act3 == FX_ACT_RELU))));
   if (!fx_pw_chain_supported(d->K1a, d->K1b, d->N1, d->N2)) return FX_ERR_UNSUPPORTED;
   FX_CHECK_ARG(d->ldx1 >= d->K1a && d->ldx1 % 8 == 0 && (!d->y1 || (d->ldy1 >= d->N1 && d->ldy1 % 8 == 0)));
   FX_CHECK_ARG(d->K1b == 0 || (d->ldx2 >= d->K1b && d->ldx2 % 8 == 0));
@@ -312,6 +397,11 @@
   FX_CHECK_ARG(((uintptr_t)d->x1 % 16) == 0 && ((uintptr_t)d->x2 % 16) == 0 && ((uintptr_t)d->residual % 16) == 0);
   FX_CHECK_ARG(((uintptr_t)d->w1 % 16) == 0 && ((uintptr_t)d->w2 % 16) == 0 && ((uintptr_t)d->y1 % 16) == 0 && ((uintptr_t)d->y2 % 16) == 0);
   FX_CHECK_ARG(((uintptr_t)d->bias1 % 16) == 0 && ((uintptr_t)d->bias2 % 16) == 0);
+  if (d->N3) {
+    if (!fx_pw_chain_proj_supported(d->K1a, d->K1b, d->N1, d->N2, d->N3)) return FX_ERR_UNSUPPORTED;
+    FX_CHECK_ARG(d->ldy3 >= d->N3 && d->ldy3 % 8 == 0);
+    FX_CHECK_ARG(((uintptr_t)d->w3 % 16) == 0 && ((uintptr_t)d->bias3 % 16) == 0 && ((uintptr_t)d->y3 % 16) == 0);
+  }
   const int64_t x1_bytes = ((int64_t)d->M - 1) * d->ldx1 * 2 + (int64_t)d->K1a * 2;
   const int64_t x2_bytes = d->K1b ? ((int64_t)d->M - 1) * d->ldx2 * 2 + (int64_t)d->K1b * 2 : 0;
   const int64_t r_bytes = d->residual ? ((int64_t)d->M - 1) * d->ldr * 2 + (int64_t)d->N1 * 2 : 0;
@@ -326,6 +416,10 @@
   a.b2 = d->bias2;
   a.y1 = reinterpret_cast<bf16_t*>(d->y1);
   a.y2 = reinterpret_cast<bf16_t*>(d->y2);
+  a.w3p = reinterpret_cast<const bf16_t*>(d->w3);
+  a.b3 = d->bias3;
+  a.y3 = reinterpret_cast<bf16_t*>(d->y3);
+  a.ldy3 = d->ldy3; a.act3 = d->act3;
   a.ldx1 = d->ldx1; a.ldx2 = d->ldx2; a.ldr = d->ldr; a.ldy1 = d->ldy1; a.ldy2 = d->ldy2;
   a.M = d->M; a.N1 = d->N1; a.act1 = d->act1; a.act2 = d->act2;
   a.x1_bytes = (unsigned)x1_bytes; a.x2_bytes = (unsigned)x2_bytes; a.r_bytes = (unsigned)r_bytes;
@@ -335,12 +429,14 @@
     FX_CHECK_ARG(d->img_h > 0 && d->img_w > 0 && d->img_h % 2 == 0 && d->img_w % 2 == 0 && d->M % (d->img_h * d->img_w) == 0);
     FX_CHECK_ARG(d->ldp >= d->N1 && d->ldp % 8 == 0 && ((uintptr_t)d->pool % 16) == 0);
     if (!fx_pw_chain_pool_supported(d->K1a, d->K1b, d->N1, d->N2)) return FX_ERR_UNSUPPORTED;
+    if (d->N3) return launch_pw_chain<128, 0, 256, true, 256>(a, stream);
 #define FX_PW_CASE(KA, KB, NN2) \
   if (d->K1a == KA && d->K1b == KB && d->N2 == NN2) return launch_pw_chain<KA, KB, NN2, true>(a, stream);
     FX_PW_POOL_INSTANCES(FX_PW_CASE)
 #undef FX_PW_CASE
     return FX_ERR_UNSUPPORTED;
   }
+  if (d->N3) return launch_pw_chain<128, 0, 256, false, 256>(a, stream);
 #define FX_PW_CASE(KA, KB, NN2) \
   if (d->K1a == KA && d->K1b == KB && d->N2 == NN2) return launch_pw_chain<KA, KB, NN2>(a, stream);
   FX_PW_INSTANCES(FX_PW_CASE)
diff --git a/focoos_amd/csrc/conv_pw_kplane.hip b/focoos_amd/csrc/conv_pw_kplane.hip
--- a/focoos_amd/csrc/conv_pw_kplane.hip
+++ b/focoos_amd/csrc/conv_pw_kplane.hip
@@ -4,6 +4,9 @@
 
 #ifndef FX_PWK_RES_DEPTH
 #define FX_PWK_RES_DEPTH 3
+#endif
+#ifndef FX_PWK_K512_BM64_MAX_M
+#define FX_PWK_K512_BM64_MAX_M 16000
 #endif
 
 int fx_tune(const char* env_name, int default_value);
@@ -34,14 +37,16 @@
 __device__ __forceinline__ float pwk_act(float v, std::integral_constant<int, FX_ACT_RELU>) { return fmaxf(v, 0.0f); }
 __device__ __forceinline__ float pwk_act(float v, std::integral_constant<int, FX_ACT_SILU>) { return v * __builtin_amdgcn_rcpf(1.0f + __expf(-v)); }
 __device__ __forceinline__ float pwk_act(float v, std::integral_constant<int, FX_ACT_NONE>) { return v; }
+__device__ __forceinline__ float pwk_act(float v, std::integral_constant<int, FX_ACT_GELU>) { return fx_act(v, FX_ACT_GELU); }
 
 template <int K, int ACT, int RESMODE, int TM = 4, int ABL = 0>
-__global__ __launch_bounds__(256, TM == 4 ? 2 : 3) void conv_pw_kplane_kernel(const PWKArgs p) {
+__global__ __launch_bounds__(256, (TM == 4 || K == 512) ? 2 : 3) void conv_pw_kplane_kernel(const PWKArgs p) {
   constexpr int TN = 2, NW = 4, BM = TM * 32, BN = 256;
   constexpr int NTHR = 256, NDW = NTHR / 64;
   constexpr int KS = K / 16;
   constexpr int PLANE = BM * 16, XBYTES = 2 * KS * PLANE;
   constexpr int PF = 4;
+  constexpr bool BIAS_LATE = ACT == FX_ACT_GELU;
   static_assert(KS % PF == 0 && (KS - 1) * PLANE < 65536, "plane offsets are 16-bit immediates");
   extern __shared__ __attribute__((aligned(16))) unsigned char smem[];
   float* biasL = reinterpret_cast<float*>(smem + XBYTES);
@@ -97,7 +102,8 @@
     for (int a = 0; a < TN; ++a)
 #pragma unroll
       for (int gq = 0; gq < 4; ++gq) {
-        const float4 bb = *reinterpret_cast<const float4*>(biasL + n0 + (wave * TN + a) * 32 + 8 * gq + 4 * half);
+        float4 bb = *reinterpret_cast<const float4*>(biasL + n0 + (wave * TN + a) * 32 + 8 * gq + 4 * half);
+        if constexpr (BIAS_LATE) bb = make_float4(0.0f, 0.0f, 0.0f, 0.0f);
 #pragma unroll
         for (int b = 0; b < TM; ++b) {
           acc[a][b][4 * gq] = bb.x; acc[a][b][4 * gq + 1] = bb.y; acc[a][b][4 * gq + 2] = bb.z; acc[a][b][4 * gq + 3] = bb.w;
@@ -183,11 +189,17 @@
           for (int q = 0; q < 2; ++q) {
             const int gq = 2 * g2 + q;
             float v[4];
+            float bl[4] = {0.0f, 0.0f, 0.0f, 0.0f};
+            if constexpr (BIAS_LATE) {
+              const float4 bb = *reinterpret_cast<const float4*>(biasL + n0 + (wave * TN + a) * 32 + 8 * gq + 4 * half);
+              bl[0] = bb.x; bl[1] = bb.y; bl[2] = bb.z; bl[3] = bb.w;
+            }
             const float r[4] = {bf16lo_to_f32(rq[q][0]), bf16hi_to_f32(rq[q][0]), bf16lo_to_f32(rq[q][1]),
                                 bf16hi_to_f32(rq[q][1])};
 #pragma unroll
             for (int e = 0; e < 4; ++e) {
               v[e] = acc[a][b][4 * gq + e];
+              if constexpr (BIAS_LATE) v[e] += bl[e];
               if constexpr (RESMODE == 1) v[e] += r[e];
               v[e] = pwk_act(v[e], std::integral_constant<int, ACT>{});
               if constexpr (RESMODE == 3) v[e] = r[e] > 0.0f ? v[e] : 0.0f;
@@ -238,7 +250,7 @@
 bool fx_pw_kplane_supported(int C, int N, int mode) {
   if (N <= 0 || N % 256 != 0 || N > 4096) return false;
   static const int k512_res = fx_tune("FX_PWK_K512_RES", 1);
-  if (C == 256) return mode == 0 || mode == 1 || mode == 3 || mode == 4 || mode == 5 || mode == 6;
+  if (C == 256) return mode == 0 || mode == 1 || mode == 3 || mode == 4 || mode == 5 || mode == 6 || mode == 7;
   if (C == 512) return mode == 0 || mode == 1 || mode == 3 || (k512_res && (mode == 4 || mode == 5 || mode == 6));
   return false;
 }
@@ -257,8 +269,20 @@
       case 4: return launch_pwk<256, FX_ACT_RELU, 1>(a, stream);
       case 5: return launch_pwk<256, FX_ACT_NONE, 3>(a, stream);
       case 6: return launch_pwk<256, FX_ACT_NONE, 1>(a, stream);
+      case 7: return launch_pwk<256, FX_ACT_GELU, 0>(a, stream);
     }
   } else {
+    const int bm64 = fx_tune("FX_PWK_K512_BM64_MAX_M", FX_PWK_K512_BM64_MAX_M);
+    if (c.M <= bm64) {
+      switch (mode) {
+        case 0: return launch_pwk<512, FX_ACT_RELU, 0, 2>(a, stream);
+        case 1: return launch_pwk<512, FX_ACT_SILU, 0, 2>(a, stream);
+        case 3: return launch_pwk<512, FX_ACT_NONE, 0, 2>(a, stream);
+        case 4: return launch_pwk<512, FX_ACT_RELU, 1, 2>(a, stream);
+        case 5: return launch_pwk<512, FX_ACT_NONE, 3, 2>(a, stream);
+        case 6: return launch_pwk<512, FX_ACT_NONE, 1, 2>(a, stream);
+      }
+    }
     switch (mode) {
       case 0: return launch_pwk<512, FX_ACT_RELU, 0>(a, stream);
       case 1: return launch_pwk<512, FX_ACT_SILU, 0>(a, stream);
diff --git a/focoos_amd/engine.py b/focoos_amd/engine.py
--- a/focoos_amd/engine.py
+++ b/focoos_amd/engine.py
@@ -661,8 +661,18 @@
         self._op(self.lib.fx_conv2d_nhwc_bf16, C.byref(d))
         return out
 
+    def _pointwise_variant(self, pc: PackedConv, B: int, H: int, W: int, ldy: int) -> str:
+        d = FxConvDesc()
+        d.x = d.y = d.w = pc.w.data_ptr()
+        d.bias, d.w_frag = pc.b.data_ptr(), (pc.wf.data_ptr() if pc.wf is not None else None)
+        d.B, d.H, d.W, d.C, d.ldx, d.Ho, d.Wo, d.N, d.ldy = B, H, W, pc.C, pc.C, H, W, pc.N, ldy
+        d.KH, d.KW, d.stride, d.pad = 1, 1, 1, 0
+        label = C.create_string_buffer(64)
+        check(self.lib.fx_conv2d_variant(C.byref(d), label, 64), "fx_conv2d_variant")
+        return label.value.decode()
+
     def pw_chain(self, x1: NT, x2: Optional[NT], residual: Optional[NT], cc: Tuple, ca: Optional[Tuple], name1: str, name2: Optional[str],
-                 pool_name: Optional[str] = None, keep_y1: bool = True):
+                 pool_name: Optional[str] = None, keep_y1: bool = True, proj: Optional[Tuple[PackedConv, NT]] = None):
         w1, b1, k1a, k1b, n1 = cc
         assert x1.C == k1a and (x2 is None) == (k1b == 0) and (x2 is None or x2.C == k1b), (name1, x1.C, k1a, k1b)
         M = x1.rows
@@ -685,12 +695,19 @@
         if pool_name is not None:
             pooled = self._new(pool_name, x1.B, x1.H // 2, x1.W // 2, n1)
             d.pool, d.ldp, d.img_h, d.img_w = pooled.ptr, pooled.ld, x1.H, x1.W
+        n3 = 0
+        if proj is not None:
+            pc3, y3 = proj
+            assert pc3.KH == 1 and pc3.KW == 1 and pc3.C == n1 and pc3.wf is not None and y3.C == pc3.N and y3.rows == M, (name1, pc3.C, n1)
+            n3 = pc3.N
+            d.N3, d.w3, d.bias3, d.y3, d.ldy3, d.act3 = n3, pc3.wf.data_ptr(), pc3.b.data_ptr(), y3.ptr, y3.ld, FX_ACT["none"]
         self.keep.append(d)
         self.meta[len(self.ops)] = {"kind": "conv", "variant": f"pw_chain<{k1a},{k1b},{n2}>" + ("+pool" if pooled is not None else "") + ("-y1" if y1 is None else ""),
-                                    "flops": 2.0 * M * n1 * (k1a + k1b + n2),
-                                    "name": name1 + ("+" + name2.rsplit("res_layers.", 1)[-1] if name2 else ""), "M": M, "N": n1, "K": k1a + k1b,
+                                    "flops": 2.0 * M * n1 * (k1a + k1b + n2 + n3),
+                                    "name": name1 + ("+" + name2.rsplit("res_layers.", 1)[-1] if name2 else "") + ("+proj" if n3 else ""),
+                                    "M": M, "N": n1, "K": k1a + k1b,
                                     "bytes": 2.0 * M * (k1a + k1b + (n1 if residual is not None else 0) + (n1 if y1 is not None else 0) + n2
-                                                        + (n1 / 4 if pooled is not None else 0))}
+                                                        + (n1 / 4 if pooled is not None else 0) + n3) + 2.0 * n1 * n3}
         self._op(self.lib.fx_pw_chain_bf16, C.byref(d))
         if pool_name is not None:
             return y1, y2, pooled
@@ -732,7 +749,8 @@
         self._op(self.lib.fx_mha_bf16, q.ptr, q.ld, k.ptr, k.ld, v.ptr, v.ld, out.ptr, out.ld, B, L, L, 8)
         return out
 
-    def build_backbone(self) -> Dict[int, NT]:
+    def build_backbone(self, proj: Optional[Dict[int, Tuple[PackedConv, NT]]] = None) -> Dict[int, NT]:
+        self.fused_proj = set()
         e, P, B, lib = self.eng, self.eng.P, self.B, self.lib
         H, W = self.H, self.W
         bb = "pixel_decoder.backbone"
@@ -796,14 +814,21 @@
                     cc = None
             if cc is not None:
                 nxt_name = f"{bb}.res_layers.{nxt[0]}.blocks.{nxt[1]}.a" if n2 else None
+                pj = proj.get(si + 2) if (proj and bi == blocks[si] - 1) else None
+                if pj is not None and not (pj[0].wf is not None and pj[0].KH == 1 and pj[0].C == cc[4]
+                                           and lib.fx_pw_chain_proj_supported(cc[2], cc[3], cc[4], n2, pj[0].N) == 1
+                                           and self._pointwise_variant(pj[0], bmid.B, bmid.H, bmid.W, pj[1].ld).startswith("pw_kplane")):
+                    pj = None
+                if pj is not None:
+                    self.fused_proj.add(si + 2)
                 want_pool = (use_pool and nxt is not None and nxt[0] == si + 1 and bi != 0 and bmid.H % 2 == 0 and bmid.W % 2 == 0
                              and lib.fx_pw_chain_pool_supported(cc[2], cc[3], cc[4], n2) == 1)
                 if want_pool:
                     keep = bool(n2 == 0 or (si + 2) in self.needed_res or os.environ.get("FX_SKIP_UNUSED_RES", "1") == "0")
                     x, a_next, pooled_next = self.pw_chain(bmid, short_in, x, cc, e.chain_a[nxt] if n2 else None, f"{p}.c", nxt_name,
-                                                           pool_name=f"{bb}.res_layers.{nxt[0]}.blocks.0.pool", keep_y1=keep)
+                                                           pool_name=f"{bb}.res_layers.{nxt[0]}.blocks.0.pool", keep_y1=keep, proj=pj)
                 else:
-                    x, a_next = self.pw_chain(bmid, short_in, None if bi == 0 else x, cc, e.chain_a[nxt] if n2 else None, f"{p}.c", nxt_name)
+                    x, a_next = self.pw_chain(bmid, short_in, None if bi == 0 else x, cc, e.chain_a[nxt] if n2 else None, f"{p}.c", nxt_name, proj=pj)
             else:
                 short = x if bi != 0 else self.conv(short_in, P[f"{p}.short" if si == 0 else f"{p}.short.conv"], name=f"{p}.s")
                 x = self.conv(bmid, P[f"{p}.branch2c"], name=f"{p}.c", residual=short, act="relu")
@@ -859,17 +884,28 @@
     def _build(self):
         e, P, B, lib = self.eng, self.eng.P, self.B, self.lib
         H, W = self.H, self.W
-        feats = self.build_stdc() if e.stdc else self.build_backbone()
         fd = e.fd
         pd = "pixel_decoder"
+        cat80 = None
+        if not e.stdc and os.environ.get("FX_PW_CHAIN_PROJ", "1") != "0":
+            h8, w8 = H, W
+            for _ in range(3):
+                h8, w8 = (h8 + 1) // 2, (w8 + 1) // 2
+            cat80 = self._new("cat80", B, h8, w8, 2 * fd)
+            feats = self.build_backbone(proj={3: (P[f"{pd}.input_proj.0"], cat80.slice(fd, fd))})
+        else:
+            feats = self.build_stdc() if e.stdc else self.build_backbone()
         (h8, w8), (h16, w16), (h32, w32) = ((feats[k].H, feats[k].W) for k in (3, 4, 5))
         if h8 * w8 + h16 * w16 + h32 * w32 < e.nq:
             raise _lib.FocoosAmdError(f"input {H}x{W} gives {h8 * w8 + h16 * w16 + h32 * w32} encoder tokens, fewer than the {e.nq} queries to select")
-        cat80 = self._new("cat80", B, h8, w8, 2 * fd)
+        if cat80 is None:
+            cat80 = self._new("cat80", B, h8, w8, 2 * fd)
+        assert (cat80.H, cat80.W) == (h8, w8)
         cat40a = self._new("cat40a", B, h16, w16, 2 * fd)
         cat40b = self._new("cat40b", B, h16, w16, 2 * fd)
         cat20 = self._new("cat20", B, h32, w32, 2 * fd)
-        self.conv(feats[3], P[f"{pd}.input_proj.0"], out=cat80.slice(fd, fd))
+        if 3 not in getattr(self, "fused_proj", ()):
+            self.conv(feats[3], P[f"{pd}.input_proj.0"], out=cat80.slice(fd, fd))
         self.conv(feats[4], P[f"{pd}.input_proj.1"], out=cat40a.slice(fd, fd))
         src = self.conv(feats[5], P[f"{pd}.input_proj.2"], name="proj5")
         L = h32 * w32
diff --git a/include/focoos_amd.h b/include/focoos_amd.h
--- a/include/focoos_amd.h
+++ b/include/focoos_amd.h
@@ -8,7 +8,7 @@
 extern "C" {
 #endif
 
-#define FX_ABI_VERSION 17
+#define FX_ABI_VERSION 18
 
 enum { FX_OK = 0, FX_ERR_INVALID_ARGUMENT = -1, FX_ERR_LAUNCH = -2, FX_ERR_UNSUPPORTED = -3, FX_ERR_RUNTIME = -4 };
 enum { FX_ACT_NONE = 0, FX_ACT_RELU = 1, FX_ACT_SILU = 2, FX_ACT_GELU = 3 };
@@ -57,10 +57,16 @@
   int32_t ldx1, ldx2, ldr, ldy1, ldy2;
   int32_t act1, act2;
   void* pool;
-  int32_t ldp, img_h, img_w, reserved0;
+  int32_t ldp, img_h, img_w;
+  int32_t N3;
+  const void* w3;
+  const float* bias3;
+  void* y3;
+  int32_t ldy3, act3;
 } fx_pw_chain_desc;
 int fx_pw_chain_supported(int K1a, int K1b, int N1, int N2);
 int fx_pw_chain_pool_supported(int K1a, int K1b, int N1, int N2);
+int fx_pw_chain_proj_supported(int K1a, int K1b, int N1, int N2, int N3);
 int fx_pw_chain_bf16(const fx_pw_chain_desc* d, fx_stream_t stream);
 
 int fx_stem_conv3x3s2(const void* x, int in_f32, const float* w, const float* bias, const float* mean,
```
